# miha-stopar/Plonky3-mobile

Hardware: AMD Instinct MI355X
Metric: fib_air proofs/sec (higher is better)
Workload: dtype u32 (BabyBear Montgomery, 31-bit modular)

## Files before the change

### plonky3-mobile_amd/csrc/common.h

```cpp
#pragma once
#include <hip/hip_runtime.h>
#include <stdint.h>

#include <map>
#include <set>
#include <string>
#include <tuple>
#include <vector>

namespace p3 {

#ifndef P3_NO_SETPRIO
#define P3_LATENCY_BOUND_KERNEL() __builtin_amdgcn_s_setprio(3)
#else
#define P3_LATENCY_BOUND_KERNEL() ((void)0)
#endif

enum Profile : int { PROFILE_THROUGHPUT = 0, PROFILE_LATENCY = 1 };

enum Status : int {
    OK = 0,
    ERR_BAD_ARG = -1,
    ERR_HIP = -2,
    ERR_BACKEND = -3,
    ERR_INTERNAL = -4,
};

void set_error(const std::string& msg);
int fail(int code, const std::string& msg);

#define P3_HIP(call)                                                                       \
    do {                                                                                   \
        hipError_t e__ = (call);                                                           \
        if (e__ != hipSuccess)                                                             \
            return p3::fail(p3::ERR_HIP, std::string(#call) + ": " + hipGetErrorString(e__)); \
    } while (0)

struct DevBuf {
    void* ptr = nullptr;
    size_t cap = 0;
    int reserve(size_t bytes);
    template <class T>
    T* as() const { return reinterpret_cast<T*>(ptr); }
    ~DevBuf();
};

struct TwoLevelTable {
    uint32_t* lo = nullptr;
    uint32_t* hi = nullptr;
    uint32_t T = 0;
};

struct CachedTable {
    TwoLevelTable t;
    hipEvent_t ready = nullptr;
    hipStream_t built_on = nullptr;
    bool complete = false;
};

struct Context {
    int device = -1;
    int profile = PROFILE_LATENCY;
    uint32_t* tile_tw[2] = {nullptr, nullptr};
    double2* tile_twd[2] = {nullptr, nullptr};
    std::map<std::pair<uint32_t, int>, CachedTable> root_tables;
    std::map<std::tuple<uint32_t, uint32_t, uint32_t>, CachedTable> scale_tables;
    std::map<std::pair<hipStream_t, int>, DevBuf> scratch;
    std::set<const void*> attr_done;
    uint64_t* rng_jump = nullptr;
    std::map<uint32_t, CachedTable> selector_tables;
    int init(int dev);
    DevBuf& ws(hipStream_t stream, int slot);
    int get_root_table(hipStream_t stream, uint32_t q, bool inverse, TwoLevelTable* out);
    int get_scale_table(hipStream_t stream, uint32_t base, uint32_t log_n, uint32_t mult, TwoLevelTable* out);
    int reserve_scale_slots(size_t k);
    int mark_built(hipStream_t stream, CachedTable& e);
    int wait_ready(hipStream_t stream, CachedTable& e);
    int ensure_dynamic_lds(const void* kernel, int bytes);
    ~Context();
};

int get_context(Context** out);
void release_thread_contexts();

int ntt_dft(Context& cx, hipStream_t stream, const uint32_t* src, uint32_t* dst, uint64_t height,
            uint32_t width, bool inverse);
std::vector<uint32_t> ntt_dft_plan(uint32_t n);
int ntt_coset_lde(Context& cx, hipStream_t stream, const uint32_t* src, uint32_t* dst, uint64_t height,
                  uint32_t width, uint32_t added_bits, uint32_t shift_monty, bool bit_reversed_out);
int ntt_coset_lde_from_coeffs(Context& cx, hipStream_t stream, const uint32_t* coeffs, uint32_t* dst, uint32_t* scratch,
                              uint64_t height, uint32_t width, uint32_t added_bits, uint32_t shift_monty);
int ntt_coset_dft(Context& cx, hipStream_t stream, const uint32_t* src, uint32_t* dst, uint64_t height,
                  uint32_t width, uint32_t shift_monty);
int bit_reverse_rows(hipStream_t stream, const uint32_t* src, uint32_t* dst, uint64_t height, uint32_t width);

int fib_trace(hipStream_t stream, uint64_t a, uint64_t b, uint64_t n, uint32_t* d_out);
enum : uint32_t {
    TRACE_BAD_FIRST_LEFT = 1, TRACE_BAD_FIRST_RIGHT = 2, TRACE_BAD_NEXT_LEFT = 4, TRACE_BAD_NEXT_RIGHT = 8, TRACE_BAD_LAST_RIGHT = 16,
    TRACE_BAD_RANGE = 32,
};
struct TraceCheck {
    int64_t first_bad_row;
    uint32_t mask;
    uint64_t bad_rows;
};
int fib_check_trace(Context& cx, hipStream_t stream, const uint32_t* d_trace, uint64_t n, const uint32_t pis[3], TraceCheck* out);

inline bool is_pow2(uint64_t v) { return v && !(v & (v - 1)); }
inline uint32_t log2u(uint64_t v) {
    uint32_t l = 0;
    while ((1ull << l) < v) l++;
    return l;
}

}
```

### plonky3-mobile_amd/csrc/mmcs.hip

```cpp
#include <algorithm>

#include "common.h"
#include "mmcs.h"
#include "poseidon2.hip.h"
#include "poseidon2_coop.hip.h"
#include "poseidon2_f64.hip.h"
#include "poseidon2_q4.hip.h"
#include "keccak.hip.h"

namespace p3 {

constexpr int MAX_CLASS_MATS = 16;

struct RowSet {
    const uint32_t* ptr[MAX_CLASS_MATS];
    uint32_t width[MAX_CLASS_MATS];
    uint32_t stride[MAX_CLASS_MATS];
    uint32_t count;
    uint32_t total;
};

__device__ __forceinline__ void load_digest(const uint32_t* p, uint32_t* out8) {
    const uint4* q = reinterpret_cast<const uint4*>(p);
    uint4 a = q[0], b = q[1];
    out8[0] = a.x; out8[1] = a.y; out8[2] = a.z; out8[3] = a.w;
    out8[4] = b.x; out8[5] = b.y; out8[6] = b.z; out8[7] = b.w;
}
__device__ __forceinline__ void store_digest(uint32_t* p, const uint32_t* s) {
    uint4* q = reinterpret_cast<uint4*>(p);
    q[0] = make_uint4(s[0], s[1], s[2], s[3]);
    q[1] = make_uint4(s[4], s[5], s[6], s[7]);
}

__device__ __forceinline__ void sponge_row(const RowSet& rs, uint64_t r, uint32_t (&s)[16]) {
#pragma unroll
    for (int i = 0; i < 16; i++) s[i] = 0;
    if (rs.count == 1) {
        const uint32_t* row = rs.ptr[0] + r * rs.stride[0];
        const uint32_t w = rs.width[0];
        for (uint32_t k = 0; k < w; k += 8) {
#pragma unroll
            for (int i = 0; i < 8; i++)
                if (k + i < w) s[i] = row[k + i];
            p2::permute(s);
        }
        return;
    }
    uint32_t m = 0, off = 0;
    for (uint32_t k = 0; k < rs.total; k += 8) {
#pragma unroll
        for (int i = 0; i < 8; i++) {
            if (k + i < rs.total) {
                while (off >= rs.width[m]) { m++; off = 0; }
                s[i] = rs.ptr[m][r * rs.stride[m] + off];
                off++;
            }
        }
        p2::permute(s);
    }
}

__global__ void __launch_bounds__(256) leaf_hash_kernel(RowSet rs, uint64_t n_rows, uint32_t* digests) {
    if (gridDim.x <= 512u) P3_LATENCY_BOUND_KERNEL();
    uint64_t r = (uint64_t)blockIdx.x * blockDim.x + threadIdx.x;
    if (r >= n_rows) return;
    uint32_t s[16];
    sponge_row(rs, r, s);
    store_digest(digests + r * 8, s);
}

__global__ void __launch_bounds__(256) compress_layer_kernel(const uint32_t* prev, uint32_t* next, uint64_t n_out,
                                                             RowSet rs, uint32_t inject) {
    if (gridDim.x <= 512u) P3_LATENCY_BOUND_KERNEL();
    uint64_t i = (uint64_t)blockIdx.x * blockDim.x + threadIdx.x;
    if (i >= n_out) return;
    uint32_t s[16];
    load_digest(prev + i * 16, s);
    load_digest(prev + i * 16 + 8, s + 8);
    p2::permute(s);
    if (inject) {
        uint32_t h[16];
        sponge_row(rs, i, h);
#pragma unroll
        for (int k = 0; k < 8; k++) s[8 + k] = h[k];
        p2::permute(s);
    }
    store_digest(next + i * 8, s);
}

__global__ void __launch_bounds__(256) tree_top_kernel(uint32_t* layer0, uint32_t n0) {
    P3_LATENCY_BOUND_KERNEL();
    extern __shared__ __attribute__((aligned(16))) uint32_t lds[];
    const uint32_t tid = threadIdx.x;
    for (uint32_t i = tid; i < n0 * 8; i += blockDim.x) lds[i] = layer0[i];
    __syncthreads();
    uint32_t* out = layer0 + (size_t)n0 * 8;
    for (uint32_t n = n0; n > 1; n >>= 1) {
        uint32_t half = n >> 1;
        uint32_t s[16];
        bool act = tid < half;
        if (act) {
#pragma unroll
            for (int k = 0; k < 16; k++) s[k] = lds[tid * 16 + k];
            p2::permute(s);
        }
        __syncthreads();
        if (act) {
#pragma unroll
            for (int k = 0; k < 8; k++) lds[tid * 8 + k] = s[k];
            store_digest(out + tid * 8, s);
        }
        __syncthreads();
        out += (size_t)half * 8;
    }
}


__global__ void __launch_bounds__(256) leaf_hash_f64_kernel(const uint32_t* mat, uint32_t width, uint64_t n_rows, uint32_t* digests) {
    if (gridDim.x <= 512u) P3_LATENCY_BOUND_KERNEL();
    uint64_t r = (uint64_t)blockIdx.x * blockDim.x + threadIdx.x;
    if (r >= n_rows) return;
    double s[16];
#pragma unroll
    for (int i = 0; i < 16; i++) s[i] = 0.0;
    const uint32_t* row = mat + r * width;
    for (uint32_t k = 0; k < width; k += 8) {
#pragma unroll
        for (int i = 0; i < 8; i++)
            if (k + i < width) s[i] = p2f::load_elem(row[k + i]);
        p2f::permute(s);
        if (k + 8 < width) {
#pragma unroll
            for (int i = 0; i < 16; i++) s[i] = p2f::reduce(s[i]);
        }
    }
    uint32_t d[8];
    const p2f::MagicRegs smk = p2f::magic_regs();
#pragma unroll
    for (int i = 0; i < 8; i++) d[i] = p2f::store_elem(s[i], smk);
    store_digest(digests + r * 8, d);
}
__global__ void __launch_bounds__(256) compress_layer_q4_kernel(const uint32_t* prev, uint32_t* next, uint64_t n_out, uint32_t prio) {
    if (prio) P3_LATENCY_BOUND_KERNEL();
    const uint32_t q = threadIdx.x & 3u;
    const uint64_t i = ((uint64_t)blockIdx.x * blockDim.x + threadIdx.x) >> 2;
    const bool act = i < n_out;
    const p2q::LaneConsts lc = p2q::lane_consts(q);
    double s[4] = {0.0, 0.0, 0.0, 0.0};
    if (act) {
        const uint4 w = *reinterpret_cast<const uint4*>(prev + i * 16 + 4 * q);
        s[0] = p2f::load_elem(w.x); s[1] = p2f::load_elem(w.y); s[2] = p2f::load_elem(w.z); s[3] = p2f::load_elem(w.w);
    }
    p2q::permute(s, lc, q == 0);
    if (act && q < 2) {
        const p2f::MagicRegs smk = p2f::magic_regs();
        *reinterpret_cast<uint4*>(next + i * 8 + 4 * q) =
            make_uint4(p2f::store_elem(s[0], smk), p2f::store_elem(s[1], smk), p2f::store_elem(s[2], smk), p2f::store_elem(s[3], smk));
    }
}
__global__ void __launch_bounds__(256) leaf_hash_q4_kernel(const uint32_t* mat, uint32_t width, uint64_t n_rows, uint32_t* digests, uint32_t prio) {
    if (prio) P3_LATENCY_BOUND_KERNEL();
    const uint32_t q = threadIdx.x & 3u;
    const uint64_t r = ((uint64_t)blockIdx.x * blockDim.x + threadIdx.x) >> 2;
    const bool act = r < n_rows;
    const p2q::LaneConsts lc = p2q::lane_consts(q);
    double s[4] = {0.0, 0.0, 0.0, 0.0};
    const uint32_t* row = mat + (act ? r : 0) * width;
    for (uint32_t k = 0; k < width; k += 8) {
        if (act && q < 2) {
#pragma unroll
            for (uint32_t i = 0; i < 4; i++)
                if (k + 4 * q + i < width) s[i] = p2f::load_elem(row[k + 4 * q + i]);
        }
        p2q::permute(s, lc, q == 0);
        if (k + 8 < width) {
#pragma unroll
            for (int i = 0; i < 4; i++) s[i] = p2f::reduce(s[i]);
        }
    }
    if (act && q < 2) {
        const p2f::MagicRegs smk = p2f::magic_regs();
        *reinterpret_cast<uint4*>(digests + r * 8 + 4 * q) =
            make_uint4(p2f::store_elem(s[0], smk), p2f::store_elem(s[1], smk), p2f::store_elem(s[2], smk), p2f::store_elem(s[3], smk));
    }
}
constexpr uint32_t LEAF_WIDE_CHUNK = 32, LEAF_WIDE_STRIDE = 36;
__global__ void __launch_bounds__(256) leaf_hash_f64_wide_kernel(const uint32_t* mat, uint32_t width, uint64_t n_rows, uint32_t* digests) {
    __shared__ __attribute__((aligned(16))) uint32_t tile[256 * LEAF_WIDE_STRIDE];
    const uint32_t tid = threadIdx.x, col = tid & 31u, rsub = tid >> 5;
    const uint64_t r0 = (uint64_t)blockIdx.x * 256u, r = r0 + tid;
    double s[16];
#pragma unroll
    for (int i = 0; i < 16; i++) s[i] = 0.0;
    uint32_t pre[32];
    auto fetch = [&](uint32_t c0) {
#pragma unroll
        for (uint32_t i = 0; i < 32; i++) {
            const uint64_t row = r0 + rsub + 8u * i;
            pre[i] = (row < n_rows && c0 + col < width) ? mat[row * width + c0 + col] : 0u;
        }
    };
    fetch(0);
    for (uint32_t c0 = 0; c0 < width; c0 += LEAF_WIDE_CHUNK) {
        __syncthreads();
#pragma unroll
        for (uint32_t i = 0; i < 32; i++) tile[(rsub + 8u * i) * LEAF_WIDE_STRIDE + col] = pre[i];
        __syncthreads();
        if (c0 + LEAF_WIDE_CHUNK < width) fetch(c0 + LEAF_WIDE_CHUNK);
        const uint4* mine = reinterpret_cast<const uint4*>(tile + tid * LEAF_WIDE_STRIDE);
#pragma unroll 1
        for (uint32_t k = 0; k < LEAF_WIDE_CHUNK && c0 + k < width; k += 8) {
            const uint4 a = mine[k / 4], b = mine[k / 4 + 1];
            const uint32_t w[8] = {a.x, a.y, a.z, a.w, b.x, b.y, b.z, b.w};
#pragma unroll
            for (int i = 0; i < 8; i++)
                if (c0 + k + i < width) s[i] = p2f::load_elem(w[i]);
            p2f::permute(s);
            if (c0 + k + 8 < width) {
#pragma unroll
                for (int i = 0; i < 16; i++) s[i] = p2f::reduce(s[i]);
            }
        }
    }
    if (r >= n_rows) return;
    uint32_t d[8];
    const p2f::MagicRegs smk = p2f::magic_regs();
#pragma unroll
    for (int i = 0; i < 8; i++) d[i] = p2f::store_elem(s[i], smk);
    store_digest(digests + r * 8, d);
}
__global__ void __launch_bounds__(256) leaf_hash_f64_rowset_kernel(RowSet rs, uint64_t n_rows, uint32_t* digests) {
    if (gridDim.x <= 512u) P3_LATENCY_BOUND_KERNEL();
    uint64_t r = (uint64_t)blockIdx.x * blockDim.x + threadIdx.x;
    if (r >= n_rows) return;
    double s[16];
#pragma unroll
    for (int i = 0; i < 16; i++) s[i] = 0.0;
    uint32_t m = 0, off = 0;
    for (uint32_t k = 0; k < rs.total; k += 8) {
#pragma unroll
        for (int i = 0; i < 8; i++) {
            if (k + i < rs.total) {
                while (off >= rs.width[m]) { m++; off = 0; }
                s[i] = p2f::load_elem(rs.ptr[m][r * rs.stride[m] + off]);
                off++;
            }
        }
        p2f::permute(s);
        if (k + 8 < rs.total) {
#pragma unroll
            for (int i = 0; i < 16; i++) s[i] = p2f::reduce(s[i]);
        }
    }
    uint32_t d[8];
    const p2f::MagicRegs smk = p2f::magic_regs();
#pragma unroll
    for (int i = 0; i < 8; i++) d[i] = p2f::store_elem(s[i], smk);
    store_digest(digests + r * 8, d);
}
__global__ void __launch_bounds__(256) compress_layer_f64_kernel(const uint32_t* prev, uint32_t* next, uint64_t n_out) {
    if (gridDim.x <= 512u) P3_LATENCY_BOUND_KERNEL();
    uint64_t i = (uint64_t)blockIdx.x * blockDim.x + threadIdx.x;
    if (i >= n_out) return;
    uint32_t w[16];
    load_digest(prev + i * 16, w);
    load_digest(prev + i * 16 + 8, w + 8);
    double s[16];
#pragma unroll
    for (int k = 0; k < 16; k++) s[k] = p2f::load_elem(w[k]);
    p2f::permute(s);
    uint32_t d[8];
    const p2f::MagicRegs smk = p2f::magic_regs();
#pragma unroll
    for (int k = 0; k < 8; k++) d[k] = p2f::store_elem(s[k], smk);
    store_digest(next + i * 8, d);
}

__global__ void __launch_bounds__(256) compress_coop_kernel(const uint32_t* prev, uint32_t* next, uint32_t n_out) {
    P3_LATENCY_BOUND_KERNEL();
    const uint32_t lane16 = threadIdx.x & 15;
    const p2c::LaneConst lc = p2c::lane_constants(lane16);
    uint32_t i = (blockIdx.x * blockDim.x + threadIdx.x) >> 4;
    bool act = i < n_out;
    uint32_t v = act ? prev[(size_t)i * 16 + lane16] : 0u;
    v = p2c::permute(v, lc);
    if (act && lane16 < 8) next[(size_t)i * 8 + lane16] = v;
}
__global__ void __launch_bounds__(256) leaf_coop_kernel(const uint32_t* mat, uint32_t width, uint32_t n_rows, uint32_t* digests) {
    P3_LATENCY_BOUND_KERNEL();
    const uint32_t lane16 = threadIdx.x & 15;
    const p2c::LaneConst lc = p2c::lane_constants(lane16);
    uint32_t r = (blockIdx.x * blockDim.x + threadIdx.x) >> 4;
    bool act = r < n_rows;
    uint32_t v = 0;
    for (uint32_t k = 0; k < width; k += 8) {
        if (act && lane16 < 8 && k + lane16 < width) v = mat[(size_t)r * width + k + lane16];
        v = p2c::permute(v, lc);
    }
    if (act && lane16 < 8) digests[(size_t)r * 8 + lane16] = v;
}
__global__ void __launch_bounds__(1024) tree_levels_coop_kernel(uint32_t* layer_in, uint32_t n_in, uint32_t chunk, uint32_t levels,
                                                                uint32_t* root_copy) {
    P3_LATENCY_BOUND_KERNEL();
    __shared__ uint32_t lds[128 * 8];
    const uint32_t tid = threadIdx.x, lane16 = tid & 15, grp = tid >> 4;
    const p2c::LaneConst lc = p2c::lane_constants(lane16);
    const uint32_t* src = layer_in + (size_t)blockIdx.x * chunk * 8;
    for (uint32_t i = tid; i < chunk * 8; i += blockDim.x) lds[i] = src[i];
    __syncthreads();
    uint32_t* out = layer_in + (size_t)n_in * 8;
    uint32_t cur_n = n_in;
    for (uint32_t l = 0; l < levels; l++) {
        const uint32_t half = chunk >> (l + 1);
        const bool wave_active = ((tid >> 6) << 2) < half;
        uint32_t res = 0;
        if (wave_active) {
            uint32_t v = grp < half ? lds[grp * 16 + lane16] : 0u;
            res = p2c::permute(v, lc);
        }
        __syncthreads();
        if (grp < half && lane16 < 8) {
            lds[grp * 8 + lane16] = res;
            out[((size_t)blockIdx.x * half + grp) * 8 + lane16] = res;
            if (cur_n == 2 && root_copy) root_copy[lane16] = res;
        }
        __syncthreads();
        cur_n >>= 1;
        out += (size_t)cur_n * 8;
    }
}

__global__ void poseidon2_permute_kernel(uint32_t* states, uint64_t n) {
    uint64_t i = (uint64_t)blockIdx.x * blockDim.x + threadIdx.x;
    if (i >= n) return;
    uint32_t s[16];
    uint4* q = reinterpret_cast<uint4*>(states + i * 16);
#pragma unroll
    for (int k = 0; k < 4; k++) { uint4 v = q[k]; s[4 * k] = v.x; s[4 * k + 1] = v.y; s[4 * k + 2] = v.z; s[4 * k + 3] = v.w; }
    p2::permute(s);
#pragma unroll
    for (int k = 0; k < 4; k++) q[k] = make_uint4(s[4 * k], s[4 * k + 1], s[4 * k + 2], s[4 * k + 3]);
}


__global__ void poseidon2_permute_f64_kernel(uint32_t* states, uint64_t n) {
    uint64_t i = (uint64_t)blockIdx.x * blockDim.x + threadIdx.x;
    if (i >= n) return;
    double s[16];
    uint4* q = reinterpret_cast<uint4*>(states + i * 16);
#pragma unroll
    for (int k = 0; k < 4; k++) {
        uint4 v = q[k];
        s[4 * k] = p2f::load_elem(v.x); s[4 * k + 1] = p2f::load_elem(v.y); s[4 * k + 2] = p2f::load_elem(v.z); s[4 * k + 3] = p2f::load_elem(v.w);
    }
    p2f::permute(s);
#pragma unroll
    for (int k = 0; k < 4; k++)
        q[k] = make_uint4(p2f::store_elem(s[4 * k]), p2f::store_elem(s[4 * k + 1]), p2f::store_elem(s[4 * k + 2]), p2f::store_elem(s[4 * k + 3]));
}

__global__ void poseidon2_f64_probe_kernel(const double* in, uint32_t* out, uint64_t n, int mode) {
    uint64_t i = (uint64_t)blockIdx.x * blockDim.x + threadIdx.x;
    if (i >= n) return;
    double s[16];
#pragma unroll
    for (int k = 0; k < 16; k++) s[k] = in[i * 16 + k];
    if (mode == 0) p2f::permute(s);
    else if (mode == 1) p2f::internal_rounds(s, p2f::magic_regs());
    else {
#pragma unroll
        for (int k = 0; k < 16; k++) s[k] = p2f::reduce(s[k]);
    }
#pragma unroll
    for (int k = 0; k < 16; k++) out[i * 16 + k] = p2f::store_elem(s[k]);
}
int poseidon2_f64_probe(hipStream_t stream, const double* d_in, uint32_t* d_out, uint64_t n, int mode) {
    if (!n) return OK;
    hipLaunchKernelGGL(poseidon2_f64_probe_kernel, dim3((uint32_t)((n + 255) / 256)), dim3(256), 0, stream, d_in, d_out, n, mode);
    P3_HIP(hipGetLastError());
    return OK;
}
int poseidon2_permute_states_variant(hipStream_t stream, uint32_t* d_states, uint64_t n, int variant) {
    if (!n) return OK;
    if (variant == 1) hipLaunchKernelGGL(poseidon2_permute_f64_kernel, dim3((uint32_t)((n + 255) / 256)), dim3(256), 0, stream, d_states, n);
    else hipLaunchKernelGGL(poseidon2_permute_kernel, dim3((uint32_t)((n + 255) / 256)), dim3(256), 0, stream, d_states, n);
    P3_HIP(hipGetLastError());
    return OK;
}

int poseidon2_permute_states(hipStream_t stream, uint32_t* d_states, uint64_t n) {
    return poseidon2_permute_states_variant(stream, d_states, n, 1);
}

__device__ __forceinline__ uint32_t rowset_elem(const RowSet& rs, uint64_t r, uint32_t k, uint32_t& m, uint32_t& base) {
    while (k - base >= rs.width[m]) { base += rs.width[m]; m++; }
    return rs.ptr[m][r * rs.stride[m] + (k - base)];
}
__device__ __forceinline__ void keccak_sponge_row(const RowSet& rs, uint64_t r, uint64_t (&st)[25]) {
#pragma unroll
    for (int i = 0; i < 25; i++) st[i] = 0;
    const uint32_t n = rs.total, n64 = (n + 1) / 2;
    uint32_t m = 0, base = 0;
    for (uint32_t i = 0; i < n64; i += 17) {
#pragma unroll
        for (int k = 0; k < 17; k++) {
            const uint32_t e = 2 * (i + k);
            if (e < n) {
                uint64_t lo = rowset_elem(rs, r, e, m, base);
                uint64_t hi = e + 1 < n ? rowset_elem(rs, r, e + 1, m, base) : 0u;
                st[k] = lo | (hi << 32);
            }
        }
        if (i + 17 >= n64) kk::permute_digest(st);
        else kk::permute(st);
    }
}
__device__ __forceinline__ void store_digest64(uint32_t* p, const uint64_t (&st)[25]) {
    uint4* q = reinterpret_cast<uint4*>(p);
    q[0] = make_uint4((uint32_t)st[0], (uint32_t)(st[0] >> 32), (uint32_t)st[1], (uint32_t)(st[1] >> 32));
    q[1] = make_uint4((uint32_t)st[2], (uint32_t)(st[2] >> 32), (uint32_t)st[3], (uint32_t)(st[3] >> 32));
}
__global__ void __launch_bounds__(256) keccak_leaf_kernel(RowSet rs, uint64_t n_rows, uint32_t* digests) {
    if (gridDim.x <= 512u) P3_LATENCY_BOUND_KERNEL();
// ... 237 lines not shown
    uint64_t base = 0, len = 1ull << a.log_max_height;
    for (uint32_t i = 0; i < a.log_max_height; i++) {
        uint64_t sib = (index >> i) ^ 1;
        if (threadIdx.x < 8) out[off + i * 8 + threadIdx.x] = layers[base + sib * 8 + threadIdx.x];
        base += len * 8;
        len >>= 1;
    }
}

__global__ void __launch_bounds__(64) open_gather_many_kernel(OpenArgs a, const uint32_t* layers, const uint32_t* indices, uint32_t row_words,
                                                              uint32_t* rows, uint32_t* paths) {
    if (gridDim.x <= 512u) P3_LATENCY_BOUND_KERNEL();
    const uint64_t index = (uint64_t)indices[blockIdx.x] & ((1ull << a.log_max_height) - 1ull);
    uint32_t* dst = rows + (size_t)blockIdx.x * row_words;
    uint32_t off = 0;
    for (uint32_t m = 0; m < a.n_mats; m++) {
        const uint64_t r = index >> a.shift[m];
        for (uint32_t c = threadIdx.x; c < a.width[m]; c += blockDim.x) dst[off + c] = a.mat[m][r * a.stride[m] + c];
        off += a.width[m];
    }
    uint32_t* pdst = paths + (size_t)blockIdx.x * a.log_max_height * 8;
    uint64_t base = 0, len = 1ull << a.log_max_height;
    for (uint32_t i = 0; i < a.log_max_height; i++) {
        const uint64_t sib = (index >> i) ^ 1;
        if (threadIdx.x < 8) pdst[i * 8 + threadIdx.x] = layers[base + sib * 8 + threadIdx.x];
        base += len * 8;
        len >>= 1;
    }
}

static RowSet make_rowset(const Tree& t, uint64_t h) {
    RowSet rs{};
    for (size_t m = 0; m < t.mats.size(); m++)
        if (t.heights[m] == h) {
            rs.ptr[rs.count] = t.mats[m];
            rs.width[rs.count] = (uint32_t)t.widths[m];
            rs.stride[rs.count] = (uint32_t)t.strides[m];
            rs.total += (uint32_t)t.widths[m];
            rs.count++;
        }
    return rs;
}


static bool has_height(const Tree& t, uint64_t h) {
    for (size_t m = 0; m < t.mats.size(); m++)
        if (t.heights[m] == h) return true;
    return false;
}

Tree::~Tree() {
    if (layers && owns_layers) (void)hipFree(layers);
    if (staging) (void)hipFree(staging);
    for (void* p : owned) (void)hipFree(p);
}

int mmcs_commit(hipStream_t stream, const uint32_t* const* d_mats, const size_t* heights, const size_t* widths,
                size_t n_mats, Tree** out, uint32_t* ext_layers, uint32_t* root_copy, int kind, const size_t* strides, int profile) {
    if (kind != HASH_POSEIDON2 && kind != HASH_KECCAK) return fail(ERR_BAD_ARG, "mmcs_commit: unknown hash configuration");
    if (!n_mats || !d_mats || !heights || !widths || !out) return fail(ERR_BAD_ARG, "mmcs_commit: null/empty argument");
    if (n_mats > 64) return fail(ERR_BAD_ARG, "mmcs_commit: at most 64 matrices per commitment");
    uint64_t maxh = 0;
    for (size_t i = 0; i < n_mats; i++) {
        if (!is_pow2(heights[i])) return fail(ERR_BAD_ARG, "mmcs_commit: heights must be powers of two");
        if (widths[i] > 0xffffffffull) return fail(ERR_BAD_ARG, "mmcs_commit: width too large");
        if (heights[i] > maxh) maxh = heights[i];
    }
    std::unique_ptr<Tree> t(new Tree());
    t->kind = kind;
    for (size_t i = 0; i < n_mats; i++) {
        t->mats.push_back(d_mats[i]); t->heights.push_back(heights[i]); t->widths.push_back(widths[i]);
        const size_t st = strides ? strides[i] : widths[i];
        if (st < widths[i] || st > 0xffffffffull) return fail(ERR_BAD_ARG, "mmcs_commit: row stride below the width");
        t->strides.push_back(st);
    }
    t->log_max_height = log2u(maxh);
    for (uint64_t h = maxh; h >= 1; h >>= 1) {
        size_t cnt = 0;
        for (size_t i = 0; i < n_mats; i++) cnt += heights[i] == h;
        if (cnt > MAX_CLASS_MATS) return fail(ERR_BAD_ARG, "mmcs_commit: more than 16 matrices of one height");
        if (h == 1) break;
    }
    size_t total_digests = 2 * maxh - 1;
    size_t staging_words = 0;
    for (size_t i = 0; i < n_mats; i++) staging_words += widths[i];
    staging_words += (size_t)t->log_max_height * 8 + 8;
    t->staging_words = staging_words;
    if (ext_layers) { t->layers = ext_layers; t->owns_layers = false; }
    else P3_HIP(hipMalloc(reinterpret_cast<void**>(&t->layers), total_digests * 32));
    size_t off = 0;
    for (uint64_t len = maxh; len >= 1; len >>= 1) {
        t->layer_off.push_back(off);
        t->layer_len.push_back(len);
        off += len * 8;
        if (len == 1) break;
    }
    constexpr uint64_t COOP_MAX = 1ull << 12;
    constexpr uint32_t COOP_CHUNK_LOG = 5;
    const uint64_t Q4_MAX = profile == PROFILE_LATENCY ? (1ull << 15) : 0;
    constexpr uint32_t Q4_PRIO = 1;
    const uint64_t KCOOP_IN = profile == PROFILE_LATENCY ? (1ull << 12) : (1ull << 10);
    constexpr uint32_t KCOOP_CHUNK_LOG = 4;
    constexpr uint64_t KLANE_CHUNK = 1ull << 7;
    if (kind == HASH_KECCAK) {
        RowSet rs0 = make_rowset(*t, maxh);
        if (rs0.count == 1 && rs0.width[0] >= 68 && rs0.stride[0] == rs0.width[0])
            hipLaunchKernelGGL(keccak_leaf_wide_kernel, dim3((uint32_t)((maxh + 255) / 256)), dim3(256), 0, stream, rs0.ptr[0], rs0.width[0], maxh,
                               t->layers);
        else if (!launch_keccak_leaf_salted(stream, rs0, maxh, t->layers))
            hipLaunchKernelGGL(keccak_leaf_kernel, dim3((uint32_t)((maxh + 255) / 256)), dim3(256), 0, stream, rs0, maxh, t->layers);
        P3_HIP(hipGetLastError());
        for (size_t l = 1; l < t->layer_len.size(); l++) {
            uint64_t len = t->layer_len[l];
            RowSet rs = make_rowset(*t, len);
            if (len < COOP_MAX && !rs.count) {
                const uint64_t n_in = t->layer_len[l - 1];
                const bool coop = n_in <= KCOOP_IN;
                uint32_t levels = 0;
                while (levels < (coop ? KCOOP_CHUNK_LOG : 11u) && l + levels < t->layer_len.size() && !has_height(*t, t->layer_len[l + levels])) levels++;
                if (!coop) while (levels > 1 && (n_in >> levels) < KCOOP_IN) levels--;
                const uint32_t chunk = (uint32_t)std::min<uint64_t>(n_in, coop ? 1ull << KCOOP_CHUNK_LOG : KLANE_CHUNK);
                while ((1u << levels) > chunk) levels--;
                if (coop)
                    hipLaunchKernelGGL(keccak_tree_levels_coop_kernel, dim3((uint32_t)(n_in / chunk)), dim3(std::max<uint32_t>(64, chunk * 32)), 0,
                                       stream, t->layers + t->layer_off[l - 1], (uint32_t)n_in, chunk, levels, root_copy);
                else
                    hipLaunchKernelGGL(keccak_tree_levels_kernel, dim3((uint32_t)(n_in / chunk)), dim3(std::max<uint32_t>(64, chunk / 2)),
                                       (size_t)chunk * 32, stream, t->layers + t->layer_off[l - 1], (uint32_t)n_in, chunk, levels, root_copy);
                P3_HIP(hipGetLastError());
                if (t->layer_len[l + levels - 1] == 1) t->root_copied = root_copy != nullptr;
                l += levels - 1;
                continue;
            }
            hipLaunchKernelGGL(keccak_compress_kernel, dim3((uint32_t)((len + 255) / 256)), dim3(256), 0, stream,
                               t->layers + t->layer_off[l - 1], t->layers + t->layer_off[l], len, rs, rs.count > 0 ? 1u : 0u);
            P3_HIP(hipGetLastError());
        }
        *out = t.release();
        return OK;
    }
    {
        RowSet rs = make_rowset(*t, maxh);
        const bool dense1 = rs.count == 1 && rs.stride[0] == rs.width[0];
        if (dense1 && maxh < COOP_MAX && maxh * 16 <= 0x7fffffffull) {
            hipLaunchKernelGGL(leaf_coop_kernel, dim3((uint32_t)((maxh * 16 + 255) / 256)), dim3(256), 0, stream, rs.ptr[0],
                               rs.width[0], (uint32_t)maxh, t->layers);
        } else if (dense1 && maxh <= Q4_MAX && rs.width[0] <= 64 && (reinterpret_cast<uintptr_t>(t->layers) & 15u) == 0) {
            hipLaunchKernelGGL(leaf_hash_q4_kernel, dim3((uint32_t)((maxh * 4 + 255) / 256)), dim3(256), 0, stream, rs.ptr[0], rs.width[0], maxh,
                               t->layers, Q4_PRIO);
        } else if (dense1 && rs.width[0] >= 64) {
            hipLaunchKernelGGL(leaf_hash_f64_wide_kernel, dim3((uint32_t)((maxh + 255) / 256)), dim3(256), 0, stream, rs.ptr[0],
                               rs.width[0], maxh, t->layers);
        } else if (dense1) {
            hipLaunchKernelGGL(leaf_hash_f64_kernel, dim3((uint32_t)((maxh + 255) / 256)), dim3(256), 0, stream, rs.ptr[0],
                               rs.width[0], maxh, t->layers);
        } else if ((maxh >= COOP_MAX || (rs.count == 1 && !dense1))) {
            hipLaunchKernelGGL(leaf_hash_f64_rowset_kernel, dim3((uint32_t)((maxh + 255) / 256)), dim3(256), 0, stream, rs, maxh, t->layers);
        } else {
            hipLaunchKernelGGL(leaf_hash_kernel, dim3((uint32_t)((maxh + 255) / 256)), dim3(256), 0, stream, rs, maxh, t->layers);
        }
        P3_HIP(hipGetLastError());
    }
    for (size_t l = 1; l < t->layer_len.size();) {
        uint64_t len = t->layer_len[l];
        RowSet rs = make_rowset(*t, len);
        bool inject = rs.count > 0;
        if (!inject && len < COOP_MAX) {
            uint32_t levels = 0;
            while (levels < COOP_CHUNK_LOG && l + levels < t->layer_len.size() && !has_height(*t, t->layer_len[l + levels])) levels++;
            uint64_t n_in = t->layer_len[l - 1];
            uint32_t chunk = (uint32_t)std::min<uint64_t>(n_in, 1ull << COOP_CHUNK_LOG);
            while ((1u << levels) > chunk) levels--;
            uint32_t blocks = (uint32_t)(n_in / chunk);
            uint32_t threads = std::max<uint32_t>(64, chunk * 8);
            bool makes_root = t->layer_len[l + levels - 1] == 1;
            hipLaunchKernelGGL(tree_levels_coop_kernel, dim3(blocks), dim3(threads), 0, stream, t->layers + t->layer_off[l - 1],
                               (uint32_t)n_in, chunk, levels, makes_root ? root_copy : nullptr);
            P3_HIP(hipGetLastError());
            if (makes_root) t->root_copied = root_copy != nullptr;
            l += levels;
            continue;
        }
        if (!inject && len <= Q4_MAX) {
            hipLaunchKernelGGL(compress_layer_q4_kernel, dim3((uint32_t)((len * 4 + 255) / 256)), dim3(256), 0, stream,
                               t->layers + t->layer_off[l - 1], t->layers + t->layer_off[l], len, Q4_PRIO);
        } else if (!inject) {
            hipLaunchKernelGGL(compress_layer_f64_kernel, dim3((uint32_t)((len + 255) / 256)), dim3(256), 0, stream,
                               t->layers + t->layer_off[l - 1], t->layers + t->layer_off[l], len);
        } else {
            hipLaunchKernelGGL(compress_layer_kernel, dim3((uint32_t)((len + 255) / 256)), dim3(256), 0, stream,
                               t->layers + t->layer_off[l - 1], t->layers + t->layer_off[l], len, rs, inject ? 1u : 0u);
        }
        P3_HIP(hipGetLastError());
        l++;
    }
    *out = t.release();
    return OK;
}

int mmcs_root(hipStream_t stream, const Tree& t, uint32_t root_out[8]) {
    P3_HIP(hipMemcpyAsync(root_out, t.layers + t.layer_off.back(), 32, hipMemcpyDeviceToHost, stream));
    P3_HIP(hipStreamSynchronize(stream));
    return OK;
}

static OpenArgs make_open_args(const Tree& t) {
    OpenArgs a{};
    a.n_mats = (uint32_t)t.mats.size();
    a.log_max_height = t.log_max_height;
    for (size_t m = 0; m < t.mats.size(); m++) {
        a.mat[m] = t.mats[m];
        a.width[m] = (uint32_t)t.widths[m];
        a.stride[m] = (uint32_t)t.strides[m];
        a.shift[m] = t.log_max_height - log2u(t.heights[m]);
    }
    return a;
}
size_t mmcs_row_words(const Tree& t) {
    size_t row_words = 0;
    for (size_t w : t.widths) row_words += w;
    return row_words;
}

int mmcs_open(hipStream_t stream, const Tree& tc, uint64_t index, uint32_t* rows_out, uint32_t* path_out) {
    Tree& t = const_cast<Tree&>(tc);
    if (index >> t.log_max_height) return fail(ERR_BAD_ARG, "mmcs_open: index out of range");
    if (!t.staging) P3_HIP(hipMalloc(reinterpret_cast<void**>(&t.staging), t.staging_words * 4));
    const OpenArgs a = make_open_args(t);
    const size_t row_words = mmcs_row_words(t);
    hipLaunchKernelGGL(open_gather_kernel, dim3(1), dim3(64), 0, stream, a, t.layers, index, t.staging);
    P3_HIP(hipGetLastError());
    std::vector<uint32_t> host(row_words + (size_t)t.log_max_height * 8);
    if (!host.empty()) {
        P3_HIP(hipMemcpyAsync(host.data(), t.staging, host.size() * 4, hipMemcpyDeviceToHost, stream));
        P3_HIP(hipStreamSynchronize(stream));
    }
    if (row_words) memcpy(rows_out, host.data(), row_words * 4);
    if (t.log_max_height) memcpy(path_out, host.data() + row_words, (size_t)t.log_max_height * 32);
    return OK;
}

int mmcs_open_many(hipStream_t stream, const Tree& t, const uint32_t* d_indices, size_t n, uint32_t* d_rows, uint32_t* d_paths) {
    const size_t row_words = mmcs_row_words(t);
    if (n > 0x7fffffffull) return fail(ERR_BAD_ARG, "mmcs_open_batch_many: more than 2^31 - 1 indices");
    if (row_words > 0xffffffffull) return fail(ERR_BAD_ARG, "mmcs_open_batch_many: row too wide");
    if (n && (!d_indices || (row_words && !d_rows) || (t.log_max_height && !d_paths))) return fail(ERR_BAD_ARG, "mmcs_open_batch_many: null argument");
    if (!n) return OK;
    hipLaunchKernelGGL(open_gather_many_kernel, dim3((uint32_t)n), dim3(64), 0, stream, make_open_args(t), t.layers, d_indices, (uint32_t)row_words,
                       d_rows, d_paths);
    P3_HIP(hipGetLastError());
    return OK;
}

}
```

### plonky3-mobile_amd/csrc/ntt.hip

```cpp
#include <algorithm>

#include "bb31.hip.h"
#include "common.h"

namespace p3 {

enum SideKind : uint32_t {
    SIDE_INPLACE = 0,
    SIDE_GROUP = 1,
    SIDE_GROUP_REV = 2,
    SIDE_STRIDED = 3,
};

struct PassArgs {
    const uint32_t* src;
    uint32_t* dst;
    uint64_t src_rows;
    uint32_t W, wshift;
    uint32_t n, b, s0;
    uint32_t dif;
    uint32_t load_kind, store_kind;
    uint32_t G;
    uint32_t n_inner;
    const uint32_t* tile_tw;
// ... 648 lines not shown
    if (bi < 5 || (W < 32 && !is_pow2(W))) return 1;
    if (bi < 6) return 1;
    const uint64_t N = 1ull << n;
    size_t bytes = N * W * 4;
    int rc = cx.ws(stream, 1).reserve(bytes);
    if (rc) return rc;
    uint32_t* coeffs = cx.ws(stream, 1).as<uint32_t>();
    {
        uint32_t digits[2] = {e1, e2};
        uint32_t s = 0;
        for (int i = 0; i < 2; i++) {
            PassArgs a{};
            a.W = W; a.n = n; a.b = digits[i]; a.s0 = s; a.dif = 0;
            a.tile_tw = cx.tile_tw[1];
            a.src_rows = N;
            if (i == 0) { a.src = src; a.dst = coeffs; a.load_kind = SIDE_STRIDED; a.store_kind = SIDE_GROUP_REV; }
            else { a.src = coeffs; a.dst = coeffs; a.load_kind = SIDE_INPLACE; a.store_kind = SIDE_INPLACE; }
            rc = set_twiddle(cx, stream, a, true);
            if (rc) return rc;
            rc = launch_pass(cx, stream, a);
            if (rc) return rc;
            s += digits[i];
        }
    }
    {
        PassArgs a{};
        a.W = W; a.n = n; a.b = bi; a.s0 = s0;
        a.wshift = is_pow2(W) ? log2u(W) : 0xffffffffu;
        a.src = coeffs; a.dst = dst;
        a.tile_tw = cx.tile_tw[1];
        a.tile_tw2 = cx.tile_tw[0];
        TwoLevelTable ti, tf, sc;
        if ((rc = cx.get_root_table(stream, s0 + bi, true, &ti))) return rc;
        if ((rc = cx.get_root_table(stream, s0 + e3, false, &tf))) return rc;
        uint32_t hinv = bb::inv(bb::to_monty((uint32_t)N));
        if ((rc = cx.get_scale_table(stream, shift, n, hinv, &sc))) return rc;
        a.tw_lo = ti.lo; a.tw_hi = ti.hi; a.tw_T = ti.T;
        a.tw2_lo = tf.lo; a.tw2_hi = tf.hi; a.tw2_T = tf.T;
        a.sc_lo = sc.lo; a.sc_hi = sc.hi; a.sc_T = sc.T;
        a.sc_step = bb::pow(shift, 1ull << s0);
        a.sc_step16 = bb::pow(a.sc_step, 16);
        uint64_t F = (uint64_t)W << s0;
        uint32_t blocks = (uint32_t)((F + 31) / 32);
        if (bi == 6 && added == 1) rc = launch_fused_mid_t<6, 1>(stream, a, blocks);
        else if (bi == 7 && added == 1) rc = launch_fused_mid_t<7, 1>(stream, a, blocks);
        else if (bi == 6 && added == 2) rc = launch_fused_mid_t<6, 2>(stream, a, blocks);
        else return fail(ERR_INTERNAL, "lde_fused: unexpected digit shape");
        if (rc) return rc;
    }
    {
        PassArgs a{};
        a.W = W; a.n = m; a.b = e2; a.s0 = e1; a.dif = 1;
        a.tile_tw = cx.tile_tw[0];
        a.src = dst; a.dst = dst; a.src_rows = 1ull << m;
        a.load_kind = SIDE_INPLACE; a.store_kind = SIDE_INPLACE;
        if ((rc = set_twiddle(cx, stream, a, false))) return rc;
        if ((rc = launch_pass(cx, stream, a))) return rc;
        PassArgs b{};
        b.W = W; b.n = m; b.b = e1; b.s0 = 0; b.dif = 1;
        b.tile_tw = cx.tile_tw[0];
        b.src = dst; b.dst = dst; b.src_rows = 1ull << m;
        b.load_kind = SIDE_GROUP; b.store_kind = SIDE_GROUP;
        if ((rc = set_twiddle(cx, stream, b, false))) return rc;
        if ((rc = launch_pass(cx, stream, b))) return rc;
    }
    return OK;
}


template <int B, int LQ, int VW, int K>
int launch_narrow_t(Context& cx, hipStream_t stream, const NarrowArgs& a, uint32_t blocks, uint32_t grid_y = 1) {
    constexpr size_t tile_bytes = ((size_t)4 * VW * narrow::lds_rows(B)) << LQ;
    constexpr size_t n_tiles = K == 2 ? (B - 4 + LQ >= 10 ? 1 : NARROW_MID_TILES) : (B >= 11 ? 1 : NARROW_EDGE_TILES);
    constexpr size_t lds = tile_bytes * n_tiles + ((size_t)4 << (B - 4)) * (K == 2 ? 2 : 1);
    static_assert(lds <= 160 * 1024, "narrow tile does not fit the LDS");
    void (*kern)(NarrowArgs);
    if constexpr (K == 1) kern = narrow_inv1_kernel<B, LQ, VW>;
    else if constexpr (K == 2) kern = narrow_mid_kernel<B, LQ, VW>;
    else kern = narrow_fwd2_kernel<B, LQ, VW>;
    if constexpr (lds > 64 * 1024) {
        int rc = cx.ensure_dynamic_lds(reinterpret_cast<const void*>(kern), (int)lds);
        if (rc) return rc;
    }
    hipLaunchKernelGGL(kern, dim3(blocks, K == 2 ? grid_y : 1u), dim3(1u << (B - 4 + LQ)), lds, stream, a);
    P3_HIP(hipGetLastError());
    return OK;
}
constexpr int narrow_lq(int b, int vw) { return (b == 12 ? 1 : 2) + (vw == 1 ? 1 : 0); }
template <int K, int VW>
int launch_narrow_v(Context& cx, hipStream_t stream, const NarrowArgs& a, uint32_t b, uint32_t blocks, uint32_t gy) {
    if (b == 10) return launch_narrow_t<10, narrow_lq(10, VW), VW, K>(cx, stream, a, blocks, gy);
    if constexpr (VW == 2) {
        if (b == 11) return launch_narrow_t<11, narrow_lq(11, 2), 2, K>(cx, stream, a, blocks, gy);
        if (b == 12) return launch_narrow_t<12, narrow_lq(12, 2), 2, K>(cx, stream, a, blocks, gy);
    }
    return fail(ERR_INTERNAL, "lde_narrow: no integer kernel for this digit / lane vector");
}
template <int K>
int launch_narrow(Context& cx, hipStream_t stream, const NarrowArgs& a, uint32_t b, uint32_t blocks, int vw, uint32_t gy = 1) {
    return vw == 1 ? launch_narrow_v<K, 1>(cx, stream, a, b, blocks, gy) : launch_narrow_v<K, 2>(cx, stream, a, b, blocks, gy);
}

template <int B, int LQ, int VW, int K, int NT>
int launch_narrow64_nt(Context& cx, hipStream_t stream, const NarrowArgs& a, uint32_t blocks, uint32_t grid_y) {
    constexpr size_t lds = narrow64::lds_bytes<B, LQ, VW, NT>(K == 2 ? 2 : 1);
    static_assert(lds <= 160 * 1024, "fp64 narrow tile does not fit the LDS");
    void (*kern)(NarrowArgs);
    if constexpr (K == 1) kern = narrow64_inv1_kernel<B, LQ, VW, NT>;
    else if constexpr (K == 2) kern = narrow64_mid_kernel<B, LQ, VW, NT, (VW == 2)>;
    else kern = narrow64_fwd2_kernel<B, LQ, VW, NT>;
    if constexpr (lds > 64 * 1024) {
        int rc = cx.ensure_dynamic_lds(reinterpret_cast<const void*>(kern), (int)lds);
        if (rc) return rc;
    }
    hipLaunchKernelGGL(kern, dim3(blocks, K == 2 ? grid_y : 1u), dim3(1u << (B - 4 + LQ)), lds, stream, a);
    P3_HIP(hipGetLastError());
    return OK;
}
template <int B, int LQ, int VW, int K>
int launch_narrow64_t(Context& cx, hipStream_t stream, const NarrowArgs& a, uint32_t blocks, uint32_t grid_y) {
    constexpr bool fits2 = narrow64::lds_bytes<B, LQ, VW, 2>(K == 2 ? 2 : 1) <= 160 * 1024;
    if constexpr (fits2) {
        const bool two = (size_t)blocks * grid_y <= 256 || narrow64::lds_bytes<B, LQ, VW, 2>(K == 2 ? 2 : 1) <= 80 * 1024;
        if (two) return launch_narrow64_nt<B, LQ, VW, K, 2>(cx, stream, a, blocks, grid_y);
    }
    return launch_narrow64_nt<B, LQ, VW, K, 1>(cx, stream, a, blocks, grid_y);
}
constexpr bool narrow64_has(int b, int vw, int k) { return b <= 10 && b - 4 + narrow_lq(b, vw) <= (k == 2 ? 9 : 10); }
template <int K, int VW>
int launch_narrow64_v(Context& cx, hipStream_t stream, const NarrowArgs& a, uint32_t b, uint32_t blocks, uint32_t gy) {
#define P3_N64_CASE(BB)                                                                                          \
    case BB:                                                                                                     \
        if constexpr (narrow64_has(BB, VW, K)) return launch_narrow64_t<BB, narrow_lq(BB, VW), VW, K>(cx, stream, a, blocks, gy); \
        else return fail(ERR_INTERNAL, "lde_narrow: fp64 shape not instantiated");
    switch (b) {
        P3_N64_CASE(8) P3_N64_CASE(9) P3_N64_CASE(10)
        default: return fail(ERR_INTERNAL, "lde_narrow: digit out of range");
    }
#undef P3_N64_CASE
}
template <int K>
int launch_narrow64(Context& cx, hipStream_t stream, const NarrowArgs& a, uint32_t b, uint32_t blocks, int vw, uint32_t gy = 1) {
    return vw == 1 ? launch_narrow64_v<K, 1>(cx, stream, a, b, blocks, gy) : launch_narrow64_v<K, 2>(cx, stream, a, b, blocks, gy);
}

template <int K>
int launch_narrow_wide(Context& cx, hipStream_t stream, const NarrowArgs& a, uint32_t b, uint32_t blocks, uint32_t gy) {
    if (b == 9) return launch_narrow_t<9, 5, 1, K>(cx, stream, a, blocks, gy);
    if (b != 8) return fail(ERR_INTERNAL, "lde_narrow: wide digit out of range");
    return launch_narrow_t<8, 5, 1, K>(cx, stream, a, blocks, gy);
}

int lde_narrow(Context& cx, hipStream_t stream, const uint32_t* src, uint32_t* dst, uint32_t n, uint32_t added, uint32_t W,
               uint32_t shift, bool bit_reversed_out, bool from_coeffs = false) {
    if (!bit_reversed_out || added < 1 || added > 3) return 1;
    constexpr uint32_t w_max = 16;
    const bool wide = W > w_max && n >= 16 && n <= 18 && W >= 64 && (((uint64_t)W << (n + added + 2)) < (1ull << 32));
    if (!wide && (W < 2 || W > w_max || !(is_pow2(W) || W == 6))) return 1;
    if (n < 16 || n > 24) return 1;
    if (!wide && ((reinterpret_cast<uintptr_t>(src) | reinterpret_cast<uintptr_t>(dst)) & 7u)) return 1;
    const uint32_t n1 = (n + 1) / 2, n2 = n - n1;
    const uint64_t N = 1ull << n;
    int vw[3];
    for (int k = 0; k < 3; k++) vw[k] = (n <= 19 || (n == 20 && k == 1)) ? 1 : 2;
    if (wide) vw[0] = vw[1] = vw[2] = 1;
    auto lq_of = [&](int k, uint32_t b) -> uint32_t { return wide ? 5u : (uint32_t)narrow_lq((int)b, vw[k]); };
    int rc = cx.ws(stream, 1).reserve(N * W * 4);
    if (rc) return rc;
    uint32_t* T = cx.ws(stream, 1).as<uint32_t>();
    NarrowArgs a{};
    a.blocked = W == 2 && !from_coeffs;
    bool k3_out_of_place = a.blocked && n1 >= 12;
    uint32_t* mid = dst;
    if (k3_out_of_place) {
        const size_t mid_bytes = (N << added) * W * 4;
        if ((rc = cx.ws(stream, 4).reserve(mid_bytes))) return rc;
        mid = cx.ws(stream, 4).as<uint32_t>();
        const uintptr_t m0 = reinterpret_cast<uintptr_t>(mid), d0 = reinterpret_cast<uintptr_t>(dst);
        if (m0 < d0 + mid_bytes && d0 < m0 + mid_bytes) { a.blocked = 0; k3_out_of_place = false; mid = dst; }
    }
    a.from_coeffs = from_coeffs;
    a.n = n; a.n1 = n1; a.n2 = n2; a.W = W; a.added = added;
    TwoLevelTable ti, tf;
    if ((rc = cx.get_root_table(stream, n, true, &ti))) return rc;
    if ((rc = cx.get_root_table(stream, n, false, &tf))) return rc;
    auto geometry = [&](int k, uint32_t b, uint64_t rows) -> uint32_t {
        const uint32_t slots_per_row = W / vw[k];
        a.spr = slots_per_row;
        a.wsl = is_pow2(slots_per_row) ? log2u(slots_per_row) : 0xffffffffu;
        const uint32_t lq = lq_of(k, b);
        const uint32_t tiles = (uint32_t)((rows * slots_per_row) >> lq);
        const uint32_t group = 8u << (wide ? 0 : (vw[k] == 2 ? 4 : 5) - lq);
        a.xcd_remap = !wide && k != 2 && tiles % group == 0 && is_pow2(slots_per_row);
        if (wide && tiles % 128 == 0) a.xcd_remap = 4;
        return tiles;
    };
    a.src = src; a.dst = T;
    a.stage_tw = cx.tile_tw[1];
    a.tw_lo = ti.lo; a.tw_hi = ti.hi; a.tw_T = ti.T;
    const bool f64 = !wide && (n <= 19 || (n == 20 && W == 2));
    a.stage_twd = cx.tile_twd[1];
    a.neg_pm1 = -2013265920.0; a.pinv = 1.0 / 2013265921.0; a.fbias = -0.5 + 1.0 / 8589934592.0;
    uint32_t tiles = geometry(0, n1, 1ull << n2);
    if (!from_coeffs)
        if ((rc = wide ? launch_narrow_wide<1>(cx, stream, a, n1, tiles, 1)
                       : f64 ? launch_narrow64<1>(cx, stream, a, n1, tiles, vw[0]) : launch_narrow<1>(cx, stream, a, n1, tiles, vw[0]))) return rc;
    a.src = from_coeffs ? src : T; a.dst = mid;
    a.stage_tw = cx.tile_tw[1]; a.stage_tw_fwd = cx.tile_tw[0];
    a.stage_twd = cx.tile_twd[1]; a.stage_twd_fwd = cx.tile_twd[0];
    a.twf_lo = tf.lo; a.twf_hi = tf.hi; a.twf_T = tf.T;
    const uint32_t hinv = from_coeffs ? bb::ONE : bb::inv(bb::to_monty((uint32_t)N));
    const uint32_t g = bb::two_adic_generator(n + added);
    uint32_t base = shift;
    for (uint32_t j = 0; j < (1u << added); j++) {
        TwoLevelTable sc;
        if ((rc = cx.get_scale_table(stream, base, n, hinv, &sc))) return rc;
        a.sc_lo[j] = sc.lo; a.sc_hi[j] = sc.hi; a.sc_T = sc.T;
        a.sc_phi[j] = bb::pow(base, 1ull << (n1 + n2 - 4));
        base = bb::mul(base, g);
    }
    tiles = geometry(1, n2, 1ull << n1);
    uint32_t split_log = 0;
    while (split_log < added && ((uint64_t)tiles << (split_log + 1)) <= 256) split_log++;
    a.cos_per_block = (1u << added) >> split_log;
    if ((rc = wide ? launch_narrow_wide<2>(cx, stream, a, n2, tiles, 1u << split_log)
                   : f64 ? launch_narrow64<2>(cx, stream, a, n2, tiles, vw[1], 1u << split_log)
                         : launch_narrow<2>(cx, stream, a, n2, tiles, vw[1], 1u << split_log))) return rc;
    a.src = mid; a.dst = dst;
    a.stage_tw = cx.tile_tw[0];
    a.stage_twd = cx.tile_twd[0];
    tiles = geometry(2, n1, (1ull << added) << n2);
    a.k3_pairs = k3_out_of_place && vw[2] == 2 && tiles % 16 == 0 ? 1u : 0u;
    if (wide && tiles % 128 == 0) a.k3_pairs = 4;
    if (wide) return launch_narrow_wide<3>(cx, stream, a, n1, tiles, 1);
    return f64 ? launch_narrow64<3>(cx, stream, a, n1, tiles, vw[2]) : launch_narrow<3>(cx, stream, a, n1, tiles, vw[2]);
}

}

std::vector<uint32_t> ntt_dft_plan(uint32_t n) { return split_digits(n); }

int ntt_dft(Context& cx, hipStream_t stream, const uint32_t* src, uint32_t* dst, uint64_t height,
            uint32_t width, bool inverse) {
    if (!height || !width) return OK;
    if (!is_pow2(height)) return fail(ERR_BAD_ARG, "hip backend requires power-of-two height, got " + std::to_string(height));
    uint32_t n = log2u(height);
    if (n > bb::TWO_ADICITY) return fail(ERR_BAD_ARG, "height exceeds BabyBear two-adicity");
    size_t bytes = height * width * 4;
    if (n == 0) {
        if (src != dst) P3_HIP(hipMemcpyAsync(dst, src, bytes, hipMemcpyDeviceToDevice, stream));
        return OK;
    }
    if (src == dst) {
        int rc = cx.ws(stream, 0).reserve(bytes);
        if (rc) return rc;
        P3_HIP(hipMemcpyAsync(cx.ws(stream, 0).ptr, src, bytes, hipMemcpyDeviceToDevice, stream));
        src = cx.ws(stream, 0).as<uint32_t>();
    }
    uint32_t hinv = inverse ? bb::inv(bb::to_monty((uint32_t)height)) : 0;
    return run_dit(cx, stream, src, dst, n, width, inverse, inverse, hinv);
}

int ntt_coset_dft(Context& cx, hipStream_t stream, const uint32_t* src, uint32_t* dst, uint64_t height,
                  uint32_t width, uint32_t shift) {
    if (!height || !width) return OK;
    if (!is_pow2(height)) return fail(ERR_BAD_ARG, "hip backend requires power-of-two height, got " + std::to_string(height));
    uint32_t n = log2u(height);
    if (n > bb::TWO_ADICITY) return fail(ERR_BAD_ARG, "height exceeds BabyBear two-adicity");
    TwoLevelTable sc;
    int rc = cx.reserve_scale_slots(1);
    if (rc) return rc;
    rc = cx.get_scale_table(stream, shift, n, bb::ONE, &sc);
    if (rc) return rc;
    if (n == 0) {
        if (src != dst) P3_HIP(hipMemcpyAsync(dst, src, height * width * 4, hipMemcpyDeviceToDevice, stream));
        return OK;
    }
    if (src == dst) return fail(ERR_BAD_ARG, "coset_dft: in-place not supported");
    return run_dif(cx, stream, src, height, dst, n, width, false, &sc, shift, true);
}

int ntt_coset_lde_from_coeffs(Context& cx, hipStream_t stream, const uint32_t* coeffs, uint32_t* dst, uint32_t* scratch,
                              uint64_t height, uint32_t width, uint32_t added_bits, uint32_t shift) {
    if (!height || !width) return OK;
    if (!is_pow2(height)) return fail(ERR_BAD_ARG, "hip backend requires power-of-two height, got " + std::to_string(height));
    const uint32_t n = log2u(height);
    if (n + added_bits > bb::TWO_ADICITY) return fail(ERR_BAD_ARG, "LDE height exceeds BabyBear two-adicity");
    { int rcs = cx.reserve_scale_slots(8); if (rcs) return rcs; }
    int rcn = lde_narrow(cx, stream, coeffs, dst, n, added_bits, width, shift, true, true);
    if (rcn != 1) return rcn;
    int rc = ntt_dft(cx, stream, coeffs, scratch, height, width, false);
    if (rc) return rc;
    return ntt_coset_lde(cx, stream, scratch, dst, height, width, added_bits, shift, true);
}

int ntt_coset_lde(Context& cx, hipStream_t stream, const uint32_t* src, uint32_t* dst, uint64_t height,
                  uint32_t width, uint32_t added_bits, uint32_t shift, bool bit_reversed_out) {
    if (!height || !width) return OK;
    if (!is_pow2(height)) return fail(ERR_BAD_ARG, "hip backend requires power-of-two height, got " + std::to_string(height));
    uint32_t n = log2u(height);
    uint32_t m = n + added_bits;
    if (m > bb::TWO_ADICITY) return fail(ERR_BAD_ARG, "LDE height exceeds BabyBear two-adicity");
    if (src == dst) return fail(ERR_BAD_ARG, "coset_lde: in-place not supported");
    size_t bytes = height * width * 4;
    { int rcs = cx.reserve_scale_slots(8); if (rcs) return rcs; }
    {
        int rcn = lde_narrow(cx, stream, src, dst, n, added_bits, width, shift, bit_reversed_out);
        if (rcn != 1) return rcn;
    }
    {
        int rcf = lde_fused(cx, stream, src, dst, n, added_bits, width, shift, bit_reversed_out);
        if (rcf != 1) return rcf;
    }
    int rc = cx.ws(stream, 1).reserve(bytes);
    if (rc) return rc;
    uint32_t* coeffs = cx.ws(stream, 1).as<uint32_t>();
    if (n == 0) P3_HIP(hipMemcpyAsync(coeffs, src, bytes, hipMemcpyDeviceToDevice, stream));
    else {
        rc = run_dit(cx, stream, src, coeffs, n, width, true, false, 0);
        if (rc) return rc;
    }
    if (m == 0) {
        P3_HIP(hipMemcpyAsync(dst, coeffs, bytes, hipMemcpyDeviceToDevice, stream));
        return OK;
    }
    TwoLevelTable sc;
    uint32_t hinv = bb::inv(bb::to_monty((uint32_t)height));
    rc = cx.get_scale_table(stream, shift, n, hinv, &sc);
    if (rc) return rc;
    return run_dif(cx, stream, coeffs, height, dst, m, width, false, &sc, shift, !bit_reversed_out);
}

}
```

### plonky3-mobile_amd/csrc/ntt_narrow.hip.h

```cpp
#pragma once

constexpr uint32_t NARROW_EDGE_TILES = 2;
constexpr uint32_t NARROW_MID_TILES = 2;
namespace p3 {

struct NarrowArgs {
    const uint32_t* src;
    uint32_t* dst;
    uint32_t n, n1, n2, W, wsl;
    uint32_t spr;
    uint32_t from_coeffs;
    uint32_t added;
    const uint32_t* stage_tw;
    const uint32_t* stage_tw_fwd;
    const uint32_t* tw_lo;
    const uint32_t* tw_hi;
    uint32_t tw_T;
    const uint32_t* twf_lo;
    const uint32_t* twf_hi;
    uint32_t twf_T;
    const uint32_t* sc_lo[8];
    const uint32_t* sc_hi[8];
    uint32_t sc_T;
    uint32_t sc_phi[8];
    uint32_t xcd_remap;
    uint32_t cos_per_block;
    const double2* stage_twd;
    const double2* stage_twd_fwd;
    double neg_pm1, pinv, fbias;
    uint32_t k3_pairs;
    uint32_t blocked;
};

namespace narrow {


template <int VW> struct Vec;
template <> struct Vec<1> { using T = uint32_t; };
template <> struct Vec<2> { using T = uint2; };
__device__ __forceinline__ uint32_t add2(uint32_t a, uint32_t b) { return bb::add(a, b); }
__device__ __forceinline__ uint32_t sub2(uint32_t a, uint32_t b) { return bb::sub(a, b); }
__device__ __forceinline__ uint32_t subl2(uint32_t a, uint32_t b) { return a - b + bb::P; }
__device__ __forceinline__ uint32_t mul2(uint32_t a, uint32_t w) { return bb::mul(a, w); }
__device__ __forceinline__ uint2 add2(uint2 a, uint2 b) { return make_uint2(bb::add(a.x, b.x), bb::add(a.y, b.y)); }
__device__ __forceinline__ uint2 sub2(uint2 a, uint2 b) { return make_uint2(bb::sub(a.x, b.x), bb::sub(a.y, b.y)); }
__device__ __forceinline__ uint2 subl2(uint2 a, uint2 b) { return make_uint2(a.x - b.x + bb::P, a.y - b.y + bb::P); }
__device__ __forceinline__ uint2 mul2(uint2 a, uint32_t w) { return make_uint2(bb::mul(a.x, w), bb::mul(a.y, w)); }

template <int A>
__device__ __forceinline__ uint32_t pt_of(uint32_t t, uint32_t j) {
    return ((t >> A) << (A + 4)) | (j << A) | (t & ((1u << A) - 1u));
}
template <int LQ, int A>
__device__ __forceinline__ uint32_t lds_base(uint32_t t, uint32_t q) {
    const uint32_t T = ((t >> A) << (A + 4)) | (t & ((1u << A) - 1u));
    return ((T + (T >> 4)) << LQ) + q;
}
template <int LQ>
constexpr uint32_t lds_joff(uint32_t J) { return (J + (J >> 4)) << LQ; }
constexpr uint32_t lds_rows(int B) { return (1u << B) + (1u << (B - 4)); }

template <int A, int UHI, int ULO, class V>
__device__ __forceinline__ void stage_block(V (&v)[16], const uint32_t* __restrict__ tw, uint32_t t) {
    const uint32_t tlo = t & ((1u << A) - 1u);
#pragma unroll
    for (int u = UHI - 1; u >= ULO; --u) {
        const int d = u - A;
        uint32_t w[8];
        if (u > 0) {
#pragma unroll
            for (int jl = 0; jl < 8; jl++)
                if (jl < (1 << d)) w[jl] = tw[(1u << u) - 1u + (tlo | ((uint32_t)jl << A))];
        }
#pragma unroll
        for (int j0 = 0; j0 < 16; j0++) {
            if ((j0 >> d) & 1) continue;
            const int j1 = j0 | (1 << d);
            const V x = v[j0], y = v[j1];
            v[j0] = add2(x, y);
            if (u == 0) v[j1] = sub2(x, y);
            else v[j1] = mul2(subl2(x, y), w[j0 & ((1 << d) - 1)]);
        }
    }
}

template <int B>
__device__ __forceinline__ void load_round1_twiddles(const uint32_t* __restrict__ tw, uint32_t t, uint32_t (&w1)[15]) {
#pragma unroll
    for (int d = 0; d < 4; d++)
#pragma unroll
        for (int jl = 0; jl < (1 << d); jl++) w1[(1 << d) - 1 + jl] = tw[(1u << (B - 4 + d)) - 1u + (t | ((uint32_t)jl << (B - 4)))];
}
template <class V>
__device__ __forceinline__ void stage_block_round1(V (&v)[16], const uint32_t (&w1)[15]) {
#pragma unroll
    for (int d = 3; d >= 0; --d) {
#pragma unroll
        for (int j0 = 0; j0 < 16; j0++) {
            if ((j0 >> d) & 1) continue;
            const int j1 = j0 | (1 << d);
            const V x = v[j0], y = v[j1];
            v[j0] = add2(x, y);
            v[j1] = mul2(subl2(x, y), w1[(1 << d) - 1 + (j0 & ((1 << d) - 1))]);
        }
    }
}

template <class V, bool TWO>
struct Tiles {
    V* a;
    V* b;
    __device__ __forceinline__ V* next() {
        if constexpr (TWO) { V* r = a; a = b; b = r; return r; }
        __syncthreads();
        return a;
    }
};

template <int LQ, int AF, int AT, class V, class TL>
__device__ __forceinline__ void exchange(TL& tiles, V (&v)[16], uint32_t t, uint32_t q) {
    V* tile = tiles.next();
    V* wp = tile + lds_base<LQ, AF>(t, q);
#pragma unroll
    for (uint32_t j = 0; j < 16; j++) wp[lds_joff<LQ>(j << AF)] = v[j];
    __syncthreads();
    const V* rp = tile + lds_base<LQ, AT>(t, q);
#pragma unroll
    for (uint32_t j = 0; j < 16; j++) v[j] = rp[lds_joff<LQ>(j << AT)];
}

template <int B, int LQ, class V, class TL>
__device__ __forceinline__ void dif_rounds_after1(V (&v)[16], TL& tile, const uint32_t* twl, uint32_t t, uint32_t q) {
    constexpr int A1 = B - 4, A2 = B > 8 ? B - 8 : 0;
    exchange<LQ, A1, A2, V>(tile, v, t, q);
    stage_block<A2, A1, A2>(v, twl, t);
    if constexpr (B > 8) {
        exchange<LQ, A2, 0, V>(tile, v, t, q);
        stage_block<0, A2, 0>(v, twl, t);
    }
}
template <int B, int LQ, class V, class TL>
__device__ __forceinline__ void dif_rounds(V (&v)[16], TL& tile, const uint32_t (&w1)[15], const uint32_t* twl, uint32_t t, uint32_t q) {
    stage_block_round1(v, w1);
    dif_rounds_after1<B, LQ>(v, tile, twl, t, q);
}
template <int B, int LQ, class V, class TL>
__device__ __forceinline__ void to_natural(TL& tiles, V (&v)[16], uint32_t t, uint32_t q) {
    V* tile = tiles.next();
    const uint32_t rt = rev_bits(t, B - 4);
    V* wp = tile + (((rt + (rt >> 4)) << LQ) + q);
#pragma unroll
    for (uint32_t j = 0; j < 16; j++) wp[lds_joff<LQ>(crev(j, 4) << (B - 4))] = v[j];
    __syncthreads();
    const V* rp = tile + lds_base<LQ, B - 4>(t, q);
#pragma unroll
    for (uint32_t j = 0; j < 16; j++) v[j] = rp[lds_joff<LQ>(j << (B - 4))];
}
template <int B, int LQ, class V, class TL>
__device__ __forceinline__ void to_rows(TL& tile, V (&v)[16], uint32_t t, uint32_t q) {
    exchange<LQ, 0, B - 4, V>(tile, v, t, q);
}

template <int LQ, int VW>
__device__ __forceinline__ uint32_t tile_of_block(uint32_t bid, uint32_t remap) {
    if (!remap) return bid;
    const uint32_t LG = remap == 1 ? (VW == 2 ? 4u : 5u) - LQ : remap;
    const uint32_t xcd = bid & 7u, s = bid >> 3;
    return ((s >> LG) << (LG + 3)) | (xcd << LG) | (s & ((1u << LG) - 1u));
}

template <class V>
__device__ __forceinline__ V ldv(const void* base, uint32_t off) {
    return *reinterpret_cast<const V*>(static_cast<const char*>(base) + off);
}
template <class V>
__device__ __forceinline__ void stv(void* base, uint32_t off, V v) {
    *reinterpret_cast<V*>(static_cast<char*>(base) + off) = v;
}

template <bool REV, class V>
__device__ __forceinline__ void scale_ladder(V (&v)[16], uint32_t c, uint32_t phi) {
    uint32_t pw[16];
    power_ladder<16>(c, phi, pw);
#pragma unroll
    for (uint32_t j = 0; j < 16; j++) v[j] = mul2(v[j], pw[REV ? crev(j, 4) : j]);
}

}

__device__ __forceinline__ uint32_t k3_tile_of_block(uint32_t bid, uint32_t lg) {
    if (!lg) return bid;
    const uint32_t xcd = bid & 7u, s = bid >> 3;
    return ((s >> lg) << (lg + 3)) | (xcd << lg) | (s & ((1u << lg) - 1u));
}
__device__ __forceinline__ uint32_t slot_row(const NarrowArgs& a, uint32_t s) { return a.wsl != 0xffffffffu ? s >> a.wsl : s / a.spr; }
__device__ __forceinline__ uint32_t slot_col(const NarrowArgs& a, uint32_t s, uint32_t row) {
    return a.wsl != 0xffffffffu ? s & ((1u << a.wsl) - 1u) : s - row * a.spr;
}

template <int B, int LQ, int VW>
__global__ void __launch_bounds__(1 << (B - 4 + LQ)) narrow_inv1_kernel(NarrowArgs a) {
    using namespace narrow;
    using V = typename Vec<VW>::T;
    constexpr uint32_t NQ = 1u << LQ, NTH = 1u << (B - 4 + LQ);
    extern __shared__ __attribute__((aligned(16))) uint32_t smem[];
    constexpr uint32_t NT = B >= 11 ? 1 : NARROW_EDGE_TILES;
    Tiles<V, (NT > 1)> tile{reinterpret_cast<V*>(smem), reinterpret_cast<V*>(smem) + (NT - 1) * (lds_rows(B) << LQ)};
    uint32_t* twl = smem + (NT * VW * lds_rows(B) << LQ);
    const uint32_t q = threadIdx.x & (NQ - 1), t = threadIdx.x >> LQ;
    const uint32_t s = tile_of_block<LQ, VW>(blockIdx.x, a.xcd_remap) * NQ + q;
    const uint32_t lo = slot_row(a, s), cp = slot_col(a, s, lo);
    const uint32_t rowstride = a.W << a.n2;
    const uint32_t ld_off = (VW * s + t * rowstride) * 4u;
    V v[16];
#pragma unroll
    for (uint32_t j = 0; j < 16; j++) v[j] = ldv<V>(a.src + ((uint64_t)j << (B - 4)) * rowstride, ld_off);
    uint32_t w1[15];
    load_round1_twiddles<B>(a.stage_tw, t, w1);
    for (uint32_t i = threadIdx.x; i + 1 < (1u << (B - 4)); i += NTH) twl[i] = a.stage_tw[i];
    const uint32_t c = two_level(a.tw_lo, a.tw_hi, a.tw_T, (uint64_t)lo * rev_bits(t, B - 4));
    const uint32_t phi = two_level(a.tw_lo, a.tw_hi, a.tw_T, (uint64_t)lo << (B - 4));
    dif_rounds<B, LQ>(v, tile, w1, twl, t, q);
    scale_ladder<true>(v, c, phi);
    to_natural<B, LQ>(tile, v, t, q);
    if (a.blocked) {
        const uint32_t blk_off = ((((lo >> 2) << (B - 2)) + (t >> 2)) * 16u + (lo & 3u) * 4u + (t & 3u)) * 8u + cp * 4u;
#pragma unroll
        for (uint32_t j = 0; j < 16; j++) stv<V>(a.dst + ((uint64_t)j << (B - 6)) * 32u, blk_off, v[j]);
        return;
    }
    const uint32_t st_off = (((lo << B) + t) * a.W + VW * cp) * 4u;
#pragma unroll
    for (uint32_t j = 0; j < 16; j++) stv<V>(a.dst + ((uint64_t)j << (B - 4)) * a.W, st_off, v[j]);
}

template <int B, int LQ, int VW>
__global__ void __launch_bounds__(1 << (B - 4 + LQ), 1)
narrow_mid_kernel(NarrowArgs a) {
    using namespace narrow;
    using V = typename Vec<VW>::T;
    constexpr uint32_t NQ = 1u << LQ, NTH = 1u << (B - 4 + LQ);
    constexpr bool LEAN = NTH >= 512;
    constexpr uint32_t NT = NTH >= 1024 ? 1 : NARROW_MID_TILES;
    extern __shared__ __attribute__((aligned(16))) uint32_t smem[];
    Tiles<V, (NT > 1)> tile{reinterpret_cast<V*>(smem), reinterpret_cast<V*>(smem) + (NT - 1) * (lds_rows(B) << LQ)};
    uint32_t* twl_i = smem + (NT * VW * lds_rows(B) << LQ);
    uint32_t* twl_f = twl_i + (1u << (B - 4));
    const uint32_t q = threadIdx.x & (NQ - 1), t = threadIdx.x >> LQ;
    const uint32_t s = tile_of_block<LQ, VW>(blockIdx.x, a.xcd_remap) * NQ + q;
    const uint32_t k1 = slot_row(a, s);
    const uint32_t rowstride = a.W << a.n1;
    const uint32_t ld_off = (VW * s + t * rowstride) * 4u, st_off = (VW * s + (t << 4) * rowstride) * 4u;
    const bool blocked = a.blocked;
    const uint32_t blk_off = ((((t >> 2) << (a.n1 - 2)) + (k1 >> 2)) * 16u + (t & 3u) * 4u + (k1 & 3u)) * 8u +
                             (VW == 1 ? (s & 1u) * 4u : 0u);
    const uint64_t blk_jstride = ((uint64_t)32u << (B - 6)) << (a.n1 - 2);
    V c[16];
#pragma unroll
    for (uint32_t j = 0; j < 16; j++)
        c[j] = blocked ? ldv<V>(a.src + (uint64_t)j * blk_jstride, blk_off) : ldv<V>(a.src + ((uint64_t)j << (B - 4)) * rowstride, ld_off);
    {
        uint32_t w1[15];
        load_round1_twiddles<B>(a.stage_tw, t, w1);
        for (uint32_t i = threadIdx.x; i + 1 < (1u << (B - 4)); i += NTH) twl_i[i] = a.stage_tw[i];
        for (uint32_t i = threadIdx.x; i + 1 < (1u << (B - 4)); i += NTH) twl_f[i] = a.stage_tw_fwd[i];
        if (!a.from_coeffs) dif_rounds<B, LQ>(c, tile, w1, twl_i, t, q);
    }
    const uint32_t c0 = two_level(a.twf_lo, a.twf_hi, a.twf_T, (uint64_t)k1 * rev_bits(t, B - 4));
    const uint32_t phi0 = two_level(a.twf_lo, a.twf_hi, a.twf_T, (uint64_t)k1 << (B - 4));
    const uint64_t kbase = (uint64_t)k1 + ((uint64_t)t << a.n1);
    const uint32_t cos0 = blockIdx.y * a.cos_per_block, ncos = cos0 + a.cos_per_block;
    uint32_t sc_next = two_level(a.sc_lo[cos0], a.sc_hi[cos0], a.sc_T, kbase);
    if (!a.from_coeffs) to_natural<B, LQ>(tile, c, t, q);
    {
        uint32_t pw2[16];
        if constexpr (!LEAN) power_ladder<16>(c0, phi0, pw2);
        for (uint32_t jc = cos0; jc < ncos; jc++) {
            const uint32_t sc = sc_next;
            if (jc + 1 < ncos) sc_next = two_level(a.sc_lo[jc + 1], a.sc_hi[jc + 1], a.sc_T, kbase);
            uint32_t w1[15];
            load_round1_twiddles<B>(a.stage_tw_fwd, t, w1);
            V v[16];
#pragma unroll
            for (uint32_t j = 0; j < 16; j++) v[j] = c[j];
            scale_ladder<false>(v, sc, a.sc_phi[jc]);
            dif_rounds<B, LQ>(v, tile, w1, twl_f, t, q);
            uint32_t* o = a.dst + ((uint64_t)rev_bits(jc, a.added) << a.n) * a.W;
            if (blocked) {
                const uint32_t fin_off = (((t << 2) << (a.n1 - 2)) + (k1 >> 2)) * 128u + (k1 & 3u) * 8u + (VW == 1 ? (s & 1u) * 4u : 0u);
                uint32_t pwl[16];
                if constexpr (LEAN) power_ladder<16>(c0, phi0, pwl);
#pragma unroll
                for (uint32_t j = 0; j < 16; j++)
                    stv<V>(o + ((uint64_t)(j >> 2) << (a.n1 - 2)) * 32u, fin_off + (j & 3u) * 32u, mul2(v[j], LEAN ? pwl[crev(j, 4)] : pw2[crev(j, 4)]));
                continue;
            }
            if constexpr (LEAN) {
                scale_ladder<true>(v, c0, phi0);
#pragma unroll
                for (uint32_t j = 0; j < 16; j++) stv<V>(o + (uint64_t)j * rowstride, st_off, v[j]);
            } else {
#pragma unroll
                for (uint32_t j = 0; j < 16; j++) stv<V>(o + (uint64_t)j * rowstride, st_off, mul2(v[j], pw2[crev(j, 4)]));
            }
        }
    }
}

template <int B, int LQ, int VW>
__global__ void __launch_bounds__(1 << (B - 4 + LQ)) narrow_fwd2_kernel(NarrowArgs a) {
    using namespace narrow;
    using V = typename Vec<VW>::T;
    constexpr uint32_t NQ = 1u << LQ, NTH = 1u << (B - 4 + LQ);
    extern __shared__ __attribute__((aligned(16))) uint32_t smem[];
    constexpr uint32_t NT = B >= 11 ? 1 : NARROW_EDGE_TILES;
    Tiles<V, (NT > 1)> tile{reinterpret_cast<V*>(smem), reinterpret_cast<V*>(smem) + (NT - 1) * (lds_rows(B) << LQ)};
    uint32_t* twl = smem + (NT * VW * lds_rows(B) << LQ);
    const uint32_t q = threadIdx.x & (NQ - 1), t = threadIdx.x >> LQ;
    const uint32_t tile0 = k3_tile_of_block(blockIdx.x, a.k3_pairs);
    const uint32_t s = tile0 * NQ + q;
    const uint32_t blk0 = slot_row(a, tile0 * NQ), blk = slot_row(a, s), cp = slot_col(a, s, blk);
    uint32_t* p = a.dst + ((uint64_t)blk0 << B) * a.W;
    const uint32_t off = ((((blk - blk0) << B) + t) * a.W + VW * cp) * 4u;
    V v[16];
    if (a.blocked) {
        const uint32_t g0 = blk0 & ~3u;
        const uint32_t* ps = a.src + ((uint64_t)g0 << B) * a.W;
        const uint32_t blk_off = ((t >> 2) * 16u + (blk - g0) * 4u + (t & 3u)) * 8u + cp * 4u;
#pragma unroll
        for (uint32_t j = 0; j < 16; j++) v[j] = ldv<V>(ps + ((uint64_t)j << (B - 6)) * 32u, blk_off);
    } else {
#pragma unroll
        for (uint32_t j = 0; j < 16; j++) v[j] = ldv<V>(p + ((uint64_t)j << (B - 4)) * a.W, off);
    }
    uint32_t w1[15];
    load_round1_twiddles<B>(a.stage_tw, t, w1);
    for (uint32_t i = threadIdx.x; i + 1 < (1u << (B - 4)); i += NTH) twl[i] = a.stage_tw[i];
    dif_rounds<B, LQ>(v, tile, w1, twl, t, q);
    to_rows<B, LQ>(tile, v, t, q);
#pragma unroll
    for (uint32_t j = 0; j < 16; j++) stv<V>(p + ((uint64_t)j << (B - 4)) * a.W, off, v[j]);
}

}
```

### plonky3-mobile_amd/csrc/ntt_narrow_f64.hip.h

```cpp
#pragma once
#include "poseidon2_f64.hip.h"

namespace p3 {
namespace narrow64 {
using namespace narrow;

constexpr double PD = 2013265921.0;

struct Magic { double m, mp; };
__device__ __forceinline__ Magic pin_magic() {
    Magic r{p2f::MAGIC, p2f::MAGIC_P};
    asm volatile("" : "+v"(r.m), "+v"(r.mp));
    return r;
}
struct Uni { double npm1, pinv, fbias; };

__device__ __forceinline__ double mulm(double a, double aP, double b, const Magic& k, double npm1) {
    const double qb = __fma_rn(b, aP, k.m);
    const double c = __fma_rn(qb, npm1, k.mp);
    const double t = __fma_rn(a, b, c);
    return t - qb;
}
__device__ __forceinline__ double canon(uint32_t monty) { return (double)bb::from_monty(monty); }

// ... 112 lines not shown
    const uint32_t rt = rev_bits(t, B - 4);
    double* wp = tile + (((rt + (rt >> 4)) << LQ) + q);
#pragma unroll
    for (uint32_t j = 0; j < 16; j++)
#pragma unroll
        for (int cc = 0; cc < VW; cc++) wp[cc * PL + lds_joff<LQ>(crev(j, 4) << (B - 4))] = v[j].c[cc];
    __syncthreads();
    const double* rp = tile + lds_base<LQ, B - 4>(t, q);
#pragma unroll
    for (uint32_t j = 0; j < 16; j++)
#pragma unroll
        for (int cc = 0; cc < VW; cc++) v[j].c[cc] = rp[cc * PL + lds_joff<LQ>(j << (B - 4))];
}

template <int B, int LQ, int VW, bool NATURAL, class TL>
__device__ __forceinline__ void exchange_words(TL& tiles, typename Vec<VW>::T (&w)[16], uint32_t t, uint32_t q) {
    using V = typename Vec<VW>::T;
    V* tile = reinterpret_cast<V*>(tiles.next());
    if constexpr (NATURAL) {
        const uint32_t rt = rev_bits(t, B - 4);
        V* wp = tile + (((rt + (rt >> 4)) << LQ) + q);
#pragma unroll
        for (uint32_t j = 0; j < 16; j++) wp[lds_joff<LQ>(crev(j, 4) << (B - 4))] = w[j];
    } else {
        V* wp = tile + lds_base<LQ, 0>(t, q);
#pragma unroll
        for (uint32_t j = 0; j < 16; j++) wp[lds_joff<LQ>(j)] = w[j];
    }
    __syncthreads();
    const V* rp = tile + lds_base<LQ, B - 4>(t, q);
#pragma unroll
    for (uint32_t j = 0; j < 16; j++) w[j] = rp[lds_joff<LQ>(j << (B - 4))];
}
template <int VW, bool CENTERED>
__device__ __forceinline__ typename Vec<VW>::T to_words(const DV<VW>& v, const Uni& u) {
    if constexpr (VW == 2) {
        if constexpr (CENTERED) return make_uint2(word_centered(v.c[0]), word_centered(v.c[1]));
        else return make_uint2(word_any(v.c[0], u), word_any(v.c[1], u));
    } else {
        if constexpr (CENTERED) return word_centered(v.c[0]);
        else return word_any(v.c[0], u);
    }
}

__device__ __forceinline__ void power_ladder16(double c, double phi, double (&pw)[16], const Magic& k, const Uni& un) {
    pw[0] = c;
    double step = phi;
#pragma unroll
    for (int len = 1; len < 16; len <<= 1) {
        const double sP = step * un.pinv;
#pragma unroll
        for (int i = 0; i < len; i++) pw[len + i] = mulm(step, sP, pw[i], k, un.npm1);
        if (len * 2 < 16) step = mulm(step, sP, step, k, un.npm1);
    }
}
template <bool REV, int VW>
__device__ __forceinline__ void scale_by(DV<VW> (&v)[16], const double (&pw)[16], const Magic& k, const Uni& un) {
#pragma unroll
    for (uint32_t j = 0; j < 16; j++) {
        const double w = pw[REV ? crev(j, 4) : j], wP = w * un.pinv;
#pragma unroll
        for (int cc = 0; cc < VW; cc++) v[j].c[cc] = mulm(w, wP, v[j].c[cc], k, un.npm1);
    }
}

template <int B, int LQ, int VW, int NT>
constexpr size_t lds_bytes(int tables) {
    return ((size_t)8 * VW * NT * lds_rows(B) << LQ) + (size_t)tables * ((size_t)16 << (B - 4));
}

}

template <int B, int LQ, int VW, int NT>
__global__ void __launch_bounds__(1 << (B - 4 + LQ)) narrow64_inv1_kernel(NarrowArgs a) {
    using namespace narrow64;
    constexpr uint32_t NQ = 1u << LQ, NTH = 1u << (B - 4 + LQ), PL = lds_rows(B) << LQ;
    extern __shared__ __attribute__((aligned(16))) uint32_t smem[];
    double* t0 = reinterpret_cast<double*>(smem);
    constexpr uint32_t TD = VW * PL;
    Tiles<double, (NT > 1)> tile{t0, t0 + (NT - 1) * TD};
    double2* twl = reinterpret_cast<double2*>(t0 + NT * TD);
    const Magic mk = pin_magic();
    const Uni un{a.neg_pm1, a.pinv, a.fbias};
    const uint32_t q = threadIdx.x & (NQ - 1), t = threadIdx.x >> LQ;
    const uint32_t s = tile_of_block<LQ, VW>(blockIdx.x, a.xcd_remap) * NQ + q;
    const uint32_t lo = slot_row(a, s), cp = slot_col(a, s, lo);
    const uint32_t rowstride = a.W << a.n2;
    const uint32_t ld_off = (VW * s + t * rowstride) * 4u;
    DV<VW> v[16];
#pragma unroll
    for (uint32_t j = 0; j < 16; j++) v[j] = ld_words<VW>(a.src + ((uint64_t)j << (B - 4)) * rowstride, ld_off);
    double w1[15];
    load_round1_twiddles<B>(a.stage_twd, t, w1);
    for (uint32_t i = threadIdx.x; i + 1 < (1u << (B - 4)); i += NTH) twl[i] = a.stage_twd[i];
    const double c = canon(two_level(a.tw_lo, a.tw_hi, a.tw_T, (uint64_t)lo * rev_bits(t, B - 4)));
    const double phi = canon(two_level(a.tw_lo, a.tw_hi, a.tw_T, (uint64_t)lo << (B - 4)));
    dif_rounds<B, LQ>(v, tile, w1, twl, t, q, mk, un);
    {
        double pw[16];
        power_ladder16(c, phi, pw, mk, un);
        scale_by<true>(v, pw, mk, un);
    }
    using WV = typename Vec<VW>::T;
    WV w[16];
#pragma unroll
    for (uint32_t j = 0; j < 16; j++) w[j] = to_words<VW, true>(v[j], un);
    exchange_words<B, LQ, VW, true>(tile, w, t, q);
    if (a.blocked) {
        const uint32_t blk_off = ((((lo >> 2) << (B - 2)) + (t >> 2)) * 16u + (lo & 3u) * 4u + (t & 3u)) * 8u + cp * 4u;
#pragma unroll
        for (uint32_t j = 0; j < 16; j++) stv<WV>(a.dst + ((uint64_t)j << (B - 6)) * 32u, blk_off, w[j]);
        return;
    }
    const uint32_t st_off = (((lo << B) + t) * a.W + VW * cp) * 4u;
#pragma unroll
    for (uint32_t j = 0; j < 16; j++) stv<WV>(a.dst + ((uint64_t)j << (B - 4)) * a.W, st_off, w[j]);
}

template <int B, int LQ, int VW, int NT, bool LEAN>
__global__ void __launch_bounds__(1 << (B - 4 + LQ)) narrow64_mid_kernel(NarrowArgs a) {
    using namespace narrow64;
    constexpr uint32_t NQ = 1u << LQ, NTH = 1u << (B - 4 + LQ), PL = lds_rows(B) << LQ;
    extern __shared__ __attribute__((aligned(16))) uint32_t smem[];
    double* t0 = reinterpret_cast<double*>(smem);
    constexpr uint32_t TD = VW * PL;
    Tiles<double, (NT > 1)> tile{t0, t0 + (NT - 1) * TD};
    double2* twl_i = reinterpret_cast<double2*>(t0 + NT * TD);
    double2* twl_f = twl_i + (1u << (B - 4));
    const Magic mk = pin_magic();
    const Uni un{a.neg_pm1, a.pinv, a.fbias};
    const uint32_t q = threadIdx.x & (NQ - 1), t = threadIdx.x >> LQ;
    const uint32_t s = tile_of_block<LQ, VW>(blockIdx.x, a.xcd_remap) * NQ + q;
    const uint32_t k1 = slot_row(a, s);
    const uint32_t rowstride = a.W << a.n1;
    const uint32_t ld_off = (VW * s + t * rowstride) * 4u, st_off = (VW * s + (t << 4) * rowstride) * 4u;
    const bool blocked = a.blocked;
    const uint32_t blk_off = ((((t >> 2) << (a.n1 - 2)) + (k1 >> 2)) * 16u + (t & 3u) * 4u + (k1 & 3u)) * 8u +
                             (VW == 1 ? (s & 1u) * 4u : 0u);
    const uint64_t blk_jstride = ((uint64_t)32u << (B - 6)) << (a.n1 - 2);
    DV<VW> c[16];
#pragma unroll
    for (uint32_t j = 0; j < 16; j++)
        c[j] = blocked ? ld_words<VW>(a.src + (uint64_t)j * blk_jstride, blk_off) : ld_words<VW>(a.src + ((uint64_t)j << (B - 4)) * rowstride, ld_off);
    {
        double w1[15];
        load_round1_twiddles<B>(a.stage_twd, t, w1);
        for (uint32_t i = threadIdx.x; i + 1 < (1u << (B - 4)); i += NTH) twl_i[i] = a.stage_twd[i];
        for (uint32_t i = threadIdx.x; i + 1 < (1u << (B - 4)); i += NTH) twl_f[i] = a.stage_twd_fwd[i];
        if (!a.from_coeffs) dif_rounds<B, LQ>(c, tile, w1, twl_i, t, q, mk, un);
    }
    const double c0 = canon(two_level(a.twf_lo, a.twf_hi, a.twf_T, (uint64_t)k1 * rev_bits(t, B - 4)));
    const double phi0 = canon(two_level(a.twf_lo, a.twf_hi, a.twf_T, (uint64_t)k1 << (B - 4)));
    const uint64_t kbase = (uint64_t)k1 + ((uint64_t)t << a.n1);
    const uint32_t cos0 = blockIdx.y * a.cos_per_block, ncos = cos0 + a.cos_per_block;
    uint32_t sc_next = two_level(a.sc_lo[cos0], a.sc_hi[cos0], a.sc_T, kbase);
    if (!a.from_coeffs) {
        to_natural<B, LQ>(tile, c, t, q);
    }
    double pw2[16];
    if constexpr (!LEAN) power_ladder16(c0, phi0, pw2, mk, un);
    for (uint32_t jc = cos0; jc < ncos; jc++) {
        const double sc = canon(sc_next);
        if (jc + 1 < ncos) sc_next = two_level(a.sc_lo[jc + 1], a.sc_hi[jc + 1], a.sc_T, kbase);
        double w1[15];
        load_round1_twiddles<B>(a.stage_twd_fwd, t, w1);
        DV<VW> v[16];
        {
            double pw[16];
            power_ladder16(sc, canon(a.sc_phi[jc]), pw, mk, un);
#pragma unroll
            for (uint32_t j = 0; j < 16; j++) {
                const double w = pw[j], wP = w * un.pinv;
#pragma unroll
                for (int cc = 0; cc < VW; cc++) v[j].c[cc] = mulm(w, wP, c[j].c[cc], mk, un.npm1);
            }
        }
        dif_rounds<B, LQ>(v, tile, w1, twl_f, t, q, mk, un);
        if constexpr (LEAN) power_ladder16(c0, phi0, pw2, mk, un);
        scale_by<true>(v, pw2, mk, un);
        uint32_t* o = a.dst + ((uint64_t)rev_bits(jc, a.added) << a.n) * a.W;
        if (blocked) {
            const uint32_t fin_off = (((t << 2) << (a.n1 - 2)) + (k1 >> 2)) * 128u + (k1 & 3u) * 8u + (VW == 1 ? (s & 1u) * 4u : 0u);
#pragma unroll
            for (uint32_t j = 0; j < 16; j++)
                st_words<VW, true>(o + ((uint64_t)(j >> 2) << (a.n1 - 2)) * 32u, fin_off + (j & 3u) * 32u, v[j], un);
            continue;
        }
#pragma unroll
        for (uint32_t j = 0; j < 16; j++) st_words<VW, true>(o + (uint64_t)j * rowstride, st_off, v[j], un);
    }
}

template <int B, int LQ, int VW, int NT>
__global__ void __launch_bounds__(1 << (B - 4 + LQ)) narrow64_fwd2_kernel(NarrowArgs a) {
    using namespace narrow64;
    constexpr uint32_t NQ = 1u << LQ, NTH = 1u << (B - 4 + LQ), PL = lds_rows(B) << LQ;
    extern __shared__ __attribute__((aligned(16))) uint32_t smem[];
    double* t0 = reinterpret_cast<double*>(smem);
    constexpr uint32_t TD = VW * PL;
    Tiles<double, (NT > 1)> tile{t0, t0 + (NT - 1) * TD};
    double2* twl = reinterpret_cast<double2*>(t0 + NT * TD);
    const Magic mk = pin_magic();
    const Uni un{a.neg_pm1, a.pinv, a.fbias};
    const uint32_t q = threadIdx.x & (NQ - 1), t = threadIdx.x >> LQ;
    const uint32_t tile0 = k3_tile_of_block(blockIdx.x, a.k3_pairs);
    const uint32_t s = tile0 * NQ + q;
    const uint32_t blk0 = slot_row(a, tile0 * NQ), blk = slot_row(a, s), cp = slot_col(a, s, blk);
    uint32_t* p = a.dst + ((uint64_t)blk0 << B) * a.W;
    const uint32_t off = ((((blk - blk0) << B) + t) * a.W + VW * cp) * 4u;
    DV<VW> v[16];
    if (a.blocked) {
        const uint32_t g0 = blk0 & ~3u;
        const uint32_t* ps = a.src + ((uint64_t)g0 << B) * a.W;
        const uint32_t blk_off = ((t >> 2) * 16u + (blk - g0) * 4u + (t & 3u)) * 8u + cp * 4u;
#pragma unroll
        for (uint32_t j = 0; j < 16; j++) v[j] = ld_words<VW>(ps + ((uint64_t)j << (B - 6)) * 32u, blk_off);
    } else {
#pragma unroll
        for (uint32_t j = 0; j < 16; j++) v[j] = ld_words<VW>(p + ((uint64_t)j << (B - 4)) * a.W, off);
    }
    double w1[15];
    load_round1_twiddles<B>(a.stage_twd, t, w1);
    for (uint32_t i = threadIdx.x; i + 1 < (1u << (B - 4)); i += NTH) twl[i] = a.stage_twd[i];
    dif_rounds<B, LQ>(v, tile, w1, twl, t, q, mk, un);
    using WV = typename Vec<VW>::T;
    WV w[16];
#pragma unroll
    for (uint32_t j = 0; j < 16; j++) w[j] = to_words<VW, false>(v[j], un);
    exchange_words<B, LQ, VW, false>(tile, w, t, q);
#pragma unroll
    for (uint32_t j = 0; j < 16; j++) stv<WV>(p + ((uint64_t)j << (B - 4)) * a.W, off, w[j]);
}

}
```

### plonky3-mobile_amd/csrc/poseidon2_f64.hip.h

```cpp
#pragma once
#include "poseidon2.hip.h"

namespace p2f {

constexpr double PD = 2013265921.0;
constexpr double PINV = 1.0 / 2013265921.0;

__device__ __forceinline__ double mulmod(double a, double b) {
    double h = a * b;
    double l = __fma_rn(a, b, -h);
    double q = __builtin_rint(h * PINV);
    double r = __fma_rn(-q, PD, h);
    return r + l;
}
constexpr double PM1 = 2013265920.0;
__device__ __forceinline__ double mulmod_p(double a, double b, double aP) {
    double q = __builtin_rint(b * aP);
    double t = __fma_rn(a, b, -(q * PM1));
    return t - q;
}
__device__ __forceinline__ double reduce(double x) {
    return __fma_rn(-__builtin_rint(x * PINV), PD, x);
}
__device__ __forceinline__ double add_scaled_pow2(double tot, double x, double inv) {
    double xt = __fma_rn(x, inv, tot);
    double fr = __builtin_amdgcn_fract(xt);
    return __fma_rn(fr, -PD, xt);
}
constexpr double MAGIC = 6755399441055744.0;
constexpr double MAGIC_P = 6755399441055744.0 * 2013265921.0;
struct MagicRegs { double m, mp; };
__device__ __forceinline__ MagicRegs magic_regs() {
    MagicRegs r{MAGIC, MAGIC_P};
    asm volatile("" : "+v"(r.m), "+v"(r.mp));
    return r;
}
__device__ __forceinline__ double mulmod_m(double a, double b, double aP, const MagicRegs& k, double neg_pm1) {
    const double qb = __fma_rn(b, aP, k.m);
    const double c = __fma_rn(qb, neg_pm1, k.mp);
    const double t = __fma_rn(a, b, c);
    return t - qb;
}
__device__ __forceinline__ double sbox7(double x, const MagicRegs& k, double neg_pm1, double pinv) {
    const double xP = x * pinv;
    const double x2 = mulmod_m(x, x, xP, k, neg_pm1), x3 = mulmod_m(x, x2, xP, k, neg_pm1), x4 = mulmod_m(x, x3, xP, k, neg_pm1);
    return mulmod_m(x3, x4, x3 * pinv, k, neg_pm1);
}

struct ConstsF64 {
    double ext[8][16];
    double in[13];
    double k3, k15, i4, i8, i16, i256;
    double neg_pm1, pinv;
};
constexpr uint32_t c_from_monty(uint32_t m) {
    uint32_t t = m * bb::MU;
    uint64_t u = (uint64_t)t * bb::P;
    uint32_t uh = (uint32_t)(u >> 32);
    return uh ? bb::P - uh : 0;
}
constexpr uint64_t c_powmod(uint64_t b, uint64_t e) { uint64_t r = 1; b %= bb::P; while (e) { if (e & 1) r = r * b % bb::P; b = b * b % bb::P; e >>= 1; } return r; }
constexpr ConstsF64 make_consts() {
    ConstsF64 c{};
    for (int r = 0; r < 4; r++)
        for (int i = 0; i < 16; i++) {
            c.ext[r][i] = (double)c_from_monty(P3_RC16_EXT_INIT_MONTY[r][i]);
            c.ext[4 + r][i] = (double)c_from_monty(P3_RC16_EXT_FINAL_MONTY[r][i]);
        }
    for (int r = 0; r < 13; r++) c.in[r] = (double)c_from_monty(P3_RC16_INTERNAL_MONTY[r]);
    c.k3 = 3.0; c.k15 = 15.0; c.i4 = 0.25; c.i8 = 0.125; c.i16 = 0.0625; c.i256 = 0.00390625;
    c.neg_pm1 = -2013265920.0; c.pinv = 1.0 / 2013265921.0;
    return c;
}
static __device__ __constant__ ConstsF64 d_c = make_consts();

__device__ __forceinline__ void mat4(double& a, double& b, double& c, double& d) {
    double t01 = a + b, t23 = c + d, t0123 = t01 + t23;
    double t01123 = t0123 + b, t01233 = t0123 + d;
    double nd = __fma_rn(a, 2.0, t01233), nb = __fma_rn(c, 2.0, t01123);
    double na = t01123 + t01, nc = t01233 + t23;
    a = na; b = nb; c = nc; d = nd;
}
__device__ __forceinline__ void external_linear(double (&s)[16]) {
#pragma unroll
    for (int i = 0; i < 16; i += 4) mat4(s[i], s[i + 1], s[i + 2], s[i + 3]);
    double t[4];
#pragma unroll
    for (int k = 0; k < 4; k++) t[k] = (s[k] + s[k + 4]) + (s[k + 8] + s[k + 12]);
#pragma unroll
    for (int i = 0; i < 16; i++) s[i] += t[i & 3];
}

__device__ __forceinline__ void internal_rounds(double (&s)[16], const MagicRegs& mk) {
    const double npm1 = d_c.neg_pm1, pinv = d_c.pinv;
    const double k3 = d_c.k3, k15 = d_c.k15, i4 = d_c.i4, i8 = d_c.i8, i16 = d_c.i16, i256 = d_c.i256;
    auto internal_round = [&](int r) {
        s[0] = sbox7(s[0] + d_c.in[r], mk, npm1, pinv);
        double tot = ((s[0] + s[1]) + (s[2] + s[3])) + ((s[4] + s[5]) + (s[6] + s[7])) +
                     (((s[8] + s[9]) + (s[10] + s[11])) + ((s[12] + s[13]) + (s[14] + s[15])));
        tot = reduce(tot);
        s[0] = __fma_rn(s[0], -2.0, tot);
        s[1] = tot + s[1];
        s[2] = __fma_rn(s[2], 2.0, tot);
        s[3] = add_scaled_pow2(tot, s[3], 0.5);
        s[4] = __fma_rn(s[4], k3, tot);
        s[5] = __fma_rn(s[5], 4.0, tot);
        s[6] = add_scaled_pow2(tot, s[6], -0.5);
        s[7] = __fma_rn(s[7], -k3, tot);
        s[8] = __fma_rn(s[8], -4.0, tot);
        s[9] = add_scaled_pow2(tot, s[9], i256);
        s[10] = add_scaled_pow2(tot, s[10], i4);
        s[11] = add_scaled_pow2(tot, s[11], i8);
        s[12] = __fma_rn(s[12], -k15, tot);
        s[13] = add_scaled_pow2(tot, s[13], -i256);
        s[14] = add_scaled_pow2(tot, s[14], -i16);
        s[15] = __fma_rn(s[15], k15, tot);
    };
    auto fold_integer_lanes = [&]() {
        s[1] = reduce(s[1]); s[2] = reduce(s[2]); s[4] = reduce(s[4]); s[5] = reduce(s[5]);
        s[7] = reduce(s[7]); s[8] = reduce(s[8]); s[12] = reduce(s[12]); s[15] = reduce(s[15]);
    };
    _Pragma("clang loop unroll(disable)")
    for (int blk = 0; blk < 3; blk++) {
        _Pragma("clang loop unroll(disable)")
        for (int r = 0; r < 4; r++) internal_round(4 * blk + r);
        fold_integer_lanes();
    }
    internal_round(12);
    fold_integer_lanes();
}

__device__ __forceinline__ void permute(double (&s)[16]) {
    const MagicRegs mk = magic_regs();
    const double npm1 = d_c.neg_pm1, pinv = d_c.pinv;
    external_linear(s);
    _Pragma("clang loop unroll(disable)")
    for (int r = 0; r < 4; r++) {
#pragma unroll
        for (int i = 0; i < 16; i++) s[i] = sbox7(s[i] + d_c.ext[r][i], mk, npm1, pinv);
        external_linear(s);
    }
    internal_rounds(s, mk);
    _Pragma("clang loop unroll(disable)")
    for (int r = 4; r < 8; r++) {
#pragma unroll
        for (int i = 0; i < 16; i++) s[i] = sbox7(s[i] + d_c.ext[r][i], mk, npm1, pinv);
        external_linear(s);
    }
}

__device__ __forceinline__ double load_elem(uint32_t monty) { return (double)bb::from_monty(monty); }
constexpr double R_MOD_P = 268435454.0;
constexpr double R_MOD_P_OVER_P = 268435454.0 / 2013265921.0;
__device__ __forceinline__ uint32_t store_elem(double v, const MagicRegs& k) {
    const double r = mulmod_m(R_MOD_P, v, R_MOD_P_OVER_P, k, d_c.neg_pm1);
    const uint32_t w = (uint32_t)(int32_t)r;
    return min(w, w + bb::P);
}
__device__ __forceinline__ uint32_t store_elem(double v) { return store_elem(v, magic_regs()); }

}
```

### plonky3-mobile_amd/csrc/prover.hip

```cpp
#include <chrono>
#include <cstddef>
#include <deque>
#include <memory>
#include <cstring>

#include "bb31.hip.h"
#include "challenger.h"
#include "common.h"
#include "keccak.hip.h"
#include "mmcs.h"
#include "poseidon2.hip.h"
#include "poseidon2_f64.hip.h"
#include "prover.h"
#include "rng.h"
#include "rng_dev.hip.h"
#include "transcript.hip.h"

namespace p3 {

using bb::Ext;

__device__ __forceinline__ uint32_t tl(const TwoLevelTable& t, uint32_t e) {
    return bb::mul(t.lo[e & ((1u << t.T) - 1u)], t.hi[e >> t.T]);
}
__device__ __forceinline__ uint32_t brev(uint32_t v, uint32_t bits) { return bits ? (__brev(v) >> (32 - bits)) : 0u; }

__device__ __forceinline__ Ext ld_ext(const uint32_t* p) {
    uint4 v = *reinterpret_cast<const uint4*>(p);
    return Ext{{v.x, v.y, v.z, v.w}};
}
__device__ __forceinline__ void st_ext(uint32_t* p, const Ext& e) {
    *reinterpret_cast<uint4*>(p) = make_uint4(e.c[0], e.c[1], e.c[2], e.c[3]);
}

constexpr int SEL_CHUNK = 8;
__global__ void selectors_kernel(TwoLevelTable roots, uint32_t n, uint32_t gen, uint32_t ginv, uint32_t zh, uint2* sel) {
    uint32_t t = blockIdx.x * blockDim.x + threadIdx.x;
    uint32_t i0 = t * SEL_CHUNK;
    if (i0 >= n) return;
    uint32_t v[2 * SEL_CHUNK], pre[2 * SEL_CHUNK];
    uint32_t acc = bb::ONE;
#pragma unroll
    for (int k = 0; k < SEL_CHUNK; k++) {
        uint32_t x = bb::mul(gen, tl(roots, (i0 + k) & (n - 1)));
        v[2 * k] = bb::sub(x, bb::ONE);
        v[2 * k + 1] = bb::sub(x, ginv);
    }
#pragma unroll
    for (int k = 0; k < 2 * SEL_CHUNK; k++) { pre[k] = acc; acc = bb::mul(acc, v[k]); }
    uint32_t inv = bb::mul(bb::inv(acc), zh);
#pragma unroll
    for (int k = 2 * SEL_CHUNK - 1; k >= 0; k--) {
        uint32_t r = bb::mul(inv, pre[k]);
        inv = bb::mul(inv, v[k]);
        v[k] = r;
    }
#pragma unroll
    for (int k = 0; k < SEL_CHUNK; k++)
        if (i0 + k < n) sel[i0 + k] = make_uint2(v[2 * k], v[2 * k + 1]);
}

struct QuotArgs {
    const uint2* lde;
    const uint2* sel;
    uint32_t* out;
    const DevState* ds;
    TwoLevelTable roots;
    uint32_t n, log_n, gen, ginv, zh_inv;
};
__global__ void __launch_bounds__(256) fib_quotient_kernel(QuotArgs a) {
    uint32_t i = blockIdx.x * blockDim.x + threadIdx.x;
    if (i >= a.n) return;
    const DevState* __restrict__ ds = a.ds;
    uint2 loc = a.lde[brev(i, a.log_n)];
    uint2 nxt = a.lde[brev((i + 1) & (a.n - 1), a.log_n)];
    uint2 s = a.sel[i];
    uint32_t x = bb::mul(a.gen, tl(a.roots, i));
    uint32_t trans = bb::sub(x, a.ginv);
    uint32_t c0 = bb::mul(s.x, bb::sub(loc.x, ds->pis[0]));
    uint32_t c1 = bb::mul(s.x, bb::sub(loc.y, ds->pis[1]));
    uint32_t c2 = bb::mul(trans, bb::sub(loc.y, nxt.x));
    uint32_t c3 = bb::mul(trans, bb::sub(bb::add(loc.x, loc.y), nxt.y));
    uint32_t c4 = bb::mul(s.y, bb::sub(loc.y, ds->pis[2]));
    Ext acc;
#pragma unroll
    for (int k = 0; k < 4; k++)
        acc.c[k] = bb::add(bb::add(bb::dot2(ds->apow[4].c[k], c0, ds->apow[3].c[k], c1), bb::dot2(ds->apow[2].c[k], c2, ds->apow[1].c[k], c3)),
                           bb::mul(ds->apow[0].c[k], c4));
    st_ext(a.out + 4 * (size_t)i, bb::scale(acc, a.zh_inv));
}

constexpr int DEN_CHUNK = 4;
__global__ void __launch_bounds__(256) inv_denoms_kernel(TwoLevelTable roots, uint32_t big, uint32_t log_big, uint32_t gen,
                                                         const DevState* __restrict__ ds, uint32_t* d0, uint32_t* d1) {
    const DenConsts k0 = ds->k0, k1 = ds->k1;
    uint32_t t = blockIdx.x * blockDim.x + threadIdx.x;
    uint32_t j0 = t * DEN_CHUNK;
    if (j0 >= big) return;
    uint32_t a0[2 * DEN_CHUNK], e0[2 * DEN_CHUNK], e1[2 * DEN_CHUNK], nrm[2 * DEN_CHUNK], pre[2 * DEN_CHUNK];
#pragma unroll
    for (int k = 0; k < DEN_CHUNK; k++) {
        uint32_t x = bb::mul(gen, tl(roots, brev((j0 + k) & (big - 1), log_big)));
#pragma unroll
        for (int z = 0; z < 2; z++) {
            const DenConsts& c = z ? k1 : k0;
            const uint32_t a = bb::sub(c.z0, x);
            const uint32_t dd0 = bb::add(bb::sqr(a), c.k0), dd1 = bb::sub(bb::mul(c.k1, a), c.c1);
            a0[2 * k + z] = a; e0[2 * k + z] = dd0; e1[2 * k + z] = dd1;
            nrm[2 * k + z] = bb::sub(bb::sqr(dd0), bb::mul(bb::W_MONTY, bb::sqr(dd1)));
        }
    }
    uint32_t acc = bb::ONE;
#pragma unroll
    for (int k = 0; k < 2 * DEN_CHUNK; k++) { pre[k] = acc; acc = bb::mul(acc, nrm[k]); }
    uint32_t inv = bb::inv(acc);
#pragma unroll
    for (int k = 2 * DEN_CHUNK - 1; k >= 0; k--) {
        const uint32_t r = bb::mul(inv, pre[k]);
        inv = bb::mul(inv, nrm[k]);
        nrm[k] = r;
    }
#pragma unroll
    for (int k = 0; k < DEN_CHUNK; k++) {
        if (j0 + k >= big) break;
#pragma unroll
        for (int z = 0; z < 2; z++) {
            const DenConsts& c = z ? k1 : k0;
            const uint32_t i = 2 * k + z;
            const uint32_t f0 = bb::mul(e0[i], nrm[i]), f1 = bb::neg(bb::mul(e1[i], nrm[i]));
            Ext r;
            r.c[0] = bb::add(bb::mul(a0[i], f0), bb::mul(c.z2w, f1));
            r.c[2] = bb::add(bb::mul(a0[i], f1), bb::mul(c.z2, f0));
            r.c[1] = bb::neg(bb::add(bb::mul(c.z1, f0), bb::mul(c.z3w, f1)));
            r.c[3] = bb::neg(bb::add(bb::mul(c.z1, f1), bb::mul(c.z3, f0)));
            st_ext((z ? d1 : d0) + 4 * (size_t)(j0 + k), r);
        }
    }
}

constexpr int BARY_BLOCK = 256;
__global__ void __launch_bounds__(BARY_BLOCK) barycentric_kernel(TwoLevelTable roots, uint32_t n, uint32_t log_big,
                                                                 uint32_t gen, const uint2* lde_t, const uint4* lde_q,
                                                                 const uint32_t* d0, const uint32_t* d1,
                                                                 uint32_t* partials) {
    Ext acc[8];
#pragma unroll
    for (int k = 0; k < 8; k++) acc[k] = bb::ext_zero();
    const uint32_t step = gridDim.x * blockDim.x;
    for (uint32_t j = blockIdx.x * blockDim.x + threadIdx.x; j < n; j += 2 * step) {
        const bool two = j + step < n;
        const uint32_t j2 = two ? j + step : j;
        const uint32_t xa = bb::mul(gen, tl(roots, brev(j, log_big))), xb = two ? bb::mul(gen, tl(roots, brev(j2, log_big))) : 0u;
        const Ext e0a = bb::scale(ld_ext(d0 + 4 * (size_t)j), xa), e1a = bb::scale(ld_ext(d1 + 4 * (size_t)j), xa);
        const Ext e0b = bb::scale(ld_ext(d0 + 4 * (size_t)j2), xb), e1b = bb::scale(ld_ext(d1 + 4 * (size_t)j2), xb);
        const uint2 ta = lde_t[j], tb = lde_t[j2];
        const uint4 qa = lde_q[j], qb = lde_q[j2];
        auto fma2 = [](Ext& s, const Ext& ea, uint32_t va, const Ext& eb, uint32_t vb) {
#pragma unroll
            for (int c = 0; c < 4; c++) s.c[c] = bb::add(s.c[c], bb::dot2(ea.c[c], va, eb.c[c], vb));
        };
        fma2(acc[0], e0a, ta.x, e0b, tb.x);
        fma2(acc[1], e0a, ta.y, e0b, tb.y);
        fma2(acc[2], e1a, ta.x, e1b, tb.x);
        fma2(acc[3], e1a, ta.y, e1b, tb.y);
        fma2(acc[4], e0a, qa.x, e0b, qb.x);
        fma2(acc[5], e0a, qa.y, e0b, qb.y);
        fma2(acc[6], e0a, qa.z, e0b, qb.z);
        fma2(acc[7], e0a, qa.w, e0b, qb.w);
    }
    __shared__ uint32_t red[BARY_BLOCK / 64][32];
    const uint32_t lane = threadIdx.x & 63, wave = threadIdx.x >> 6;
#pragma unroll
    for (int k = 0; k < 8; k++)
#pragma unroll
        for (int c = 0; c < 4; c++) {
            uint32_t v = acc[k].c[c];
#pragma unroll
            for (int off = 32; off > 0; off >>= 1) v = bb::add(v, (uint32_t)__shfl_down((int)v, off, 64));
            if (lane == 0) red[wave][4 * k + c] = v;
        }
    __syncthreads();
    if (threadIdx.x < 32) {
        uint32_t v = 0;
#pragma unroll
        for (int w = 0; w < BARY_BLOCK / 64; w++) v = bb::add(v, red[w][threadIdx.x]);
        partials[blockIdx.x * 32 + threadIdx.x] = v;
    }
}

struct ReducedArgs {
    const uint2* lde_t;
    const uint4* lde_q;
    const uint32_t* d0;
    const uint32_t* d1;
    uint32_t* ro;
    const DevState* ds;
    uint32_t big;
};
__global__ void __launch_bounds__(256) reduced_openings_kernel(ReducedArgs a) {
    uint32_t j = blockIdx.x * blockDim.x + threadIdx.x;
    if (j >= a.big) return;
    const DevState* __restrict__ ds = a.ds;
    uint2 t = a.lde_t[j];
    uint4 q = a.lde_q[j];
    Ext u, w;
#pragma unroll
    for (int c = 0; c < 4; c++) {
        u.c[c] = bb::add(bb::add(bb::dot2(ds->alp[4].c[c], q.x, ds->alp[5].c[c], q.y), bb::dot2(ds->alp[6].c[c], q.z, ds->alp[7].c[c], q.w)),
                         bb::mul(ds->alp[1].c[c], t.y));
        w.c[c] = bb::dot2(ds->alp[2].c[c], t.x, ds->alp[3].c[c], t.y);
    }
    u.c[0] = bb::add(u.c[0], t.x);
    Ext e0 = ld_ext(a.d0 + 4 * (size_t)j), e1 = ld_ext(a.d1 + 4 * (size_t)j);
    Ext r = bb::add(bb::mul(bb::sub(ds->y02, u), e0), bb::mul(bb::sub(ds->y1, w), e1));
    st_ext(a.ro + 4 * (size_t)j, r);
}

__global__ void __launch_bounds__(256) fri_fold_kernel(TwoLevelTable inv_roots , const uint32_t* in,
                                                       uint32_t* out, uint32_t half, uint32_t log_half,
                                                       const DevState* __restrict__ ds, uint32_t round, uint32_t one_half) {
    if (gridDim.x <= 512u) P3_LATENCY_BOUND_KERNEL();
    uint32_t i = blockIdx.x * blockDim.x + threadIdx.x;
    if (i >= half) return;
    const Ext half_beta = ds->half_beta[round];
    Ext lo = ld_ext(in + 8 * (size_t)i), hi = ld_ext(in + 8 * (size_t)i + 4);
    uint32_t p = tl(inv_roots, brev(i, log_half));
    Ext s = bb::scale(bb::add(lo, hi), one_half);
    Ext d = bb::mul(bb::scale(half_beta, p), bb::sub(lo, hi));
    st_ext(out + 4 * (size_t)i, bb::add(s, d));
}

__global__ void __launch_bounds__(256) grind_kernel(DevState* ds, uint32_t mask, uint32_t base) {
    uint32_t w = base + blockIdx.x * blockDim.x + threadIdx.x;
    if (w >= bb::P) return;
    if (base + blockIdx.x * blockDim.x > *(volatile uint32_t*)&ds->grind_result) return;
    const uint32_t pos = ds->n_in;
    double s[16];
#pragma unroll
    for (int i = 0; i < 16; i++) s[i] = p2f::load_elem((i < 8 && (uint32_t)i < pos) ? ds->inb[i & 7] : ds->st[i]);
#pragma unroll
    for (int i = 0; i < 8; i++) s[i] = (i == (int)pos) ? (double)w : s[i];
    p2f::permute(s);
    if ((bb::from_monty(p2f::store_elem(s[7])) & mask) == 0) atomicMin(&ds->grind_result, w);
}

__global__ void __launch_bounds__(256) grind_keccak_kernel(DevState* ds, uint32_t mask, uint32_t base) {
    uint32_t w = base + blockIdx.x * blockDim.x + threadIdx.x;
    if (w >= bb::P) return;
    if (base + blockIdx.x * blockDim.x > *(volatile uint32_t*)&ds->grind_result) return;
    const KeccakGrindArgs& a = ds->kgrind;
    const uint32_t wm = bb::to_monty(w);
    uint64_t st[25];
#pragma unroll
    for (int i = 0; i < 25; i++) st[i] = a.state[i];
    for (uint32_t blk = 0; blk < a.n_blocks; blk++) {
#pragma unroll
        for (int i = 0; i < 17; i++) {
            uint64_t lane = a.block[blk][i];
            const int32_t rel = (int32_t)(a.wpos) - (int32_t)(blk * 136 + i * 8);
            if (rel > -4 && rel < 8) {
                const uint64_t v = (uint64_t)wm;
                lane ^= rel >= 0 ? (v << (8 * rel)) : (v >> (8 * -rel));
            }
            st[i] ^= lane;
        }
        if (blk + 1 == a.n_blocks) kk::permute_digest(st);
        else kk::permute(st);
    }
    bool ok = false;
#pragma unroll
    for (int t = 0; t < 8; t++) {
        const uint64_t lane = st[3 - t / 2];
        const uint32_t hi_or_lo = (t & 1) ? (uint32_t)lane : (uint32_t)(lane >> 32);
        const uint32_t v = __builtin_bswap32(hi_or_lo) & 0x7fffffffu;
        if (v < bb::P) { ok = (v & mask) == 0; break; }
    }
    if (ok) atomicMin(&ds->grind_result, w);
}

constexpr uint32_t QTREE_MAX_MATS = 8;
struct QTree {
    const uint32_t* mat[QTREE_MAX_MATS];
    uint32_t width[QTREE_MAX_MATS];
    uint32_t stride[QTREE_MAX_MATS];
    uint32_t n_mats;
    const uint32_t* layers;
    uint32_t log_height, shift, slot_off;
};
__global__ void query_gather_kernel(const QTree* trees, const uint32_t* indices, uint32_t slot_words, uint32_t* out) {
    P3_LATENCY_BOUND_KERNEL();
    const QTree& t = trees[blockIdx.y];
    const uint64_t index = (indices[blockIdx.x] >> t.shift) & ((1ull << t.log_height) - 1ull);
    uint32_t* dst = out + (size_t)blockIdx.x * slot_words + t.slot_off;
    uint32_t off = 0;
    for (uint32_t m = 0; m < t.n_mats; m++) {
        for (uint32_t c = threadIdx.x; c < t.width[m]; c += blockDim.x) dst[off + c] = t.mat[m][index * t.stride[m] + c];
        off += t.width[m];
    }
    uint64_t base = 0, len = 1ull << t.log_height;
    for (uint32_t i = 0; i < t.log_height; i++) {
        const uint64_t sib = (index >> i) ^ 1;
        if (threadIdx.x < 8) dst[off + i * 8 + threadIdx.x] = t.layers[base + sib * 8 + threadIdx.x];
        base += len * 8;
        len >>= 1;
    }
}

struct StageLayout {
    uint32_t root_t = 0, root_q = 8, opened = 16, froots = 48, fpoly = 0, witness = 0, status = 0, qidx = 0, slots = 0, words = 0;
};
struct TsArgs {
    DevState* ds;
    uint32_t* ps;
    int kind;
    StageLayout lay;
};
struct TsPis {
    uint32_t w[3];
    uint32_t given;
};

__global__ void __launch_bounds__(64) ts_begin_kernel(TsArgs a, const uint32_t* trace, uint32_t n, uint32_t log_n, TsPis given) {
    P3_LATENCY_BOUND_KERNEL();
    __shared__ KState ks;
    DevChal ch;
    ch.begin(a.kind, a.ds, &ks, true);
    uint32_t pis[3];
    if (given.given) {
        for (int k = 0; k < 3; k++) pis[k] = given.w[k];
    } else {
        pis[0] = trace[0]; pis[1] = trace[1]; pis[2] = trace[2 * (size_t)(n - 1) + 1];
    }
    ch.observe(bb::to_monty(log_n));
    ch.observe(bb::to_monty(log_n));
    ch.observe_n(a.ps + a.lay.root_t, 8);
    ch.observe_n(pis, 3);
    const Ext alpha = ch.sample_ext();
    Ext ap[5];
    ap[0] = bb::ext_one();
#pragma unroll
    for (int k = 1; k < 5; k++) ap[k] = bb::mul(ap[k - 1], alpha);
    if (threadIdx.x == 0) {
        for (int k = 0; k < 3; k++) a.ds->pis[k] = pis[k];
        for (int k = 0; k < 5; k++) a.ds->apow[k] = ap[k];
        a.ds->status = 0;
        a.ps[a.lay.status] = 0;
    }
    ch.end();
}
__global__ void __launch_bounds__(64) ts_zeta_kernel(TsArgs a, uint32_t g_n) {
    P3_LATENCY_BOUND_KERNEL();
    __shared__ KState ks;
    DevChal ch;
    ch.begin(a.kind, a.ds, &ks, false);
    ch.observe_n(a.ps + a.lay.root_q, 8);
    const Ext zeta = ch.sample_ext();
    const Ext zeta_next = bb::scale(zeta, g_n);
    if (threadIdx.x == 0) {
        a.ds->zeta = zeta;
        a.ds->zeta_next = zeta_next;
        a.ds->k0 = den_consts(zeta);
        a.ds->k1 = den_consts(zeta_next);
    }
    ch.end();
}
constexpr int TS_OPEN_THREADS = 256;
__global__ void __launch_bounds__(TS_OPEN_THREADS) ts_open_kernel(TsArgs a, const uint32_t* partials, uint32_t n_blocks,
                                                                  uint32_t log_n, uint32_t sn, uint32_t denom) {
    P3_LATENCY_BOUND_KERNEL();
    __shared__ KState ks;
    __shared__ uint32_t red[TS_OPEN_THREADS / 32][32];
    __shared__ uint32_t tot[32];
    {
        const uint32_t col = threadIdx.x & 31u, part = threadIdx.x >> 5;
        uint32_t v = 0;
        constexpr uint32_t STEP = TS_OPEN_THREADS / 32;
        uint32_t b = part;
        for (; b + 3 * STEP < n_blocks; b += 4 * STEP) {
            const uint32_t p0 = partials[b * 32 + col], p1 = partials[(b + STEP) * 32 + col],
                           p2 = partials[(b + 2 * STEP) * 32 + col], p3 = partials[(b + 3 * STEP) * 32 + col];
            v = bb::add(bb::add(v, bb::add(p0, p1)), bb::add(p2, p3));
        }
        for (; b < n_blocks; b += STEP) v = bb::add(v, partials[b * 32 + col]);
        red[part][col] = v;
    }
    __syncthreads();
    if (threadIdx.x < 32) {
        uint32_t v = 0;
#pragma unroll
        for (int p = 0; p < TS_OPEN_THREADS / 32; p++) v = bb::add(v, red[p][threadIdx.x]);
        tot[threadIdx.x] = v;
    }
    __syncthreads();
    if (threadIdx.x >= 64) return;
    DevChal ch;
    ch.begin(a.kind, a.ds, &ks, false);
    Ext opened[8];
#pragma unroll
    for (int k = 0; k < 8; k++)
#pragma unroll
        for (int c = 0; c < 4; c++) opened[k].c[c] = tot[4 * k + c];
    {
        Ext z0 = a.ds->zeta, z1 = a.ds->zeta_next;
        for (uint32_t i = 0; i < log_n; i++) { z0 = bb::sqr(z0); z1 = bb::sqr(z1); }
        const Ext f0 = bb::scale(bb::sub(z0, bb::ext_from_base(sn)), denom);
        const Ext f1 = bb::scale(bb::sub(z1, bb::ext_from_base(sn)), denom);
#pragma unroll
        for (int k = 0; k < 8; k++) opened[k] = bb::mul(opened[k], (k == 2 || k == 3) ? f1 : f0);
    }
#pragma unroll
    for (int k = 0; k < 8; k++) ch.observe_ext(opened[k]);
    const Ext al = ch.sample_ext();
    Ext alp[8];
    alp[0] = bb::ext_one();
#pragma unroll
    for (int k = 1; k < 8; k++) alp[k] = bb::mul(alp[k - 1], al);
    const Ext ry0 = bb::add(opened[0], bb::mul(alp[1], opened[1]));
    const Ext ry1 = bb::add(opened[2], bb::mul(alp[1], opened[3]));
    const Ext ry2 = bb::add(bb::add(opened[4], bb::mul(alp[1], opened[5])),
                            bb::add(bb::mul(alp[2], opened[6]), bb::mul(alp[3], opened[7])));
    if (threadIdx.x == 0) {
        for (int k = 0; k < 8; k++) {
            a.ds->alp[k] = alp[k];
            for (int c = 0; c < 4; c++) a.ps[a.lay.opened + 4 * k + c] = opened[k].c[c];
        }
        a.ds->y02 = bb::add(ry0, bb::mul(alp[4], ry2));
        a.ds->y1 = bb::mul(alp[2], ry1);
    }
    ch.end();
}
// ... 148 lines not shown
    memcpy(b.data() + o, w, 4 * n);
}
static void put_opening(std::vector<uint8_t>& pf, const uint32_t*& slot, uint32_t n, const uint32_t* widths, uint32_t salt_words,
                        uint32_t depth) {
    put_u32(pf, n);
    for (uint32_t m = 0; m < n; m++) { put_u32(pf, widths[m]); put_words(pf, slot, widths[m]); slot += widths[m]; }
    if (salt_words)
        for (uint32_t m = 0; m < n; m++) { put_u32(pf, salt_words); put_words(pf, slot, salt_words); slot += salt_words; }
    put_u32(pf, depth); put_words(pf, slot, (size_t)depth * 8); slot += (size_t)depth * 8;
}

static uint32_t grind_first_log() {
    const char* e = getenv("P3HIP_GRIND_FIRST_LOG");
    return e ? (uint32_t)atoi(e) : 0u;
}

struct ProverCore {
    int hash = HASH_POSEIDON2, profile = PROFILE_LATENCY;
    int device = -1;
    hipStream_t stream = nullptr;
    bool own_stream = false;
    FriParams fp{};
    uint32_t log_big = 0, n_rounds = 0, salt_words = 0;
    std::vector<void*> allocs;
    uint32_t *fri_vec = nullptr, *fri_layers = nullptr, *fri_salts = nullptr, *fp_ev = nullptr;
    std::vector<size_t> fri_vec_off, fri_layer_off, fri_salt_off;
    size_t fri_vec_words = 0, fri_layer_words = 0, fri_salt_words = 0;
    std::vector<QTree> trees;
    QTree* qtrees = nullptr;
    uint32_t *pstage = nullptr, *qidx = nullptr;
    StageLayout lay;
    size_t slot_words = 0;

    ~ProverCore() {
        for (void* p : allocs) (void)hipFree(p);
        if (own_stream && stream) (void)hipStreamDestroy(stream);
    }
    int alloc(uint32_t** p, size_t words) {
        P3_HIP(hipMalloc(reinterpret_cast<void**>(p), words * 4 + 64));
        allocs.push_back(*p);
        return OK;
    }
    static int bad_arg(const char* who, const char* what) { return fail(ERR_BAD_ARG, std::string(who) + ": " + what); }

    int begin(const char* who, hipStream_t st, bool own, int hash_kind, int prof) {
        stream = st; own_stream = own;
        if (prof != PROFILE_THROUGHPUT && prof != PROFILE_LATENCY) return bad_arg(who, "unknown profile");
        if (hash_kind != HASH_POSEIDON2 && hash_kind != HASH_KECCAK) return bad_arg(who, "unknown hash configuration");
        hash = hash_kind; profile = prof;
        P3_HIP(hipGetDevice(&device));
        return OK;
    }
    int set_fri(const char* who, const FriParams& p, uint32_t log_height) {
        if (p.log_final_poly_len >= log_height) return bad_arg(who, "log_final_poly_len must be below the committed trace's log height");
        if (p.proof_of_work_bits > 30) return bad_arg(who, "proof_of_work_bits too large");
        fp = p; log_big = log_height + p.log_blowup; n_rounds = log_height - p.log_final_poly_len;
        if (n_rounds > MAX_FRI_ROUNDS) return bad_arg(who, "too many FRI rounds");
        return OK;
    }
    int alloc_fri() {
        const size_t big = (size_t)1 << log_big;
        for (uint32_t r = 0; r <= n_rounds; r++) { fri_vec_off.push_back(fri_vec_words); fri_vec_words += (big >> r) * 4; }
        for (uint32_t r = 0; r < n_rounds; r++) {
            fri_layer_off.push_back(fri_layer_words); fri_layer_words += mmcs_layer_words(big >> (r + 1));
            fri_salt_off.push_back(fri_salt_words); fri_salt_words += (big >> (r + 1)) * salt_words;
        }
        int rc;
        if ((rc = alloc(&fri_vec, fri_vec_words))) return rc;
        if ((rc = alloc(&fri_layers, fri_layer_words + 8))) return rc;
        if (salt_words && (rc = alloc(&fri_salts, fri_salt_words + 8))) return rc;
        return alloc(&fp_ev, ((size_t)4) << fp.log_final_poly_len);
    }
    int layout(const char* who, uint32_t extra_words) {
        for (uint32_t r = 0; r < n_rounds; r++) {
            const uint32_t w = salt_words;
            trees.push_back(QTree{{fri_vec + fri_vec_off[r], w ? fri_salts + fri_salt_off[r] : nullptr}, {8, w}, {8, w}, w ? 2u : 1u,
                                  fri_layers + fri_layer_off[r], log_big - 1 - r, r + 1});
        }
        slot_words = 0;
        for (QTree& t : trees) {
            t.slot_off = (uint32_t)slot_words;
            for (uint32_t m = 0; m < t.n_mats; m++) slot_words += t.width[m];
            slot_words += (size_t)t.log_height * 8;
        }
        const uint32_t nq = fp.num_queries;
        StageLayout& L = lay;
        L.fpoly = L.froots + 8 * n_rounds;
        L.witness = L.fpoly + (4u << fp.log_final_poly_len);
        L.status = L.witness + 1;
        L.qidx = L.status + 1;
        L.slots = (L.qidx + nq + 3u) & ~3u;
        const size_t stage_words = (size_t)L.slots + slot_words * nq;
        if (stage_words > 0xffffffffull) return bad_arg(who, "proof staging buffer too large");
        L.words = (uint32_t)stage_words;
        int rc;
        if ((rc = alloc(&pstage, stage_words + extra_words))) return rc;
        if ((rc = alloc(&qidx, std::max<uint32_t>(nq, 1)))) return rc;
        uint32_t* p = nullptr;
        if ((rc = alloc(&p, (sizeof(QTree) + 3) / 4 * trees.size()))) return rc;
        qtrees = reinterpret_cast<QTree*>(p);
        P3_HIP(hipMemcpy(qtrees, trees.data(), trees.size() * sizeof(QTree), hipMemcpyHostToDevice));
        return OK;
    }

    int commit(size_t n, const uint32_t* const* mats, const size_t* widths, uint32_t* const* salts, size_t height, uint32_t* layers,
               uint32_t root_slot, size_t mat_stride = 0, hipStream_t on = nullptr) {
        hipStream_t cs = on ? on : stream;
        const uint32_t* mp[QTREE_MAX_MATS]; size_t hh[QTREE_MAX_MATS], ww[QTREE_MAX_MATS], ss[QTREE_MAX_MATS];
        size_t k = 0;
        for (size_t i = 0; i < n; i++, k++) {
            mp[k] = mats[i]; hh[k] = height; ww[k] = widths[i]; ss[k] = mat_stride ? mat_stride : widths[i];
            if (salt_words) { k++; mp[k] = salts[i]; hh[k] = height; ww[k] = ss[k] = salt_words; }
        }
        Tree* tp = nullptr;
        int r = mmcs_commit(cs, mp, hh, ww, k, &tp, layers, pstage + root_slot, hash, ss, profile);
        if (r) return r;
        std::unique_ptr<Tree> t(tp);
        if (!t->root_copied) P3_HIP(hipMemcpyAsync(pstage + root_slot, t->layers + t->layer_off.back(), 32, hipMemcpyDeviceToDevice, cs));
        return OK;
    }
    int fri_rounds(Context& cx, const TsArgs& ts, uint32_t r_end) {
        const uint32_t one_half = bb::inv(bb::to_monty(2));
        const size_t row = 8;
        int rc;
        for (uint32_t r = 0; r < r_end; r++) {
            const uint32_t log_half = log_big - 1 - r, half = 1u << log_half;
            uint32_t* vec = fri_vec + fri_vec_off[r];
            uint32_t* salts = salt_words ? fri_salts + fri_salt_off[r] : nullptr;
            if ((rc = commit(1, &vec, &row, &salts, half, fri_layers + fri_layer_off[r], lay.froots + 8 * r))) return rc;
            hipLaunchKernelGGL(ts_fri_round_kernel, dim3(1), dim3(64), 0, stream, ts, r, one_half);
            P3_HIP(hipGetLastError());
            TwoLevelTable inv_roots;
            if ((rc = cx.get_root_table(stream, log_half + 1, true, &inv_roots))) return rc;
            hipLaunchKernelGGL(fri_fold_kernel, dim3((half + 255) / 256), dim3(256), 0, stream, inv_roots, vec, fri_vec + fri_vec_off[r + 1],
                               half, log_half, ts.ds, r, one_half);
            P3_HIP(hipGetLastError());
        }
        return OK;
    }
    int fri_final(Context& cx, const TsArgs& ts) {
        const uint32_t fpl = 1u << fp.log_final_poly_len;
        int rc;
        if ((rc = bit_reverse_rows(stream, fri_vec + fri_vec_off[n_rounds], fp_ev, fpl, 4))) return rc;
        if ((rc = ntt_dft(cx, stream, fp_ev, pstage + lay.fpoly, fpl, 4, true))) return rc;
        hipLaunchKernelGGL(ts_final_kernel, dim3(1), dim3(64), 0, stream, ts, fpl, pow_mask());
        P3_HIP(hipGetLastError());
        return OK;
    }

    uint32_t pow_mask() const { return (1u << fp.proof_of_work_bits) - 1u; }
    uint32_t grind_range(uint32_t first_log) const {
        return 1u << std::min<uint32_t>(std::max<uint32_t>(first_log ? first_log : fp.proof_of_work_bits + 4, 8), 24);
    }
    int grind(const TsArgs& ts, uint64_t base, uint32_t count) {
        if (hash == HASH_KECCAK) hipLaunchKernelGGL(grind_keccak_kernel, dim3(count / 256), dim3(256), 0, stream, ts.ds, pow_mask(), (uint32_t)base);
        else hipLaunchKernelGGL(grind_kernel, dim3(count / 256), dim3(256), 0, stream, ts.ds, pow_mask(), (uint32_t)base);
        P3_HIP(hipGetLastError());
        return OK;
    }
    int grind_start(const TsArgs& ts) {
        const uint32_t first_log = grind_first_log(), batch = grind_range(first_log);
        const uint32_t head = first_log ? batch : std::min<uint32_t>(batch, 1u << std::max<uint32_t>(fp.proof_of_work_bits + 1, 8));
        int rc;
        if ((rc = grind(ts, 0, head))) return rc;
        if (batch > head && (rc = grind(ts, head, batch - head))) return rc;
        return OK;
    }
    int queries(const TsArgs& ts, uint32_t* host, size_t words) {
        const uint32_t nq = fp.num_queries;
        hipLaunchKernelGGL(ts_queries_kernel, dim3(1), dim3(64), 0, stream, ts, nq, log_big, fp.proof_of_work_bits, qidx);
        P3_HIP(hipGetLastError());
        if (nq) {
            hipLaunchKernelGGL(query_gather_kernel, dim3(nq, (uint32_t)trees.size()), dim3(64), 0, stream, qtrees, qidx, (uint32_t)slot_words,
                               pstage + lay.slots);
            P3_HIP(hipGetLastError());
        }
        P3_HIP(hipMemcpyAsync(host, pstage, words * 4, hipMemcpyDeviceToHost, stream));
        return OK;
    }
    int continue_grind(const TsArgs& ts, uint32_t* host, size_t words) {
        uint32_t batch = grind_range(grind_first_log()), found = 0xffffffffu;
        int rc;
        for (uint64_t base = batch; base < bb::P && found == 0xffffffffu; base += batch) {
            batch = std::min<uint32_t>(batch * 4, 1u << 24);
            if ((rc = grind(ts, base, batch))) return rc;
            P3_HIP(hipMemcpyAsync(&found, &ts.ds->grind_result, 4, hipMemcpyDeviceToHost, stream));
            P3_HIP(hipStreamSynchronize(stream));
        }
        if (found == 0xffffffffu) return fail(ERR_INTERNAL, "grind: no proof-of-work witness found");
        if ((rc = queries(ts, host, words))) return rc;
        P3_HIP(hipStreamSynchronize(stream));
        return OK;
    }

    void put_fri(std::vector<uint8_t>& pf, const uint32_t* hp) const {
        const StageLayout& L = lay;
        const uint32_t nq = fp.num_queries, fpl = 1u << fp.log_final_poly_len, n_inputs = (uint32_t)trees.size() - n_rounds;
        put_u32(pf, n_rounds); put_words(pf, hp + L.froots, (size_t)n_rounds * 8);
        put_u32(pf, nq);
        for (uint32_t q = 0; q < nq; q++) {
            const uint32_t* slot = hp + L.slots + (size_t)q * slot_words;
            put_u32(pf, n_inputs);
            for (uint32_t i = 0; i < n_inputs; i++) {
                const QTree& t = trees[i];
                put_opening(pf, slot, salt_words ? t.n_mats / 2 : t.n_mats, t.width, salt_words, t.log_height);
            }
            put_u32(pf, n_rounds);
            for (uint32_t r = 0; r < n_rounds; r++) {
                const uint32_t lh = log_big - 1 - r, idx = hp[L.qidx + q] >> r;
                put_words(pf, slot + 4 * ((idx ^ 1) & 1), 4);
                if (salt_words) { put_u32(pf, salt_words); put_words(pf, slot + 8, salt_words); }
                put_u32(pf, lh); put_words(pf, slot + 8 + salt_words, (size_t)lh * 8);
                slot += 8 + salt_words + (size_t)lh * 8;
            }
        }
        put_u32(pf, fpl);
        put_words(pf, hp + L.fpoly, (size_t)fpl * 4);
        put_u32(pf, hp[L.witness]);
    }
};

constexpr int N_STAGE_EVENTS = 7;

struct FibProver::Impl : ProverCore {
    uint32_t log_n = 0;
    uint32_t *trace = nullptr, *lde_t = nullptr, *qflat = nullptr, *lde_q = nullptr, *d0 = nullptr, *d1 = nullptr;
    uint32_t *layers_t = nullptr, *layers_q = nullptr, *partials = nullptr;
    DevState* ds = nullptr;
    uint32_t* host_stage[2] = {nullptr, nullptr};
    hipEvent_t done[2] = {nullptr, nullptr};
    struct Pending {
        uint64_t a, b; int slot; std::chrono::steady_clock::time_point t_start, t_enq; uint64_t seq;
        const uint32_t* trace;
        TsPis pis;
    };
    std::deque<Pending> pending;
    uint64_t next_seq = 1, arena_owner = 0;
    hipEvent_t ev[2][N_STAGE_EVENTS] = {{nullptr}, {nullptr}};
    uint32_t bary_blocks = 0;
    StageTimes times{};
    uint64_t grind_misses = 0;
    std::vector<uint32_t> miss_qidx;
    ~Impl() {
        for (auto* h : host_stage) if (h) (void)hipHostFree(h);
        for (auto& set : ev) for (auto& e : set) if (e) (void)hipEventDestroy(e);
        for (auto& e : done) if (e) (void)hipEventDestroy(e);
    }
};

FibProver::FibProver() : im(new Impl()) {}
FibProver::~FibProver() { delete im; }

int FibProver::init(uint32_t log_n, const FriParams& fp, hipStream_t stream, bool own_stream, int hash, int profile) {
    Impl& s = *im;
    int rc;
    if ((rc = s.begin("fib prover", stream, own_stream, hash, profile))) return rc;
    if (log_n < 1) return fail(ERR_BAD_ARG, "fib prover: log_n must be >= 1");
    if (log_n + fp.log_blowup > MAX_LOG_DOMAIN)
        return fail(ERR_BAD_ARG, "fib prover: LDE domain above 2^" + std::to_string(MAX_LOG_DOMAIN) + " points (log_n + log_blowup)");
    if (fp.log_blowup < 1) return fail(ERR_BAD_ARG, "fib prover: log_blowup must be >= 1");
    if ((rc = s.set_fri("fib prover", fp, log_n))) return rc;
    s.log_n = log_n;
    const size_t n = (size_t)1 << log_n, big = (size_t)1 << s.log_big;
    if ((rc = s.alloc(&s.trace, n * 2))) return rc;
    if ((rc = s.alloc(&s.lde_t, big * 2))) return rc;
    if ((rc = s.alloc(&s.qflat, n * 4))) return rc;
    if ((rc = s.alloc(&s.lde_q, big * 4))) return rc;
    if ((rc = s.alloc(&s.d0, big * 4))) return rc;
    if ((rc = s.alloc(&s.d1, big * 4))) return rc;
    if ((rc = s.alloc(&s.layers_t, mmcs_layer_words(big)))) return rc;
    if ((rc = s.alloc(&s.layers_q, mmcs_layer_words(big)))) return rc;
    if ((rc = s.alloc_fri())) return rc;
    s.bary_blocks = (uint32_t)std::min<size_t>(256, (n + BARY_BLOCK - 1) / BARY_BLOCK);
    if ((rc = s.alloc(&s.partials, (size_t)s.bary_blocks * 32))) return rc;
    {
        uint32_t* p = nullptr;
        if ((rc = s.alloc(&p, (sizeof(DevState) + 3) / 4))) return rc;
        s.ds = reinterpret_cast<DevState*>(p);
        P3_HIP(hipMemset(s.ds, 0, sizeof(DevState)));
    }
    s.trees.push_back(QTree{{s.lde_t}, {2}, {2}, 1, s.layers_t, s.log_big});
    s.trees.push_back(QTree{{s.lde_q}, {4}, {4}, 1, s.layers_q, s.log_big});
    if ((rc = s.layout("fib prover", 0))) return rc;
    for (auto& h : s.host_stage) P3_HIP(hipHostMalloc(reinterpret_cast<void**>(&h), (size_t)s.lay.words * 4 + 64));
    for (auto& set : s.ev) for (auto& e : set) P3_HIP(hipEventCreate(&e));
    for (auto& e : s.done) P3_HIP(hipEventCreateWithFlags(&e, hipEventDisableTiming));
    return OK;
}

static int get_selectors(Context& cx, hipStream_t stream, uint32_t log_n, const uint2** out) {
    auto it = cx.selector_tables.find(log_n);
    if (it == cx.selector_tables.end()) {
        const uint32_t n = 1u << log_n;
        CachedTable e;
        P3_HIP(hipMalloc(reinterpret_cast<void**>(&e.t.lo), (size_t)n * 8));
        TwoLevelTable roots;
        int rc = cx.get_root_table(stream, log_n, false, &roots);
        if (rc) { (void)hipFree(e.t.lo); return rc; }
        uint32_t gen = bb::to_monty(bb::GEN);
        uint32_t g = bb::two_adic_generator(log_n), ginv = bb::inv(g);
        uint32_t zh = bb::sub(bb::pow(gen, n), bb::ONE);
        uint32_t threads = (n + SEL_CHUNK - 1) / SEL_CHUNK;
        hipLaunchKernelGGL(selectors_kernel, dim3((threads + 255) / 256), dim3(256), 0, stream, roots, n, gen, ginv, zh,
                           reinterpret_cast<uint2*>(e.t.lo));
        P3_HIP(hipGetLastError());
        if ((rc = cx.mark_built(stream, e))) return rc;
        it = cx.selector_tables.emplace(log_n, e).first;
    }
    int rc = cx.wait_ready(stream, it->second);
    if (rc) return rc;
    *out = reinterpret_cast<const uint2*>(it->second.t.lo);
    return OK;
}

int FibProver::prove(uint64_t a, uint64_t b, std::vector<uint8_t>* proof) {
    if (!im->pending.empty()) return fail(ERR_BAD_ARG, "fib prover: finish the enqueued proofs before a synchronous prove");
    int rc = enqueue(a, b);
    if (rc) return rc;
    return finish(proof);
}
int FibProver::enqueue(uint64_t a, uint64_t b) { return enqueue_any(a, b, nullptr, nullptr); }
int FibProver::enqueue_trace(const uint32_t* d_trace, const uint32_t pis[3]) {
    if (!d_trace || !pis) return fail(ERR_BAD_ARG, "fib prover: null trace or public values");
    return enqueue_any(0, 0, d_trace, pis);
}
int FibProver::prove_trace(const uint32_t* d_trace, const uint32_t pis[3], std::vector<uint8_t>* proof) {
    if (!im->pending.empty()) return fail(ERR_BAD_ARG, "fib prover: finish the enqueued proofs before a synchronous prove");
    int rc = enqueue_trace(d_trace, pis);
    if (rc) return rc;
    return finish(proof);
}
uint32_t* FibProver::arena_trace() const { return im->trace; }
bool FibProver::has_pending() const { return !im->pending.empty(); }
hipStream_t FibProver::stream() const { return im->stream; }
uint32_t FibProver::log_n() const { return im->log_n; }
int FibProver::device() const { return im->device; }
int FibProver::enqueue_any(uint64_t a, uint64_t b, const uint32_t* d_trace, const uint32_t* pis) {
    Impl& s = *im;
    if (s.pending.size() >= 2) return fail(ERR_BAD_ARG, "fib prover: two proofs already in flight (finish one first)");
    const int slot = s.pending.empty() ? 0 : 1 - s.pending.back().slot;
    Impl::Pending p{a, b, slot, std::chrono::steady_clock::now(), {}, s.next_seq++, d_trace, TsPis{{0, 0, 0}, 0}};
    if (pis) p.pis = TsPis{{pis[0], pis[1], pis[2]}, 1};
    int rc = run(a, b, slot, 0, nullptr, &p);
    if (rc) return rc;
    s.pending.push_back(p);
    return OK;
}
int FibProver::finish(std::vector<uint8_t>* proof) {
    Impl& s = *im;
    if (s.pending.empty()) return fail(ERR_BAD_ARG, "fib prover: no proof in flight");
    Impl::Pending p = s.pending.front();
    int rc = run(p.a, p.b, p.slot, 1, proof, &p);
    s.pending.pop_front();
    return rc;
}
int FibProver::run(uint64_t a, uint64_t b, int slot, int phase, std::vector<uint8_t>* proof, void* pending_rec) {
    Impl& s = *im;
    Impl::Pending& pend = *static_cast<Impl::Pending*>(pending_rec);
    hipEvent_t* const ev = s.ev[slot];
    Context* cxp;
    int rc = get_context(&cxp);
    if (rc) return rc;
    Context& cx = *cxp;
    if (cx.device != s.device)
        return fail(ERR_BAD_ARG, "fib prover: created on device " + std::to_string(s.device) + ", current device is " + std::to_string(cx.device));
    hipStream_t st = s.stream;
    const uint32_t log_n = s.log_n, log_big = s.log_big;
    const uint32_t n = 1u << log_n, big = 1u << log_big;
    const uint32_t gen = bb::to_monty(bb::GEN);
    const uint32_t g_n = bb::two_adic_generator(log_n), g_n_inv = bb::inv(g_n);
    const StageLayout& L = s.lay;
    const TsArgs ts{s.ds, s.pstage, s.hash, L};
    const size_t w_trace = 2, w_quot = 4;
    const uint32_t nq = s.fp.num_queries;
    auto body = [&]() -> int {
        s.arena_owner = pend.seq;
        P3_HIP(hipEventRecord(ev[0], st));

        const uint32_t* trace = pend.trace ? pend.trace : s.trace;
        if (!pend.trace && (rc = fib_trace(st, a, b, n, s.trace))) return rc;
        if ((rc = ntt_coset_lde(cx, st, trace, s.lde_t, n, 2, s.fp.log_blowup, gen, true))) return rc;
        if ((rc = s.commit(1, &s.lde_t, &w_trace, nullptr, big, s.layers_t, L.root_t))) return rc;
        hipLaunchKernelGGL(ts_begin_kernel, dim3(1), dim3(64), 0, st, ts, trace, n, log_n, pend.pis);
        P3_HIP(hipGetLastError());
        P3_HIP(hipEventRecord(ev[1], st));

        const uint2* sel = nullptr;
        if ((rc = get_selectors(cx, st, log_n, &sel))) return rc;
        {
            QuotArgs qa{};
            qa.lde = reinterpret_cast<const uint2*>(s.lde_t);
            qa.sel = sel;
            qa.out = s.qflat;
            qa.ds = s.ds;
            if ((rc = cx.get_root_table(st, log_n, false, &qa.roots))) return rc;
            qa.n = n; qa.log_n = log_n; qa.gen = gen; qa.ginv = g_n_inv;
            qa.zh_inv = bb::inv(bb::sub(bb::pow(gen, n), bb::ONE));
            hipLaunchKernelGGL(fib_quotient_kernel, dim3((n + 255) / 256), dim3(256), 0, st, qa);
            P3_HIP(hipGetLastError());
        }
        if ((rc = ntt_coset_lde(cx, st, s.qflat, s.lde_q, n, 4, s.fp.log_blowup, bb::ONE, true))) return rc;
        if ((rc = s.commit(1, &s.lde_q, &w_quot, nullptr, big, s.layers_q, L.root_q))) return rc;
        hipLaunchKernelGGL(ts_zeta_kernel, dim3(1), dim3(64), 0, st, ts, g_n);
        P3_HIP(hipGetLastError());
        P3_HIP(hipEventRecord(ev[2], st));

        TwoLevelTable roots_big;
        if ((rc = cx.get_root_table(st, log_big, false, &roots_big))) return rc;
        {
            uint32_t threads = (big + DEN_CHUNK - 1) / DEN_CHUNK;
            hipLaunchKernelGGL(inv_denoms_kernel, dim3((threads + 255) / 256), dim3(256), 0, st, roots_big, big, log_big, gen,
                               s.ds, s.d0, s.d1);
            P3_HIP(hipGetLastError());
            hipLaunchKernelGGL(barycentric_kernel, dim3(s.bary_blocks), dim3(BARY_BLOCK), 0, st, roots_big, n, log_big, gen,
                               reinterpret_cast<const uint2*>(s.lde_t), reinterpret_cast<const uint4*>(s.lde_q), s.d0, s.d1,
                               s.partials);
            P3_HIP(hipGetLastError());
            const uint32_t sn = bb::pow(gen, n);
            const uint32_t denom = bb::inv(bb::mul(bb::to_monty(n), sn));
            hipLaunchKernelGGL(ts_open_kernel, dim3(1), dim3(TS_OPEN_THREADS), 0, st, ts, s.partials, s.bary_blocks, log_n, sn, denom);
            P3_HIP(hipGetLastError());
        }
        P3_HIP(hipEventRecord(ev[3], st));

        {
            ReducedArgs ra{};
            ra.lde_t = reinterpret_cast<const uint2*>(s.lde_t);
            ra.lde_q = reinterpret_cast<const uint4*>(s.lde_q);
            ra.d0 = s.d0; ra.d1 = s.d1; ra.ro = s.fri_vec + s.fri_vec_off[0]; ra.big = big;
            ra.ds = s.ds;
            hipLaunchKernelGGL(reduced_openings_kernel, dim3((big + 255) / 256), dim3(256), 0, st, ra);
            P3_HIP(hipGetLastError());
        }

        uint32_t r_tail = s.n_rounds;
        if (s.profile == PROFILE_LATENCY && s.hash == HASH_POSEIDON2)
            while (r_tail > 0 && (big >> (r_tail - 1)) <= (1u << FRI_TAIL_MAX_LOG)) r_tail--;
        if ((rc = s.fri_rounds(cx, ts, r_tail))) return rc;
        if (r_tail < s.n_rounds) {
            FriTailArgs ta{};
            ta.ts = ts; ta.vec = s.fri_vec; ta.layers = s.fri_layers;
            ta.r0 = r_tail; ta.n_tail = s.n_rounds - r_tail; ta.log_len0 = log_big - r_tail; ta.one_half = bb::inv(bb::to_monty(2));
            for (uint32_t k = 0; k <= ta.n_tail; k++) {
                if (s.fri_vec_off[r_tail + k] > 0xffffffffull) return fail(ERR_INTERNAL, "fri tail: vector offset out of range");
                ta.vec_off[k] = (uint32_t)s.fri_vec_off[r_tail + k];
            }
            for (uint32_t k = 0; k < ta.n_tail; k++) {
                if (s.fri_layer_off[r_tail + k] > 0xffffffffull) return fail(ERR_INTERNAL, "fri tail: layer offset out of range");
                ta.layer_off[k] = (uint32_t)s.fri_layer_off[r_tail + k];
                if ((rc = cx.get_root_table(st, ta.log_len0 - k, true, &ta.inv_roots[k]))) return rc;
            }
            hipLaunchKernelGGL(fri_tail_kernel, dim3(1), dim3(1024), 0, st, ta);
            P3_HIP(hipGetLastError());
        }
        if ((rc = s.fri_final(cx, ts))) return rc;
        P3_HIP(hipEventRecord(ev[4], st));

        if ((rc = s.grind_start(ts))) return rc;
        P3_HIP(hipEventRecord(ev[5], st));

        if ((rc = s.queries(ts, s.host_stage[slot], L.words))) return rc;
        P3_HIP(hipEventRecord(ev[6], st));
        return OK;
    };
    if (phase == 0) {
        if ((rc = body())) return rc;
        P3_HIP(hipEventRecord(s.done[slot], st));
        pend.t_enq = std::chrono::steady_clock::now();
        return OK;
    }
    const auto t_start = pend.t_start, t_enq = pend.t_enq;
    P3_HIP(hipEventSynchronize(s.done[slot]));
    const uint32_t* hp = s.host_stage[slot];
    static const bool trace = getenv("P3HIP_TRACE") != nullptr;
#define TR(...) do { if (trace) { fprintf(stderr, __VA_ARGS__); fflush(stderr); } } while (0)
    TR("prove: enqueued in %.0f us of host time, synced after another %.0f us, status %u\n",
       std::chrono::duration<double, std::micro>(t_enq - t_start).count(),
       std::chrono::duration<double, std::micro>(std::chrono::steady_clock::now() - t_enq).count(), hp[L.status]);
    if (hp[L.status] == ST_GRIND_MISS) {
        if (s.arena_owner != pend.seq) {
            P3_HIP(hipStreamSynchronize(st));
            if ((rc = body())) return rc;
            P3_HIP(hipStreamSynchronize(st));
        }
        s.grind_misses++;
        s.miss_qidx.assign(nq, 0xdeadbeefu);
        if (nq) P3_HIP(hipMemcpyAsync(s.miss_qidx.data(), s.qidx, (size_t)nq * 4, hipMemcpyDeviceToHost, st));
        P3_HIP(hipStreamSynchronize(st));
        TR("prove: first proof-of-work range empty, continuing the search\n");
        if ((rc = s.continue_grind(ts, s.host_stage[slot], L.words))) return rc;
        TR("prove: witness %u, queries redone, status %u\n", hp[L.witness], hp[L.status]);
    }
    if (hp[L.status] != 0) return fail(ERR_INTERNAL, "grind: witness rejected by the device transcript");

    std::vector<uint8_t>& pf = *proof;
    pf.clear();
    pf.reserve(64 + (size_t)nq * s.slot_words * 4 + 4096);
    put_u32(pf, 0x42463350u); put_u32(pf, 1); put_u32(pf, log_n);
    put_words(pf, hp + L.root_t, 8); put_words(pf, hp + L.root_q, 8);
    const uint32_t* op = hp + L.opened;
    put_u32(pf, 2); put_words(pf, op, 8);
    put_u32(pf, 2); put_words(pf, op + 8, 8);
    put_u32(pf, 1); put_u32(pf, 4); put_words(pf, op + 16, 16);
    s.put_fri(pf, hp);
    TR("prove: serialised %zu bytes\n", pf.size());
    float ms[N_STAGE_EVENTS - 1] = {0};
    for (int k = 0; k + 1 < N_STAGE_EVENTS; k++) (void)hipEventElapsedTime(&ms[k], ev[k], ev[k + 1]);
    s.times.trace_commit_ms += ms[0]; s.times.quotient_commit_ms += ms[1]; s.times.open_ms += ms[2];
    s.times.fri_commit_ms += ms[3]; s.times.grind_ms += ms[4]; s.times.query_ms += ms[5]; s.times.proofs += 1;
    return OK;
}

const StageTimes& FibProver::times() const { return im->times; }
void FibProver::reset_times() { im->times = StageTimes{}; }
uint64_t FibProver::grind_misses(std::vector<uint32_t>* last_indices) const {
    if (last_indices) *last_indices = im->miss_qidx;
    return im->grind_misses;
}

}

#include "prover_hiding.hip.inc"
#include "pcs.hip.inc"
```

### plonky3-mobile_amd/csrc/prover_hiding.hip.inc

```

namespace p3 {

constexpr uint32_t HW = 2, HNRC = 4, HSALT = 4, HD = 4, HTW = HW + HNRC, HRW = HNRC + HD, HCH = 4;
constexpr uint32_t HOPEN = HRW + 2 * HTW + HCH * HD;
constexpr uint32_t HQS = HCH * HD;

struct DevStateH {
    DevState base;
    Ext alp[HOPEN];
    Ext y0, y1;
    uint32_t err;
};

__global__ void randomize_trace_kernel(const uint2* trace, const uint32_t* rnd, uint32_t h, uint32_t* out) {
    uint32_t i = blockIdx.x * blockDim.x + threadIdx.x;
    if (i >= h) return;
    const uint2 t = trace[i];
    const uint32_t* d = rnd + (size_t)i * (HW + 2 * HNRC);
    uint32_t* even = out + (size_t)(2 * i) * HTW;
    even[0] = t.x; even[1] = t.y;
#pragma unroll
    for (uint32_t k = 0; k < HNRC; k++) even[HW + k] = d[k];
#pragma unroll
    for (uint32_t k = 0; k < HTW; k++) even[HTW + k] = d[HNRC + k];
// ... 447 lines not shown
    return prove_any(0, 0, d_trace, pis, proof);
}
uint32_t* FibHidingProver::arena_trace() const { return im->trace; }
hipStream_t FibHidingProver::stream() const { return im->stream; }
uint32_t FibHidingProver::log_n() const { return im->log_n; }
int FibHidingProver::device() const { return im->device; }
int FibHidingProver::prove_any(uint64_t a, uint64_t b, const uint32_t* d_trace, const uint32_t* pis, std::vector<uint8_t>* proof) {
    Impl& s = *im;
    const TsPis given = pis ? TsPis{{pis[0], pis[1], pis[2]}, 1} : TsPis{{0, 0, 0}, 0};
    Context* cxp;
    int rc = get_context(&cxp);
    if (rc) return rc;
    Context& cx = *cxp;
    if (cx.device != s.device) return fail(ERR_BAD_ARG, "hiding prover: created on another device");
    hipStream_t st = s.stream;
    const uint32_t log_n = s.log_n, log_ext = s.log_ext, log_big = s.log_big;
    const uint32_t h = 1u << log_n, h2 = 2 * h, big = 1u << log_big, log_q = log_n + 2;
    const uint32_t gen = bb::to_monty(bb::GEN);
    const uint32_t g_h = bb::two_adic_generator(log_n);
    const StageLayout& L = s.lay;
    DevState* ds = &s.hs->base;
    const TsArgs ts{ds, s.pstage, s.hash, L};
    DevRng *rng_mmcs = s.rngs, *rng_fri = s.rngs + 1, *rng_pcs = s.rngs + 2;
    uint32_t* err = s.pstage + L.words;
    const uint32_t nq = s.fp.num_queries;
    const uint32_t* const hp = s.host_stage;
    if (s.tiny) {
        TinyArgs ta{};
        ta.hash = (uint32_t)s.hash; ta.log_n = log_n; ta.log_blowup = s.fp.log_blowup; ta.log_fpl = s.fp.log_final_poly_len;
        ta.nq = nq; ta.pow_bits = s.fp.proof_of_work_bits;
        ta.a_monty = bb::to_monty((uint32_t)(a % bb::P)); ta.b_monty = bb::to_monty((uint32_t)(b % bb::P));
        rng_seed_from_u64(ta.seed, s.seed);
        if ((rc = rng_jump_table(cx, &ta.jump))) return rc;
        ta.n_pcs = (uint32_t)s.pcs_words; ta.n_mmcs = (uint32_t)s.mmcs_words; ta.n_fri = (uint32_t)s.fri_salt_words;
        const bool short_chunks = rng_tiny_chunks(s.pcs_words) && rng_tiny_chunks(s.mmcs_words) && (!s.fri_salt_words || rng_tiny_chunks(s.fri_salt_words));
        ta.chunk_log = short_chunks ? RNG_TINY_CHUNK_LOG : RNG_CHUNK_LOG;
        if (short_chunks) {
            ta.jump += (size_t)RNG_MAX_JUMP * 256 * 4;
            ta.ch_pcs = rng_tiny_chunks(s.pcs_words); ta.ch_mmcs = rng_tiny_chunks(s.mmcs_words);
            ta.ch_fri = s.fri_salt_words ? rng_tiny_chunks(s.fri_salt_words) : 0;
        } else {
            ta.ch_pcs = rng_small_chunks(s.pcs_words); ta.ch_mmcs = rng_small_chunks(s.mmcs_words);
            ta.ch_fri = s.fri_salt_words ? rng_small_chunks(s.fri_salt_words) : 0;
        }
        ta.pcs_draws = s.pcs_draws; ta.mmcs_draws = s.mmcs_draws; ta.fri_salts = s.fri_salts;
        ta.trace = s.trace; ta.in_trace = d_trace; ta.pis = given; ta.rt = s.rt; ta.lde_t = s.lde_t; ta.salt_t = s.salt_t; ta.layers_t = s.layers_t;
        ta.qchunks = s.qchunks; ta.co = s.co; ta.ext = s.ext; ta.lde_qb = s.lde_qb; ta.layers_q = s.layers_q; ta.t012 = s.t012;
        for (uint32_t c = 0; c < HCH; c++) ta.salt_q[c] = s.salt_q[c];
        ta.rm = s.rm; ta.lde_r = s.lde_r; ta.salt_r = s.salt_r; ta.layers_r = s.layers_r;
        ta.d0 = s.d0; ta.d1 = s.d1; ta.fri_vec = s.fri_vec; ta.fri_layers = s.fri_layers; ta.fp_ev = s.fp_ev;
        ta.n_rounds = s.n_rounds;
        for (uint32_t r = 0; r <= s.n_rounds; r++) ta.fri_vec_off[r] = (uint32_t)s.fri_vec_off[r];
        for (uint32_t r = 0; r < s.n_rounds; r++) { ta.fri_salt_off[r] = (uint32_t)s.fri_salt_off[r]; ta.fri_layer_off[r] = (uint32_t)s.fri_layer_off[r]; }
        ta.hs = s.hs; ta.pstage = s.pstage; ta.lay = L; ta.root_r_off = s.root_r_off; ta.slot_words = (uint32_t)s.slot_words;
        ta.qtrees = s.qtrees; ta.n_trees = (uint32_t)s.trees.size(); ta.qidx = s.qidx; ta.err = err;
        const size_t lds = (size_t)3 * RNG_SMALL_CHUNKS * RNG_SMALL_STRIDE * 4 + 4096;
        if ((rc = cx.ensure_dynamic_lds(reinterpret_cast<const void*>(tiny_hiding_prover_kernel), (int)lds))) return rc;
        hipLaunchKernelGGL(tiny_hiding_prover_kernel, dim3(1), dim3(TINY_THREADS), lds, st, ta);
        P3_HIP(hipGetLastError());
        P3_HIP(hipMemcpyAsync(s.host_stage, s.pstage, ((size_t)L.words + 1) * 4, hipMemcpyDeviceToHost, st));
        P3_HIP(hipStreamSynchronize(st));
    } else {
        if (s.side) P3_HIP(hipStreamWaitEvent(st, s.ev_fri, 0));
        if (s.side2) P3_HIP(hipStreamWaitEvent(st, s.ev_r, 0));
        if ((rc = rng_seed(st, s.rngs, s.seed, 3, err))) return rc;
        auto fill = [&](DevRng* r, uint32_t* out, uint64_t n) {
            return s.one_fill ? OK : rng_fill_field(cx, st, r, out, n, s.rng_ws, err);
        };
        if (s.one_fill) {
            hipStream_t fs = s.side ? s.side : st;
            if (s.side) { P3_HIP(hipEventRecord(s.ev_start, st)); P3_HIP(hipStreamWaitEvent(s.side, s.ev_start, 0)); }
            if ((rc = rng_fill_field(cx, fs, rng_pcs, s.pcs_draws, s.pcs_words, s.rng_ws, err))) return rc;
            if (s.side) P3_HIP(hipEventRecord(s.ev_pcs, s.side));
            if ((rc = rng_fill_field(cx, fs, rng_mmcs, s.mmcs_draws, s.mmcs_words, s.rng_ws, err))) return rc;
            if (s.side) P3_HIP(hipEventRecord(s.ev_mmcs, s.side));
            if ((rc = rng_fill_field(cx, fs, rng_fri, s.fri_salts, s.fri_salt_words, s.rng_ws, err))) return rc;
            if (s.side) P3_HIP(hipEventRecord(s.ev_fri, s.side));
        }
        auto wait_fill = [&](hipEvent_t e) -> int { if (s.side) P3_HIP(hipStreamWaitEvent(st, e, 0)); return OK; };
        const size_t w_r = HRW, w_t = HTW, w_q[HCH] = {HD, HD, HD, HD};
        auto commit_random = [&](hipStream_t on) -> int {
            int r = ntt_coset_lde(cx, on, s.rm, s.lde_r, h2, HRW, s.fp.log_blowup, gen, true);
            if (r) return r;
            return s.commit(1, &s.lde_r, &w_r, &s.salt_r, big, s.layers_r, s.root_r_off, 0, on);
        };
        if (s.side2) {
            P3_HIP(hipStreamWaitEvent(s.side2, s.ev_start, 0));
            P3_HIP(hipStreamWaitEvent(s.side2, s.ev_pcs, 0));
            P3_HIP(hipStreamWaitEvent(s.side2, s.ev_mmcs, 0));
            if ((rc = commit_random(s.side2))) return rc;
            P3_HIP(hipEventRecord(s.ev_r, s.side2));
        }

        const uint32_t* trace = d_trace ? d_trace : s.trace;
        if (!d_trace && (rc = fib_trace(st, a, b, h, s.trace))) return rc;
        if ((rc = fill(rng_pcs, s.rnd_t, (uint64_t)h * (HW + 2 * HNRC)))) return rc;
        if ((rc = wait_fill(s.ev_pcs))) return rc;
        hipLaunchKernelGGL(randomize_trace_kernel, dim3((h + 255) / 256), dim3(256), 0, st, reinterpret_cast<const uint2*>(trace), s.rnd_t, h, s.rt);
        P3_HIP(hipGetLastError());
        if ((rc = ntt_coset_lde(cx, st, s.rt, s.lde_t, h2, HTW, s.fp.log_blowup, gen, true))) return rc;
        if ((rc = fill(rng_mmcs, s.salt_t, (uint64_t)big * HSALT))) return rc;
        if ((rc = wait_fill(s.ev_mmcs))) return rc;
        if ((rc = s.commit(1, &s.lde_t, &w_t, &s.salt_t, big, s.layers_t, L.root_t))) return rc;
        hipLaunchKernelGGL(ts_begin_h_kernel, dim3(1), dim3(64), 0, st, ts, trace, h, log_n, given);
        P3_HIP(hipGetLastError());

        {
            QuotHArgs qa{};
            qa.lde = s.lde_t; qa.chunks = s.qchunks; qa.ds = ds; qa.sel_fl = s.sel_fl; qa.sel_tr = s.sel_tr;
            qa.h = h; qa.log_h = log_n;
            const uint32_t gh = bb::pow(gen, h), w4 = bb::two_adic_generator(2);
            uint32_t p = bb::ONE;
            for (int c = 0; c < 4; c++) { qa.zh_inv[c] = bb::inv(bb::sub(bb::mul(gh, p), bb::ONE)); p = bb::mul(p, w4); }
            hipLaunchKernelGGL(fib_quotient_h_kernel, dim3((h + 255) / 256), dim3(256), 0, st, qa);
            P3_HIP(hipGetLastError());
        }
        if ((rc = fill(rng_pcs, s.t012, (uint64_t)(HCH - 1) * h * HD))) return rc;
        if ((rc = ntt_dft(cx, st, s.qchunks, s.co, h, HQS, true))) return rc;
        {
            BlindArgs ba{};
            ba.co = s.co; ba.t012 = s.t012; ba.ext = s.ext; ba.h = h;
            const uint32_t gh = bb::pow(gen, h), w4 = bb::two_adic_generator(2), g4 = bb::two_adic_generator(log_q);
            uint32_t sh[HCH], kc[HCH], p = bb::ONE;
            for (uint32_t c = 0; c < HCH; c++) { sh[c] = bb::mul(gh, p); p = bb::mul(p, w4); }
            if ((rc = cx.reserve_scale_slots(HCH))) return rc;
            for (uint32_t c = 0; c < HCH; c++) {
                uint32_t k = bb::ONE;
                for (uint32_t j = 0; j < HCH; j++) if (j != c) k = bb::mul(k, bb::sub(sh[c], sh[j]));
                kc[c] = k;
                ba.sh[c] = sh[c]; ba.kinv[c] = bb::inv(k);
                if ((rc = cx.get_scale_table(st, bb::inv(bb::mul(gen, bb::pow(g4, c))), log_n, bb::ONE, &ba.sp[c]))) return rc;
            }
            ba.k_last = kc[HCH - 1];
            hipLaunchKernelGGL(blind_chunks_kernel, dim3((h + 255) / 256), dim3(256), 0, st, ba);
            P3_HIP(hipGetLastError());
        }
        if ((rc = ntt_coset_lde_from_coeffs(cx, st, s.ext, s.lde_qb, s.ev2, h2, HQS, s.fp.log_blowup, gen))) return rc;
        for (uint32_t c = 0; c < HCH; c++) if ((rc = fill(rng_mmcs, s.salt_q[c], (uint64_t)big * HSALT))) return rc;
        if ((rc = s.commit(HCH, s.lde_q, w_q, s.salt_q, big, s.layers_q, L.root_q, HQS))) return rc;

        if (s.side2) {
            P3_HIP(hipStreamWaitEvent(st, s.ev_r, 0));
        } else {
            if ((rc = fill(rng_pcs, s.rm, (uint64_t)h2 * HRW))) return rc;
            if ((rc = fill(rng_mmcs, s.salt_r, (uint64_t)big * HSALT))) return rc;
            if ((rc = commit_random(st))) return rc;
        }
        hipLaunchKernelGGL(ts_zeta_h_kernel, dim3(1), dim3(64), 0, st, ts, s.root_r_off, g_h);
        P3_HIP(hipGetLastError());

        TwoLevelTable roots_big;
        if ((rc = cx.get_root_table(st, log_big, false, &roots_big))) return rc;
        {
            uint32_t threads = (big + DEN_CHUNK - 1) / DEN_CHUNK;
            hipLaunchKernelGGL(inv_denoms_kernel, dim3((threads + 255) / 256), dim3(256), 0, st, roots_big, big, log_big, gen, ds, s.d0, s.d1);
            P3_HIP(hipGetLastError());
            const size_t ps = (size_t)s.bary_blocks * 32;
            {
                BaryAllArgs ba{};
                ba.roots = roots_big; ba.n2 = h2; ba.log_big = log_big; ba.gen = gen;
                ba.lde_r = s.lde_r; ba.lde_t = s.lde_t;
                for (uint32_t c = 0; c < HCH; c++) ba.lde_q[c] = s.lde_q[c];
                ba.d0 = s.d0; ba.d1 = s.d1; ba.partials = s.partials; ba.set_stride = (uint32_t)ps;
                hipLaunchKernelGGL(bary_all_kernel, dim3(s.bary_blocks), dim3(BARY_BLOCK), 0, st, ba);
                P3_HIP(hipGetLastError());
            }
            const uint32_t sn = bb::pow(gen, h2);
            const uint32_t denom = bb::inv(bb::mul(bb::to_monty(h2), sn));
            hipLaunchKernelGGL(ts_open_h_kernel, dim3(1), dim3(TS_OPEN_H_THREADS), 0, st, ts, s.hs, s.partials, s.bary_blocks, log_ext, sn, denom);
            P3_HIP(hipGetLastError());
        }
        {
            ReducedHArgs ra{};
            ra.lde_r = s.lde_r; ra.lde_t = s.lde_t;
            for (uint32_t c = 0; c < HCH; c++) ra.lde_q[c] = s.lde_q[c];
            ra.d0 = s.d0; ra.d1 = s.d1; ra.ro = s.fri_vec + s.fri_vec_off[0]; ra.hs = s.hs; ra.big = big;
            hipLaunchKernelGGL(reduced_openings_h_kernel, dim3((big + 255) / 256), dim3(256), 0, st, ra);
            P3_HIP(hipGetLastError());
        }

        if ((rc = wait_fill(s.ev_fri))) return rc;
        for (uint32_t r = 0; r < s.n_rounds; r++)
            if ((rc = fill(rng_fri, s.fri_salts + s.fri_salt_off[r], (uint64_t)(big >> (r + 1)) * HSALT))) return rc;
        if ((rc = s.fri_rounds(cx, ts, s.n_rounds))) return rc;
        if ((rc = s.fri_final(cx, ts))) return rc;
        if ((rc = s.grind_start(ts))) return rc;
        const size_t words = (size_t)L.words + 1;
        if ((rc = s.queries(ts, s.host_stage, words))) return rc;
        P3_HIP(hipStreamSynchronize(st));
        if (hp[L.status] == ST_GRIND_MISS && (rc = s.continue_grind(ts, s.host_stage, words))) return rc;
    }
    if (hp[L.status] != 0) return fail(ERR_INTERNAL, "grind: witness rejected by the device transcript");
    if (hp[L.words] != 0) return fail(ERR_INTERNAL, "rng: a random stream ran out of raw draws");

    std::vector<uint8_t>& pf = *proof;
    pf.clear();
    pf.reserve(64 + (size_t)nq * (s.slot_words + 64) * 4 + 4096);
    put_u32(pf, 0x42463350u); put_u32(pf, 2); put_u32(pf, log_n);
    put_words(pf, hp + L.root_t, 8); put_words(pf, hp + L.root_q, 8); put_words(pf, hp + s.root_r_off, 8);
    const uint32_t* op = hp + L.opened;
    put_u32(pf, HRW); put_words(pf, op, 4 * HRW); op += 4 * HRW;
    put_u32(pf, HTW); put_words(pf, op, 4 * HTW); op += 4 * HTW;
    put_u32(pf, HTW); put_words(pf, op, 4 * HTW); op += 4 * HTW;
    put_u32(pf, HCH);
    for (uint32_t c = 0; c < HCH; c++) { put_u32(pf, HD); put_words(pf, op, 4 * HD); op += 4 * HD; }
    s.put_fri(pf, hp);
    return OK;
}

}
```

Before: 527.0.

## Specialize Poseidon2 for sparse inputs, skip coset-0 LDE, share denominators, grid-stride grinding

Several independent changes. Poseidon2 leaf and compress hashing gets templated variants that simplify the first external linear layer when only 2, 4 or 8 input words are nonzero. The quotient kernel writes its output bit-reversed straight into the LDE buffer, so the coset LDE can skip coset 0. The inverse-denominator kernel computes only one set of denominators and derives the second by an index shift and a scale. Grinding becomes a grid-stride loop with a capped lane count in throughput mode. The aim is to cut redundant hashing, NTT and field-inversion work, at the cost of more kernel variants and index arithmetic whose correctness depends on subtle assumptions such as the shifted-zeta relation.

```diff
diff --git a/plonky3-mobile_amd/csrc/common.h b/plonky3-mobile_amd/csrc/common.h
--- a/plonky3-mobile_amd/csrc/common.h
+++ b/plonky3-mobile_amd/csrc/common.h
@@ -87,7 +87,7 @@
             uint32_t width, bool inverse);
 std::vector<uint32_t> ntt_dft_plan(uint32_t n);
 int ntt_coset_lde(Context& cx, hipStream_t stream, const uint32_t* src, uint32_t* dst, uint64_t height,
-                  uint32_t width, uint32_t added_bits, uint32_t shift_monty, bool bit_reversed_out);
+                  uint32_t width, uint32_t added_bits, uint32_t shift_monty, bool bit_reversed_out, bool coset0_in_place = false);
 int ntt_coset_lde_from_coeffs(Context& cx, hipStream_t stream, const uint32_t* coeffs, uint32_t* dst, uint32_t* scratch,
                               uint64_t height, uint32_t width, uint32_t added_bits, uint32_t shift_monty);
 int ntt_coset_dft(Context& cx, hipStream_t stream, const uint32_t* src, uint32_t* dst, uint64_t height,
diff --git a/plonky3-mobile_amd/csrc/mmcs.hip b/plonky3-mobile_amd/csrc/mmcs.hip
--- a/plonky3-mobile_amd/csrc/mmcs.hip
+++ b/plonky3-mobile_amd/csrc/mmcs.hip
@@ -116,6 +116,7 @@
 }
 
 
+template <int CLASS>
 __global__ void __launch_bounds__(256) leaf_hash_f64_kernel(const uint32_t* mat, uint32_t width, uint64_t n_rows, uint32_t* digests) {
     if (gridDim.x <= 512u) P3_LATENCY_BOUND_KERNEL();
     uint64_t r = (uint64_t)blockIdx.x * blockDim.x + threadIdx.x;
@@ -124,14 +125,21 @@
 #pragma unroll
     for (int i = 0; i < 16; i++) s[i] = 0.0;
     const uint32_t* row = mat + r * width;
-    for (uint32_t k = 0; k < width; k += 8) {
-#pragma unroll
-        for (int i = 0; i < 8; i++)
-            if (k + i < width) s[i] = p2f::load_elem(row[k + i]);
-        p2f::permute(s);
-        if (k + 8 < width) {
-#pragma unroll
-            for (int i = 0; i < 16; i++) s[i] = p2f::reduce(s[i]);
+    if constexpr (CLASS != 0) {
+#pragma unroll
+        for (int i = 0; i < CLASS; i++)
+            if ((uint32_t)i < width) s[i] = p2f::load_elem(row[i]);
+        p2f::permute<CLASS, true>(s);
+    } else {
+        for (uint32_t k = 0; k < width; k += 8) {
+#pragma unroll
+            for (int i = 0; i < 8; i++)
+                if (k + i < width) s[i] = p2f::load_elem(row[k + i]);
+            p2f::permute(s);
+            if (k + 8 < width) {
+#pragma unroll
+                for (int i = 0; i < 16; i++) s[i] = p2f::reduce(s[i]);
+            }
         }
     }
     uint32_t d[8];
@@ -268,7 +276,7 @@
     double s[16];
 #pragma unroll
     for (int k = 0; k < 16; k++) s[k] = p2f::load_elem(w[k]);
-    p2f::permute(s);
+    p2f::permute<16, true>(s);
     uint32_t d[8];
     const p2f::MagicRegs smk = p2f::magic_regs();
 #pragma unroll
@@ -812,8 +820,9 @@
             hipLaunchKernelGGL(leaf_hash_f64_wide_kernel, dim3((uint32_t)((maxh + 255) / 256)), dim3(256), 0, stream, rs.ptr[0],
                                rs.width[0], maxh, t->layers);
         } else if (dense1) {
-            hipLaunchKernelGGL(leaf_hash_f64_kernel, dim3((uint32_t)((maxh + 255) / 256)), dim3(256), 0, stream, rs.ptr[0],
-                               rs.width[0], maxh, t->layers);
+            const size_t w = rs.width[0];
+            auto kern = w == 0 || w > 8 ? leaf_hash_f64_kernel<0> : w <= 2 ? leaf_hash_f64_kernel<2> : w <= 4 ? leaf_hash_f64_kernel<4> : leaf_hash_f64_kernel<8>;
+            hipLaunchKernelGGL(kern, dim3((uint32_t)((maxh + 255) / 256)), dim3(256), 0, stream, rs.ptr[0], rs.width[0], maxh, t->layers);
         } else if ((maxh >= COOP_MAX || (rs.count == 1 && !dense1))) {
             hipLaunchKernelGGL(leaf_hash_f64_rowset_kernel, dim3((uint32_t)((maxh + 255) / 256)), dim3(256), 0, stream, rs, maxh, t->layers);
         } else {
diff --git a/plonky3-mobile_amd/csrc/ntt.hip b/plonky3-mobile_amd/csrc/ntt.hip
--- a/plonky3-mobile_amd/csrc/ntt.hip
+++ b/plonky3-mobile_amd/csrc/ntt.hip
@@ -824,7 +824,7 @@
 }
 
 int lde_narrow(Context& cx, hipStream_t stream, const uint32_t* src, uint32_t* dst, uint32_t n, uint32_t added, uint32_t W,
-               uint32_t shift, bool bit_reversed_out, bool from_coeffs = false) {
+               uint32_t shift, bool bit_reversed_out, bool from_coeffs = false, bool coset0_in_place = false) {
     if (!bit_reversed_out || added < 1 || added > 3) return 1;
     constexpr uint32_t w_max = 16;
     const bool wide = W > w_max && n >= 16 && n <= 18 && W >= 64 && (((uint64_t)W << (n + added + 2)) < (1ull << 32));
@@ -853,6 +853,7 @@
     }
     a.from_coeffs = from_coeffs;
     a.n = n; a.n1 = n1; a.n2 = n2; a.W = W; a.added = added;
+    a.cos_first = coset0_in_place && shift == bb::ONE && !from_coeffs && !wide && !a.blocked ? 1u : 0u;
     TwoLevelTable ti, tf;
     if ((rc = cx.get_root_table(stream, n, true, &ti))) return rc;
     if ((rc = cx.get_root_table(stream, n, false, &tf))) return rc;
@@ -895,15 +896,20 @@
     uint32_t split_log = 0;
     while (split_log < added && ((uint64_t)tiles << (split_log + 1)) <= 256) split_log++;
     a.cos_per_block = (1u << added) >> split_log;
-    if ((rc = wide ? launch_narrow_wide<2>(cx, stream, a, n2, tiles, 1u << split_log)
-                   : f64 ? launch_narrow64<2>(cx, stream, a, n2, tiles, vw[1], 1u << split_log)
-                         : launch_narrow<2>(cx, stream, a, n2, tiles, vw[1], 1u << split_log))) return rc;
+    const uint32_t cos_groups = ((1u << added) - a.cos_first + a.cos_per_block - 1) / a.cos_per_block;
+    if ((rc = wide ? launch_narrow_wide<2>(cx, stream, a, n2, tiles, cos_groups)
+                   : f64 ? launch_narrow64<2>(cx, stream, a, n2, tiles, vw[1], cos_groups)
+                         : launch_narrow<2>(cx, stream, a, n2, tiles, vw[1], cos_groups))) return rc;
     a.src = mid; a.dst = dst;
     a.stage_tw = cx.tile_tw[0];
     a.stage_twd = cx.tile_twd[0];
     tiles = geometry(2, n1, (1ull << added) << n2);
     a.k3_pairs = k3_out_of_place && vw[2] == 2 && tiles % 16 == 0 ? 1u : 0u;
     if (wide && tiles % 128 == 0) a.k3_pairs = 4;
+    if (a.cos_first) {
+        a.k3_first_tile = tiles >> added;
+        tiles -= a.k3_first_tile;
+    }
     if (wide) return launch_narrow_wide<3>(cx, stream, a, n1, tiles, 1);
     return f64 ? launch_narrow64<3>(cx, stream, a, n1, tiles, vw[2]) : launch_narrow<3>(cx, stream, a, n1, tiles, vw[2]);
 }
@@ -967,7 +973,7 @@
 }
 
 int ntt_coset_lde(Context& cx, hipStream_t stream, const uint32_t* src, uint32_t* dst, uint64_t height,
-                  uint32_t width, uint32_t added_bits, uint32_t shift, bool bit_reversed_out) {
+                  uint32_t width, uint32_t added_bits, uint32_t shift, bool bit_reversed_out, bool coset0_in_place) {
     if (!height || !width) return OK;
     if (!is_pow2(height)) return fail(ERR_BAD_ARG, "hip backend requires power-of-two height, got " + std::to_string(height));
     uint32_t n = log2u(height);
@@ -977,7 +983,7 @@
     size_t bytes = height * width * 4;
     { int rcs = cx.reserve_scale_slots(8); if (rcs) return rcs; }
     {
-        int rcn = lde_narrow(cx, stream, src, dst, n, added_bits, width, shift, bit_reversed_out);
+        int rcn = lde_narrow(cx, stream, src, dst, n, added_bits, width, shift, bit_reversed_out, false, coset0_in_place);
         if (rcn != 1) return rcn;
     }
     {
diff --git a/plonky3-mobile_amd/csrc/ntt_narrow.hip.h b/plonky3-mobile_amd/csrc/ntt_narrow.hip.h
--- a/plonky3-mobile_amd/csrc/ntt_narrow.hip.h
+++ b/plonky3-mobile_amd/csrc/ntt_narrow.hip.h
@@ -29,6 +29,8 @@
     const double2* stage_twd_fwd;
     double neg_pm1, pinv, fbias;
     uint32_t k3_pairs;
+    uint32_t cos_first;
+    uint32_t k3_first_tile;
     uint32_t blocked;
 };
 
@@ -269,7 +271,7 @@
     const uint32_t c0 = two_level(a.twf_lo, a.twf_hi, a.twf_T, (uint64_t)k1 * rev_bits(t, B - 4));
     const uint32_t phi0 = two_level(a.twf_lo, a.twf_hi, a.twf_T, (uint64_t)k1 << (B - 4));
     const uint64_t kbase = (uint64_t)k1 + ((uint64_t)t << a.n1);
-    const uint32_t cos0 = blockIdx.y * a.cos_per_block, ncos = cos0 + a.cos_per_block;
+    const uint32_t cos0 = a.cos_first + blockIdx.y * a.cos_per_block, ncos = min(cos0 + a.cos_per_block, 1u << a.added);
     uint32_t sc_next = two_level(a.sc_lo[cos0], a.sc_hi[cos0], a.sc_T, kbase);
     if (!a.from_coeffs) to_natural<B, LQ>(tile, c, t, q);
     {
@@ -317,7 +319,7 @@
     Tiles<V, (NT > 1)> tile{reinterpret_cast<V*>(smem), reinterpret_cast<V*>(smem) + (NT - 1) * (lds_rows(B) << LQ)};
     uint32_t* twl = smem + (NT * VW * lds_rows(B) << LQ);
     const uint32_t q = threadIdx.x & (NQ - 1), t = threadIdx.x >> LQ;
-    const uint32_t tile0 = k3_tile_of_block(blockIdx.x, a.k3_pairs);
+    const uint32_t tile0 = k3_tile_of_block(blockIdx.x, a.k3_pairs) + a.k3_first_tile;
     const uint32_t s = tile0 * NQ + q;
     const uint32_t blk0 = slot_row(a, tile0 * NQ), blk = slot_row(a, s), cp = slot_col(a, s, blk);
     uint32_t* p = a.dst + ((uint64_t)blk0 << B) * a.W;
diff --git a/plonky3-mobile_amd/csrc/ntt_narrow_f64.hip.h b/plonky3-mobile_amd/csrc/ntt_narrow_f64.hip.h
--- a/plonky3-mobile_amd/csrc/ntt_narrow_f64.hip.h
+++ b/plonky3-mobile_amd/csrc/ntt_narrow_f64.hip.h
@@ -288,7 +288,7 @@
     const double c0 = canon(two_level(a.twf_lo, a.twf_hi, a.twf_T, (uint64_t)k1 * rev_bits(t, B - 4)));
     const double phi0 = canon(two_level(a.twf_lo, a.twf_hi, a.twf_T, (uint64_t)k1 << (B - 4)));
     const uint64_t kbase = (uint64_t)k1 + ((uint64_t)t << a.n1);
-    const uint32_t cos0 = blockIdx.y * a.cos_per_block, ncos = cos0 + a.cos_per_block;
+    const uint32_t cos0 = a.cos_first + blockIdx.y * a.cos_per_block, ncos = min(cos0 + a.cos_per_block, 1u << a.added);
     uint32_t sc_next = two_level(a.sc_lo[cos0], a.sc_hi[cos0], a.sc_T, kbase);
     if (!a.from_coeffs) {
         to_natural<B, LQ>(tile, c, t, q);
@@ -339,7 +339,7 @@
     const Magic mk = pin_magic();
     const Uni un{a.neg_pm1, a.pinv, a.fbias};
     const uint32_t q = threadIdx.x & (NQ - 1), t = threadIdx.x >> LQ;
-    const uint32_t tile0 = k3_tile_of_block(blockIdx.x, a.k3_pairs);
+    const uint32_t tile0 = k3_tile_of_block(blockIdx.x, a.k3_pairs) + a.k3_first_tile;
     const uint32_t s = tile0 * NQ + q;
     const uint32_t blk0 = slot_row(a, tile0 * NQ), blk = slot_row(a, s), cp = slot_col(a, s, blk);
     uint32_t* p = a.dst + ((uint64_t)blk0 << B) * a.W;
diff --git a/plonky3-mobile_amd/csrc/poseidon2_f64.hip.h b/plonky3-mobile_amd/csrc/poseidon2_f64.hip.h
--- a/plonky3-mobile_amd/csrc/poseidon2_f64.hip.h
+++ b/plonky3-mobile_amd/csrc/poseidon2_f64.hip.h
@@ -130,10 +130,39 @@
     fold_integer_lanes();
 }
 
+template <int FIRST>
+__device__ __forceinline__ void external_linear_first(double (&s)[16]) {
+    static_assert(FIRST == 2 || FIRST == 4 || FIRST == 8 || FIRST == 16, "row classes: 2, 4, 8 words, or a dense state");
+    if constexpr (FIRST == 16) {
+        external_linear(s);
+    } else if constexpr (FIRST == 8) {
+        mat4(s[0], s[1], s[2], s[3]);
+        mat4(s[4], s[5], s[6], s[7]);
+#pragma unroll
+        for (int k = 0; k < 4; k++) {
+            const double t = s[k] + s[k + 4];
+            s[k] += t; s[k + 4] += t; s[k + 8] = t; s[k + 12] = t;
+        }
+    } else {
+        if constexpr (FIRST == 4) {
+            mat4(s[0], s[1], s[2], s[3]);
+        } else {
+            const double a = s[0], b = s[1], ab = a + b;
+            s[1] = ab + b; s[2] = ab; s[3] = __fma_rn(a, 2.0, ab); s[0] = s[1] + ab;
+        }
+#pragma unroll
+        for (int k = 0; k < 4; k++) {
+            const double t = s[k];
+            s[k] = t + t; s[k + 4] = t; s[k + 8] = t; s[k + 12] = t;
+        }
+    }
+}
+
+template <int FIRST = 16, bool DIGEST = false>
 __device__ __forceinline__ void permute(double (&s)[16]) {
     const MagicRegs mk = magic_regs();
     const double npm1 = d_c.neg_pm1, pinv = d_c.pinv;
-    external_linear(s);
+    external_linear_first<FIRST>(s);
     _Pragma("clang loop unroll(disable)")
     for (int r = 0; r < 4; r++) {
 #pragma unroll
@@ -142,9 +171,14 @@
     }
     internal_rounds(s, mk);
     _Pragma("clang loop unroll(disable)")
-    for (int r = 4; r < 8; r++) {
+    for (int r = 4; r < (DIGEST ? 7 : 8); r++) {
 #pragma unroll
         for (int i = 0; i < 16; i++) s[i] = sbox7(s[i] + d_c.ext[r][i], mk, npm1, pinv);
+        external_linear(s);
+    }
+    if constexpr (DIGEST) {
+#pragma unroll
+        for (int i = 0; i < 16; i++) s[i] = sbox7(s[i] + d_c.ext[7][i], mk, npm1, pinv);
         external_linear(s);
     }
 }
diff --git a/plonky3-mobile_amd/csrc/prover.hip b/plonky3-mobile_amd/csrc/prover.hip
--- a/plonky3-mobile_amd/csrc/prover.hip
+++ b/plonky3-mobile_amd/csrc/prover.hip
@@ -64,6 +64,7 @@
     const uint2* lde;
     const uint2* sel;
     uint32_t* out;
+    uint32_t* out_rev;
     const DevState* ds;
     TwoLevelTable roots;
     uint32_t n, log_n, gen, ginv, zh_inv;
@@ -72,7 +73,8 @@
     uint32_t i = blockIdx.x * blockDim.x + threadIdx.x;
     if (i >= a.n) return;
     const DevState* __restrict__ ds = a.ds;
-    uint2 loc = a.lde[brev(i, a.log_n)];
+    const uint32_t ir = brev(i, a.log_n);
+    uint2 loc = a.lde[ir];
     uint2 nxt = a.lde[brev((i + 1) & (a.n - 1), a.log_n)];
     uint2 s = a.sel[i];
     uint32_t x = bb::mul(a.gen, tl(a.roots, i));
@@ -87,55 +89,60 @@
     for (int k = 0; k < 4; k++)
         acc.c[k] = bb::add(bb::add(bb::dot2(ds->apow[4].c[k], c0, ds->apow[3].c[k], c1), bb::dot2(ds->apow[2].c[k], c2, ds->apow[1].c[k], c3)),
                            bb::mul(ds->apow[0].c[k], c4));
-    st_ext(a.out + 4 * (size_t)i, bb::scale(acc, a.zh_inv));
+    const Ext qv = bb::scale(acc, a.zh_inv);
+    st_ext(a.out + 4 * (size_t)i, qv);
+    st_ext(a.out_rev + 4 * (size_t)ir, qv);
 }
 
 constexpr int DEN_CHUNK = 4;
+constexpr int DEN_CHUNK2 = 8;
 __global__ void __launch_bounds__(256) inv_denoms_kernel(TwoLevelTable roots, uint32_t big, uint32_t log_big, uint32_t gen,
-                                                         const DevState* __restrict__ ds, uint32_t* d0, uint32_t* d1) {
-    const DenConsts k0 = ds->k0, k1 = ds->k1;
+                                                         const DevState* __restrict__ ds, uint32_t* d0, uint32_t* d1,
+                                                         uint32_t log_shift, uint32_t g_inv) {
+    const DenConsts c = ds->k0;
     uint32_t t = blockIdx.x * blockDim.x + threadIdx.x;
-    uint32_t j0 = t * DEN_CHUNK;
+    uint32_t j0 = t * DEN_CHUNK2;
     if (j0 >= big) return;
-    uint32_t a0[2 * DEN_CHUNK], e0[2 * DEN_CHUNK], e1[2 * DEN_CHUNK], nrm[2 * DEN_CHUNK], pre[2 * DEN_CHUNK];
-#pragma unroll
-    for (int k = 0; k < DEN_CHUNK; k++) {
+    uint32_t a0[DEN_CHUNK2], e0[DEN_CHUNK2], e1[DEN_CHUNK2], nrm[DEN_CHUNK2], pre[DEN_CHUNK2];
+#pragma unroll
+    for (int k = 0; k < DEN_CHUNK2; k++) {
         uint32_t x = bb::mul(gen, tl(roots, brev((j0 + k) & (big - 1), log_big)));
-#pragma unroll
-        for (int z = 0; z < 2; z++) {
-            const DenConsts& c = z ? k1 : k0;
-            const uint32_t a = bb::sub(c.z0, x);
-            const uint32_t dd0 = bb::add(bb::sqr(a), c.k0), dd1 = bb::sub(bb::mul(c.k1, a), c.c1);
-            a0[2 * k + z] = a; e0[2 * k + z] = dd0; e1[2 * k + z] = dd1;
-            nrm[2 * k + z] = bb::sub(bb::sqr(dd0), bb::mul(bb::W_MONTY, bb::sqr(dd1)));
-        }
+        const uint32_t a = bb::sub(c.z0, x);
+        const uint32_t dd0 = bb::add(bb::sqr(a), c.k0), dd1 = bb::sub(bb::mul(c.k1, a), c.c1);
+        a0[k] = a; e0[k] = dd0; e1[k] = dd1;
+        nrm[k] = bb::sub(bb::sqr(dd0), bb::mul(bb::W_MONTY, bb::sqr(dd1)));
     }
     uint32_t acc = bb::ONE;
 #pragma unroll
-    for (int k = 0; k < 2 * DEN_CHUNK; k++) { pre[k] = acc; acc = bb::mul(acc, nrm[k]); }
+    for (int k = 0; k < DEN_CHUNK2; k++) { pre[k] = acc; acc = bb::mul(acc, nrm[k]); }
     uint32_t inv = bb::inv(acc);
 #pragma unroll
-    for (int k = 2 * DEN_CHUNK - 1; k >= 0; k--) {
+    for (int k = DEN_CHUNK2 - 1; k >= 0; k--) {
         const uint32_t r = bb::mul(inv, pre[k]);
         inv = bb::mul(inv, nrm[k]);
         nrm[k] = r;
     }
 #pragma unroll
-    for (int k = 0; k < DEN_CHUNK; k++) {
+    for (int k = 0; k < DEN_CHUNK2; k++) {
         if (j0 + k >= big) break;
-#pragma unroll
-        for (int z = 0; z < 2; z++) {
-            const DenConsts& c = z ? k1 : k0;
-            const uint32_t i = 2 * k + z;
-            const uint32_t f0 = bb::mul(e0[i], nrm[i]), f1 = bb::neg(bb::mul(e1[i], nrm[i]));
-            Ext r;
-            r.c[0] = bb::add(bb::mul(a0[i], f0), bb::mul(c.z2w, f1));
-            r.c[2] = bb::add(bb::mul(a0[i], f1), bb::mul(c.z2, f0));
-            r.c[1] = bb::neg(bb::add(bb::mul(c.z1, f0), bb::mul(c.z3w, f1)));
-            r.c[3] = bb::neg(bb::add(bb::mul(c.z1, f1), bb::mul(c.z3, f0)));
-            st_ext((z ? d1 : d0) + 4 * (size_t)(j0 + k), r);
-        }
-    }
+        const uint32_t f0 = bb::mul(e0[k], nrm[k]), f1 = bb::neg(bb::mul(e1[k], nrm[k]));
+        Ext r;
+        r.c[0] = bb::add(bb::mul(a0[k], f0), bb::mul(c.z2w, f1));
+        r.c[2] = bb::add(bb::mul(a0[k], f1), bb::mul(c.z2, f0));
+        r.c[1] = bb::neg(bb::add(bb::mul(c.z1, f0), bb::mul(c.z3w, f1)));
+        r.c[3] = bb::neg(bb::add(bb::mul(c.z1, f1), bb::mul(c.z3, f0)));
+        st_ext(d0 + 4 * (size_t)(j0 + k), r);
+        const uint32_t j1 = brev((brev(j0 + k, log_big) + (1u << log_shift)) & (big - 1), log_big);
+        st_ext(d1 + 4 * (size_t)j1, bb::scale(r, g_inv));
+    }
+}
+static int launch_inv_denoms(hipStream_t st, const TwoLevelTable& roots_big, uint32_t log_big, uint32_t log_n, uint32_t gen,
+                             const DevState* ds, uint32_t* d0, uint32_t* d1) {
+    const uint32_t big = 1u << log_big, threads = (big + DEN_CHUNK2 - 1) / DEN_CHUNK2;
+    hipLaunchKernelGGL(inv_denoms_kernel, dim3((threads + 255) / 256), dim3(256), 0, st, roots_big, big, log_big, gen, ds, d0, d1,
+                       log_big - log_n, bb::inv(bb::two_adic_generator(log_n)));
+    P3_HIP(hipGetLastError());
+    return OK;
 }
 
 constexpr int BARY_BLOCK = 256;
@@ -230,25 +237,25 @@
     st_ext(out + 4 * (size_t)i, bb::add(s, d));
 }
 
-__global__ void __launch_bounds__(256) grind_kernel(DevState* ds, uint32_t mask, uint32_t base) {
-    uint32_t w = base + blockIdx.x * blockDim.x + threadIdx.x;
-    if (w >= bb::P) return;
-    if (base + blockIdx.x * blockDim.x > *(volatile uint32_t*)&ds->grind_result) return;
+__global__ void __launch_bounds__(256) grind_kernel(DevState* ds, uint32_t mask, uint32_t base, uint32_t count) {
+    const uint32_t stride = gridDim.x * blockDim.x;
+    const uint64_t end = std::min<uint64_t>((uint64_t)base + count, bb::P);
     const uint32_t pos = ds->n_in;
-    double s[16];
-#pragma unroll
-    for (int i = 0; i < 16; i++) s[i] = p2f::load_elem((i < 8 && (uint32_t)i < pos) ? ds->inb[i & 7] : ds->st[i]);
-#pragma unroll
-    for (int i = 0; i < 8; i++) s[i] = (i == (int)pos) ? (double)w : s[i];
-    p2f::permute(s);
-    if ((bb::from_monty(p2f::store_elem(s[7])) & mask) == 0) atomicMin(&ds->grind_result, w);
-}
-
-__global__ void __launch_bounds__(256) grind_keccak_kernel(DevState* ds, uint32_t mask, uint32_t base) {
-    uint32_t w = base + blockIdx.x * blockDim.x + threadIdx.x;
-    if (w >= bb::P) return;
-    if (base + blockIdx.x * blockDim.x > *(volatile uint32_t*)&ds->grind_result) return;
-    const KeccakGrindArgs& a = ds->kgrind;
+    double s0[16];
+#pragma unroll
+    for (int i = 0; i < 16; i++) s0[i] = p2f::load_elem((i < 8 && (uint32_t)i < pos) ? ds->inb[i & 7] : ds->st[i]);
+    for (uint64_t w64 = (uint64_t)base + blockIdx.x * blockDim.x + threadIdx.x; w64 < end; w64 += stride) {
+        const uint32_t w = (uint32_t)w64;
+        if (*(volatile uint32_t*)&ds->grind_result < w) return;
+        double s[16];
+#pragma unroll
+        for (int i = 0; i < 16; i++) s[i] = (i < 8 && i == (int)pos) ? (double)w : s0[i];
+        p2f::permute<16, true>(s);
+        if ((bb::from_monty(p2f::store_elem(s[7])) & mask) == 0) atomicMin(&ds->grind_result, w);
+    }
+}
+
+__device__ __forceinline__ bool grind_keccak_try(const KeccakGrindArgs& a, uint32_t mask, uint32_t w) {
     const uint32_t wm = bb::to_monty(w);
     uint64_t st[25];
 #pragma unroll
@@ -275,7 +282,16 @@
         const uint32_t v = __builtin_bswap32(hi_or_lo) & 0x7fffffffu;
         if (v < bb::P) { ok = (v & mask) == 0; break; }
     }
-    if (ok) atomicMin(&ds->grind_result, w);
+    return ok;
+}
+__global__ void __launch_bounds__(256) grind_keccak_kernel(DevState* ds, uint32_t mask, uint32_t base, uint32_t count) {
+    const uint32_t stride = gridDim.x * blockDim.x;
+    const uint64_t end = std::min<uint64_t>((uint64_t)base + count, bb::P);
+    for (uint64_t w64 = (uint64_t)base + blockIdx.x * blockDim.x + threadIdx.x; w64 < end; w64 += stride) {
+        const uint32_t w = (uint32_t)w64;
+        if (*(volatile uint32_t*)&ds->grind_result < w) return;
+        if (grind_keccak_try(ds->kgrind, mask, w)) atomicMin(&ds->grind_result, w);
+    }
 }
 
 constexpr uint32_t QTREE_MAX_MATS = 8;
@@ -730,9 +746,12 @@
     uint32_t grind_range(uint32_t first_log) const {
         return 1u << std::min<uint32_t>(std::max<uint32_t>(first_log ? first_log : fp.proof_of_work_bits + 4, 8), 24);
     }
+    static constexpr uint32_t GRIND_LANES = 1u << 14;
     int grind(const TsArgs& ts, uint64_t base, uint32_t count) {
-        if (hash == HASH_KECCAK) hipLaunchKernelGGL(grind_keccak_kernel, dim3(count / 256), dim3(256), 0, stream, ts.ds, pow_mask(), (uint32_t)base);
-        else hipLaunchKernelGGL(grind_kernel, dim3(count / 256), dim3(256), 0, stream, ts.ds, pow_mask(), (uint32_t)base);
+        const uint32_t lanes = profile == PROFILE_THROUGHPUT ? std::min(count, GRIND_LANES) : count;
+        const dim3 grid((lanes + 255) / 256);
+        if (hash == HASH_KECCAK) hipLaunchKernelGGL(grind_keccak_kernel, grid, dim3(256), 0, stream, ts.ds, pow_mask(), (uint32_t)base, count);
+        else hipLaunchKernelGGL(grind_kernel, grid, dim3(256), 0, stream, ts.ds, pow_mask(), (uint32_t)base, count);
         P3_HIP(hipGetLastError());
         return OK;
     }
@@ -970,6 +989,7 @@
             qa.lde = reinterpret_cast<const uint2*>(s.lde_t);
             qa.sel = sel;
             qa.out = s.qflat;
+            qa.out_rev = s.lde_q;
             qa.ds = s.ds;
             if ((rc = cx.get_root_table(st, log_n, false, &qa.roots))) return rc;
             qa.n = n; qa.log_n = log_n; qa.gen = gen; qa.ginv = g_n_inv;
@@ -977,7 +997,7 @@
             hipLaunchKernelGGL(fib_quotient_kernel, dim3((n + 255) / 256), dim3(256), 0, st, qa);
             P3_HIP(hipGetLastError());
         }
-        if ((rc = ntt_coset_lde(cx, st, s.qflat, s.lde_q, n, 4, s.fp.log_blowup, bb::ONE, true))) return rc;
+        if ((rc = ntt_coset_lde(cx, st, s.qflat, s.lde_q, n, 4, s.fp.log_blowup, bb::ONE, true, true))) return rc;
         if ((rc = s.commit(1, &s.lde_q, &w_quot, nullptr, big, s.layers_q, L.root_q))) return rc;
         hipLaunchKernelGGL(ts_zeta_kernel, dim3(1), dim3(64), 0, st, ts, g_n);
         P3_HIP(hipGetLastError());
@@ -986,10 +1006,7 @@
         TwoLevelTable roots_big;
         if ((rc = cx.get_root_table(st, log_big, false, &roots_big))) return rc;
         {
-            uint32_t threads = (big + DEN_CHUNK - 1) / DEN_CHUNK;
-            hipLaunchKernelGGL(inv_denoms_kernel, dim3((threads + 255) / 256), dim3(256), 0, st, roots_big, big, log_big, gen,
-                               s.ds, s.d0, s.d1);
-            P3_HIP(hipGetLastError());
+            if ((rc = launch_inv_denoms(st, roots_big, log_big, log_n, gen, s.ds, s.d0, s.d1))) return rc;
             hipLaunchKernelGGL(barycentric_kernel, dim3(s.bary_blocks), dim3(BARY_BLOCK), 0, st, roots_big, n, log_big, gen,
                                reinterpret_cast<const uint2*>(s.lde_t), reinterpret_cast<const uint4*>(s.lde_q), s.d0, s.d1,
                                s.partials);
diff --git a/plonky3-mobile_amd/csrc/prover_hiding.hip.inc b/plonky3-mobile_amd/csrc/prover_hiding.hip.inc
--- a/plonky3-mobile_amd/csrc/prover_hiding.hip.inc
+++ b/plonky3-mobile_amd/csrc/prover_hiding.hip.inc
@@ -623,9 +623,7 @@
         TwoLevelTable roots_big;
         if ((rc = cx.get_root_table(st, log_big, false, &roots_big))) return rc;
         {
-            uint32_t threads = (big + DEN_CHUNK - 1) / DEN_CHUNK;
-            hipLaunchKernelGGL(inv_denoms_kernel, dim3((threads + 255) / 256), dim3(256), 0, st, roots_big, big, log_big, gen, ds, s.d0, s.d1);
-            P3_HIP(hipGetLastError());
+            if ((rc = launch_inv_denoms(st, roots_big, log_big, log_n, gen, ds, s.d0, s.d1))) return rc;
             const size_t ps = (size_t)s.bary_blocks * 32;
             {
                 BaryAllArgs ba{};
```

Result: no change. 524.0, median of 3 (-0.6%).
